# BAMresearch/PGDrome

Hardware: AMD Instinct MI355X
Metric: PGD fixed-point iters/sec + SpMV HBM GB/s, 256^3 P1 space x 1D param (higher is better)
Workload: dtype f64

## Files before the change

### include/pgd_amd.h

```cpp
#ifndef PGD_AMD_H
#define PGD_AMD_H

#include <stdint.h>

#ifdef __cplusplus
extern "C" {
#endif

typedef int64_t pgd_handle;

enum {
    PGD_OK = 0,
    PGD_ERR_INVALID = -1,
    PGD_ERR_HIP = -2,
    PGD_ERR_NOMEM = -3,
    PGD_ERR_LIMIT = -4,
    PGD_ERR_SINGULAR = -5,
    PGD_ERR_NODEVICE = -6,
    PGD_ERR_TIMEOUT = -7,
    PGD_ERR_PEER = -8
};

enum {
    PGD_ATOM_MASS = 0,
// ... 139 lines not shown
int pgd_comm_push(pgd_handle ctx, int mode, int *state);
int pgd_comm_allreduce_attach(pgd_handle ctx, const uint8_t *all_blobs, int *state);
int pgd_comm_allreduce_direct(pgd_handle ctx, int mode, int *state);
int pgd_pcg_solve_sharded(pgd_handle ctx, pgd_handle A, pgd_handle b, pgd_handle x, int64_t own0,
                          int64_t own1, int64_t lo_ghost, int64_t hi_ghost, double rtol, double atol,
                          int maxit, int *iters, double *rel_res);

int pgd_bicgstab_solve(pgd_handle ctx, pgd_handle A, pgd_handle b, pgd_handle x, double rtol, double atol,
                       int maxit, int *iters, double *rel_res);

int pgd_start_gram(pgd_handle ctx, pgd_handle A, const pgd_handle *vecs, int k, pgd_handle b, int64_t r0,
                   int64_t r1, double *out);
int pgd_start_residual(pgd_handle ctx, pgd_handle A, int k, const double *coefs, pgd_handle b, pgd_handle r);

int pgd_vec_multidot(pgd_handle ctx, pgd_handle x, const pgd_handle *ys, int k, int64_t lo, int64_t hi,
                     double *out);

int pgd_vec_multidot_pair(pgd_handle ctx, pgd_handle x0, pgd_handle x1, const pgd_handle *ys, int k, int64_t lo,
                          int64_t hi, double *out);

enum { PGD_BLOCK_F32 = 0, PGD_BLOCK_F64 = 1 };
int pgd_block_create(pgd_handle ctx, int64_t n, int k, int dtype, pgd_handle *block);
int pgd_block_free(pgd_handle ctx, pgd_handle block);
int pgd_block_info(pgd_handle ctx, pgd_handle block, int64_t *n, int *k, int *dtype, int64_t *bytes);
int pgd_block_storage(pgd_handle ctx, int *dtype);
int pgd_block_set_column(pgd_handle ctx, pgd_handle block, int j, pgd_handle vec);
int pgd_block_get_column(pgd_handle ctx, pgd_handle block, int j, pgd_handle vec);
int pgd_block_dots(pgd_handle ctx, pgd_handle block, pgd_handle vec_r, int64_t lo, int64_t hi, double *out);
int pgd_block_combine(pgd_handle ctx, pgd_handle block, const double *coefs, pgd_handle vec_base_or_0, pgd_handle vec_x);

enum { PGD_EVAL_STATS = 1, PGD_EVAL_ENVELOPE = 2, PGD_EVAL_EXCEED = 4, PGD_EVAL_FIELDS = 8 };
int pgd_eval_batch(pgd_handle ctx, const pgd_handle *modes, int k, const double *coefs, int64_t s, int want,
                   double threshold, double *sample_stats, pgd_handle env_min, pgd_handle env_max, pgd_handle exceed,
                   pgd_handle fields);

int pgd_cell_gradient(pgd_handle ctx, pgd_handle mesh, pgd_handle u, const double *L, int q, pgd_handle scale_or_0,
                      pgd_handle out);

int pgd_eval_batch_norm(pgd_handle ctx, const pgd_handle *modes, int k, int q, const double *coefs, int64_t s, int want,
                        double threshold, double *sample_stats, pgd_handle env_min, pgd_handle env_max, pgd_handle exceed,
                        pgd_handle fields);
int pgd_eval_batch_grad(pgd_handle ctx, pgd_handle mesh, const pgd_handle *modes, int k, const double *L, int q,
                        pgd_handle scale_or_0, const double *coefs, int64_t s, int want, double threshold, double *sample_stats,
                        pgd_handle env_min, pgd_handle env_max, pgd_handle exceed, pgd_handle fields);
int pgd_eval_norm_last_shape(pgd_handle ctx, int *rows, int *staged);

int pgd_cell_gradient_p2(pgd_handle ctx, pgd_handle mesh, pgd_handle u, const double *lam, int npt, const double *L, int q,
                         pgd_handle scale_or_0, pgd_handle out);
int pgd_eval_batch_grad_p2(pgd_handle ctx, pgd_handle mesh, const pgd_handle *modes, int k, const double *lam, int npt,
                           const double *L, int q, pgd_handle scale_or_0, const double *coefs, int64_t s, int want, double threshold,
                           double *sample_stats, pgd_handle env_min, pgd_handle env_max, pgd_handle exceed, pgd_handle fields);

enum {
    PGD_TUNE_SPMV_P2_LATTICE = 59,
    PGD_TUNE_SPMV_BLOCK_DIA = 58,
    PGD_TUNE_PCG_FUSED_MARCH = 57,
    PGD_TUNE_PCG_SCALAR_S = 56,
    PGD_TUNE_PCG_FOLD_MARCH = 55,
    PGD_TUNE_BLOCK_STORAGE = 54,
    PGD_TUNE_PCG_RECOMPUTE_Q = 53,
    PGD_TUNE_EVAL_SAMPLE_CHUNK = 52,
    PGD_TUNE_EVAL_GRID_MAX = 51,
    PGD_TUNE_EVAL_VARIANT = 50,
    PGD_TUNE_PUSH_IN_UPDATE = 49,
    PGD_TUNE_STENCIL_ROWS = 48,
    PGD_TUNE_DIA_MARCH3 = 47,
    PGD_TUNE_SHARD_ONE_MARCH = 46,
    PGD_TUNE_HALO_OVERLAP_MIN_ROWS = 45,
    PGD_TUNE_COMM_SELF_PERIODIC = 44,
    PGD_TUNE_PCG_DERIVE_SCALED = 43,
    PGD_TUNE_MG_MARCH_MIN = 42,
    PGD_TUNE_MG_CHUNK = 41,
    PGD_TUNE_PCG_PRECOND = 40,
    PGD_TUNE_CLS_CACHE = 39,
    PGD_TUNE_STENCIL_DEPTH = 38,
    PGD_TUNE_STENCIL_WG_PER_CU = 37,
    PGD_TUNE_SPMV_ZCHUNK_STENCIL = 36,
    PGD_TUNE_SPMV_STENCIL = 35,
    PGD_TUNE_FAULT_STALL_MS = 34,
    PGD_TUNE_FAULT_STAGE = 33,
    PGD_TUNE_SPMV_ZCHUNK_CODED2 = 32,
    PGD_TUNE_PCG_PIPELINE = 31,
    PGD_TUNE_PCG_EXACT_PHASE = 30,
    PGD_TUNE_PCG_FOLD_FINISH = 29,
    PGD_TUNE_LAZY_CSR = 28,
    PGD_TUNE_ATOM_FAST = 27,
    PGD_TUNE_SPMV_ROWS = 1,
    PGD_TUNE_SPMV_GRID_MIN_BYTES = 8,
    PGD_TUNE_PCG_FOLD_REDUCE = 12,
    PGD_TUNE_PCG_SCALED = 10,
    PGD_TUNE_SPMV_ZCHUNK_FORCE = 7,
    PGD_TUNE_PCG_SMALL_ROWS = 26,
    PGD_TUNE_PCG_SMALL_SINGLE_SYNC = 25,
    PGD_TUNE_SPMV_FETCH_DEPTH = 24,
    PGD_TUNE_PCG_STREAM_HINTS = 23,
    PGD_TUNE_PCG_LAG_X = 22,
    PGD_TUNE_SPMV_ZCHUNK_CODED = 21,
    PGD_TUNE_ASM_LATTICE = 20,
    PGD_TUNE_SPMV_ROW_CLASSES = 19,
    PGD_TUNE_PCG_SINGLE_SYNC = 18,
    PGD_TUNE_UNIT_DIAG = 17,
    PGD_TUNE_PCG_DEFER_X = 16,
    PGD_TUNE_FAULT_ITERATION = 15,
    PGD_TUNE_COMBINE_DIA = 14,
    PGD_TUNE_SPMV_VARIANT = 13,
    PGD_TUNE_SPMV_ZCHUNK = 6,
    PGD_TUNE_SPMV_SYM = 3,
    PGD_TUNE_SPMV_DICT = 2
};
int pgd_tune(pgd_handle ctx, int knob, int64_t value);

int pgd_prof_enable(pgd_handle ctx, int on);
int pgd_prof_read(pgd_handle ctx, int64_t *launches, double *seconds, double *alg_bytes);
int pgd_prof_read_own(pgd_handle ctx, double *own_bytes);
int pgd_prof_read_update(pgd_handle ctx, int64_t *launches, double *seconds, double *bytes);
int pgd_prof_read_dropped(pgd_handle ctx, int64_t *dropped);
int pgd_prof_event_overhead(pgd_handle ctx, double *seconds);
int pgd_kernel_counts(pgd_handle ctx, int64_t *out, int n);
int pgd_pcg_recompute_counts(pgd_handle ctx, int64_t *updates);
int pgd_pcg_fused_counts(pgd_handle ctx, int64_t *marches);
int pgd_classify_counts(pgd_handle ctx, int64_t *full, int64_t *cached);
int pgd_mg_counts(pgd_handle ctx, int64_t *solves, int64_t *fallbacks);
int pgd_vmg_counts(pgd_handle ctx, int64_t *solves, int64_t *fallbacks, int64_t *levels);
int pgd_vmg_times(pgd_handle ctx, double *setup_ms, int64_t *march_passes);
int pgd_cmg_counts(pgd_handle ctx, int64_t *solves, int64_t *fallbacks, int64_t *levels);
int pgd_cmg_times(pgd_handle ctx, double *setup_ms, int64_t *march_passes);
int pgd_pmg_counts(pgd_handle ctx, int64_t *solves, int64_t *fallbacks, int64_t *levels);
int pgd_pmg_times(pgd_handle ctx, double *setup_ms, int64_t *march_passes);
int pgd_pmg_coarse(pgd_handle ctx, int comp, double *slots_out, uint8_t *el_out);
int pgd_bdia_counts(pgd_handle ctx, int64_t *forms_built, int64_t *products, int64_t *fallbacks);
int pgd_bdia_times(pgd_handle ctx, double *extract_ms);
int pgd_p2lat_counts(pgd_handle ctx, int64_t *forms_built, int64_t *products, int64_t *fallbacks);
int pgd_p2lat_times(pgd_handle ctx, double *extract_ms);
int pgd_mg_slab_setup(pgd_handle ctx, pgd_handle A, int nz_global, int z_first, int64_t own0, int64_t own1,
                      int64_t *n_coarse, int *applies);
int pgd_mg_slab_fix_start(pgd_handle ctx, pgd_handle A, pgd_handle b, pgd_handle x, int64_t own0, int64_t own1);
int pgd_mg_slab_down(pgd_handle ctx, pgd_handle r, pgd_handle t);
int pgd_mg_slab_restrict(pgd_handle ctx, pgd_handle t, pgd_handle b1);
int pgd_mg_coarse(pgd_handle ctx, pgd_handle b1, pgd_handle x1);
int pgd_mg_slab_up(pgd_handle ctx, pgd_handle r, pgd_handle x1, pgd_handle t, pgd_handle z, int slot, double *dot);
int pgd_calib_stream(pgd_handle ctx, pgd_handle vec, int bytes_per_lane, int store);
int pgd_timer_start(pgd_handle ctx);
int pgd_timer_stop(pgd_handle ctx, double *seconds);

#ifdef __cplusplus
}
#endif
#endif
```

### pgdrome_amd/_lib.py

```python
from __future__ import annotations

import ctypes as C
from pathlib import Path

import numpy as np

LIB_PATH = Path(__file__).resolve().parent / "lib" / "libpgd_amd.so"

H = C.c_int64
I64 = C.c_int64
I32 = C.c_int32
F64 = C.c_double
PD = C.POINTER(C.c_double)
PI32 = C.POINTER(C.c_int32)
PI64 = C.POINTER(C.c_int64)
PH = C.POINTER(C.c_int64)
VP = C.c_void_p

PU8 = C.POINTER(C.c_uint8)
HALO_FN = C.CFUNCTYPE(C.c_int, VP, H, I64, I64, I64, I64)
ALLREDUCE_FN = C.CFUNCTYPE(C.c_int, VP, C.c_int, C.c_int)

SIGNATURES = {
    "pgd_ctx_create": (C.c_int, [C.c_int, VP, PH]),
# ... 63 lines not shown
    "pgd_mg_slab_up": (C.c_int, [H, H, H, H, H, C.c_int, PD]),
    "pgd_bicgstab_solve": (C.c_int, [H, H, H, H, C.c_double, C.c_double, C.c_int, C.POINTER(C.c_int), PD]),
    "pgd_atom_product_form": (C.c_int, [H, H, C.POINTER(C.c_int)]),
    "pgd_product_plan": (C.c_int, [H, H, I64, I64, C.c_int, PI64, C.c_int]),
    "pgd_vec_multidot": (C.c_int, [H, H, PH, C.c_int, I64, I64, PD]),
    "pgd_vec_multidot_pair": (C.c_int, [H, H, H, PH, C.c_int, I64, I64, PD]),
    "pgd_pcg_solve": (C.c_int, [H, H, H, H, F64, F64, C.c_int, C.POINTER(C.c_int), PD]),
    "pgd_pcg_last_form": (C.c_int, [H, C.POINTER(C.c_int), C.POINTER(C.c_int)]),
    "pgd_band_solve": (C.c_int, [H, H, H, H]),
    "pgd_slots_ptr": (C.c_int, [H, C.POINTER(VP)]),
    "pgd_slots_download": (C.c_int, [H, PD, C.c_int, C.c_int]),
    "pgd_slots_upload": (C.c_int, [H, PD, C.c_int, C.c_int]),
    "pgd_flags_reset": (C.c_int, [H]),
    "pgd_flags_download": (C.c_int, [H, PI32, PI32, PI32]),
    "pgd_op_diag_inv": (C.c_int, [H, H, H]),
    "pgd_spmv_dot_slot": (C.c_int, [H, H, H, H, H, I64, I64, C.c_int]),
    "pgd_pcg_init_slot": (C.c_int, [H, H, H, H, H, H, H, I64, I64, C.c_int]),
    "pgd_pcg_tol_slot": (C.c_int, [H, F64, F64, C.c_int, C.c_int, C.c_int]),
    "pgd_pcg_xr_slot": (C.c_int, [H, H, H, H, H, H, H, I64, I64, C.c_int, C.c_int, C.c_int]),
    "pgd_pcg_check_slot": (C.c_int, [H, C.c_int, C.c_int]),
    "pgd_pcg_p_slot": (C.c_int, [H, H, H, I64, I64, C.c_int, C.c_int]),
    "pgd_cg_init_slot": (C.c_int, [H, H, H, H, H, H, H, H, I64, I64, C.c_int]),
    "pgd_cg_update_slot": (C.c_int, [H, H, H, H, H, H, H, H, I64, I64, C.c_int]),
    "pgd_cg_scalars_slot": (C.c_int, [H, C.c_int, C.c_int, F64, F64]),
    "pgd_comm_bind_callbacks": (C.c_int, [H, HALO_FN, ALLREDUCE_FN, VP, C.c_int, C.c_int]),
    "pgd_comm_unique_id": (C.c_int, [H, PU8]),
    "pgd_comm_bind_rccl": (C.c_int, [H, PU8, C.c_int, C.c_int]),
    "pgd_comm_overlap": (C.c_int, [H, C.c_int, C.POINTER(C.c_int)]),
    "pgd_comm_unbind": (C.c_int, [H]),
    "pgd_comm_timeout": (C.c_int, [H, F64]),
    "pgd_comm_prof": (C.c_int, [H, C.c_int, PD]),
    "pgd_comm_info": (C.c_int, [H, C.POINTER(C.c_int), C.POINTER(C.c_int), C.POINTER(C.c_int)]),
    "pgd_comm_halo": (C.c_int, [H, H, I64, I64, I64, I64]),
    "pgd_comm_allreduce_slots": (C.c_int, [H, C.c_int, C.c_int]),
    "pgd_comm_push_export": (C.c_int, [H, I64, I64, I64, I64, I64, PU8]),
    "pgd_comm_push_attach": (C.c_int, [H, PU8, PU8, C.POINTER(C.c_int)]),
    "pgd_comm_push": (C.c_int, [H, C.c_int, C.POINTER(C.c_int)]),
    "pgd_comm_allreduce_attach": (C.c_int, [H, PU8, C.POINTER(C.c_int)]),
    "pgd_comm_allreduce_direct": (C.c_int, [H, C.c_int, C.POINTER(C.c_int)]),
    "pgd_pcg_solve_sharded": (C.c_int, [H, H, H, H, I64, I64, I64, I64, F64, F64, C.c_int, C.POINTER(C.c_int), PD]),
    "pgd_op_symmetrize": (C.c_int, [H, H, C.POINTER(C.c_int)]),
    "pgd_op_classify": (C.c_int, [H, H, C.POINTER(C.c_int)]),
    "pgd_tune": (C.c_int, [H, C.c_int, I64]),
    "pgd_prof_enable": (C.c_int, [H, C.c_int]),
    "pgd_prof_read": (C.c_int, [H, PI64, PD, PD]),
    "pgd_prof_read_own": (C.c_int, [H, PD]),
    "pgd_prof_read_update": (C.c_int, [H, PI64, PD, PD]),
    "pgd_prof_read_dropped": (C.c_int, [H, PI64]),
    "pgd_prof_event_overhead": (C.c_int, [H, PD]),
    "pgd_kernel_counts": (C.c_int, [H, PI64, C.c_int]),
    "pgd_pcg_recompute_counts": (C.c_int, [H, PI64]),
    "pgd_pcg_fused_counts": (C.c_int, [H, PI64]),
    "pgd_classify_counts": (C.c_int, [H, PI64, PI64]),
    "pgd_mg_counts": (C.c_int, [H, PI64, PI64]),
    "pgd_vmg_counts": (C.c_int, [H, PI64, PI64, PI64]),
    "pgd_vmg_times": (C.c_int, [H, C.POINTER(C.c_double), PI64]),
    "pgd_cmg_counts": (C.c_int, [H, PI64, PI64, PI64]),
    "pgd_cmg_times": (C.c_int, [H, C.POINTER(C.c_double), PI64]),
    "pgd_pmg_counts": (C.c_int, [H, PI64, PI64, PI64]),
    "pgd_pmg_times": (C.c_int, [H, C.POINTER(C.c_double), PI64]),
    "pgd_pmg_coarse": (C.c_int, [H, C.c_int, PD, PU8]),
    "pgd_bdia_counts": (C.c_int, [H, PI64, PI64, PI64]),
    "pgd_bdia_times": (C.c_int, [H, C.POINTER(C.c_double)]),
    "pgd_p2lat_counts": (C.c_int, [H, PI64, PI64, PI64]),
    "pgd_p2lat_times": (C.c_int, [H, C.POINTER(C.c_double)]),
    "pgd_calib_stream": (C.c_int, [H, H, C.c_int, C.c_int]),
    "pgd_timer_start": (C.c_int, [H]),
    "pgd_timer_stop": (C.c_int, [H, PD]),
}

NSLOTS = 64
EVAL_STATS, EVAL_ENVELOPE, EVAL_EXCEED, EVAL_FIELDS = 1, 2, 4, 8
TUNE_EVAL_VARIANT, TUNE_EVAL_GRID_MAX, TUNE_EVAL_SAMPLE_CHUNK = 50, 51, 52
TUNE_BLOCK_STORAGE = 54
TUNE_PCG_FOLD_MARCH, TUNE_PCG_SCALAR_S, TUNE_PCG_FUSED_MARCH = 55, 56, 57
TUNE_SPMV_BLOCK_DIA = 58
TUNE_SPMV_P2_LATTICE = 59
BLOCK_F32, BLOCK_F64, BLOCK_MAXK = 0, 1, 64


ERR_TIMEOUT, ERR_PEER = -7, -8


class PgdError(RuntimeError):
    def __init__(self, code, msg):
        super().__init__(f"libpgd_amd error {code}: {msg}")
        self.code = code


_lib = None


def load(path: Path | None = None):
    global _lib
    if _lib is not None and path is None:
        return _lib
    p = Path(path) if path else LIB_PATH
    if not p.exists():
        raise RuntimeError(
            f"{p} not found: build the HIP library first (python -m pgdrome_amd.build). "
            "pgdrome_amd has no CPU fallback.")
    _preload_hip_runtime()
    lib = C.CDLL(str(p))
    for name, (res, args) in SIGNATURES.items():
        fn = getattr(lib, name)
        fn.restype = res
# ... 620 lines not shown
        n = C.c_int(0)
        self._ck(self.lib.pgd_op_classify(self.h, op, C.byref(n)))
        return int(n.value)

    def tune(self, knob, value):
        self._ck(self.lib.pgd_tune(self.h, int(knob), int(value)))

    def prof_enable(self, on=True):
        self._ck(self.lib.pgd_prof_enable(self.h, int(on)))

    def prof_read(self):
        n, s, b = I64(), F64(), F64()
        self._ck(self.lib.pgd_prof_read(self.h, C.byref(n), C.byref(s), C.byref(b)))
        own = F64()
        self._ck(self.lib.pgd_prof_read_own(self.h, C.byref(own)))
        un, us, ub = I64(), F64(), F64()
        self._ck(self.lib.pgd_prof_read_update(self.h, C.byref(un), C.byref(us), C.byref(ub)))
        dr, ov = I64(), F64()
        self._ck(self.lib.pgd_prof_read_dropped(self.h, C.byref(dr)))
        self._ck(self.lib.pgd_prof_event_overhead(self.h, C.byref(ov)))
        return dict(launches=n.value, seconds=s.value, bytes=b.value, own_bytes=own.value,
                    update_launches=un.value, update_seconds=us.value, update_bytes=ub.value, dropped_noop_samples=dr.value,
                    event_overhead=ov.value)

    KERNEL_FAMILIES = ("csr", "csr_dict", "sym_rows", "dia_rows", "dia_march", "multi", "diac_march", "stencil_march")

    def kernel_counts(self):
        out = (C.c_int64 * 8)()
        self._ck(self.lib.pgd_kernel_counts(self.h, out, 8))
        return {k: int(out[i]) for i, k in enumerate(self.KERNEL_FAMILIES)}

    def product_plan(self, op, r0=0, r1=-1, pcg_like=True):
        out = (C.c_int64 * 7)()
        self._ck(self.lib.pgd_product_plan(self.h, op, int(r0), int(r1), 1 if pcg_like else 0, out, 7))
        plan = dict(zip(("form", "wgs", "zchunk", "tiles_x", "tiles_y", "rows_per_thread", "depth"), map(int, out)))
        plan["family"] = self.KERNEL_FAMILIES[plan["form"]] if plan["form"] >= 0 else None
        return plan

    def pcg_recompute_updates(self):
        n = I64()
        self._ck(self.lib.pgd_pcg_recompute_counts(self.h, C.byref(n)))
        return n.value

    def pcg_fused_marches(self):
        n = I64()
        self._ck(self.lib.pgd_pcg_fused_counts(self.h, C.byref(n)))
        return n.value

    def classify_counts(self):
        full, cached = I64(), I64()
        self._ck(self.lib.pgd_classify_counts(self.h, C.byref(full), C.byref(cached)))
        return {"full": full.value, "cached": cached.value}

    def precondition(self, multigrid):
        self.tune(40, 1 if multigrid else 0)
        return self.mg_stats()["solves"]

    def mg_stats(self):
        a, b = I64(), I64()
        self._ck(self.lib.pgd_mg_counts(self.h, C.byref(a), C.byref(b)))
        return {"solves": a.value, "fallbacks": b.value}

    def precondition_variable(self, on):
        self.tune(40, 2 if on else 0)
        return self.vmg_stats()["solves"]

    def vmg_stats(self):
        a, b, l, m, ms = I64(), I64(), I64(), I64(), C.c_double()
        self._ck(self.lib.pgd_vmg_counts(self.h, C.byref(a), C.byref(b), C.byref(l)))
        self._ck(self.lib.pgd_vmg_times(self.h, C.byref(ms), C.byref(m)))
        return {"solves": a.value, "fallbacks": b.value, "levels": l.value, "setup_ms": ms.value, "march_passes": m.value}

    def precondition_component(self, on):
        self.tune(40, 3 if on else 0)
        return self.cmg_stats()["solves"]

    def cmg_stats(self):
        a, b, l, m, ms = I64(), I64(), I64(), I64(), C.c_double()
        self._ck(self.lib.pgd_cmg_counts(self.h, C.byref(a), C.byref(b), C.byref(l)))
        self._ck(self.lib.pgd_cmg_times(self.h, C.byref(ms), C.byref(m)))
        return {"solves": a.value, "fallbacks": b.value, "levels": l.value, "setup_ms": ms.value, "march_passes": m.value}

    def precondition_p(self, on):
        self.tune(40, 4 if on else 0)
        return self.pmg_stats()["solves"]

    def pmg_stats(self):
        a, b, l, m, ms = I64(), I64(), I64(), I64(), C.c_double()
        self._ck(self.lib.pgd_pmg_counts(self.h, C.byref(a), C.byref(b), C.byref(l)))
        self._ck(self.lib.pgd_pmg_times(self.h, C.byref(ms), C.byref(m)))
        return {"solves": a.value, "fallbacks": b.value, "levels": l.value, "setup_ms": ms.value, "march_passes": m.value}

    def pmg_coarse(self, comp, nvert):
        slots = np.empty((8, int(nvert)), dtype=np.float64)
        el = np.empty(int(nvert), dtype=np.uint8)
        self._ck(self.lib.pgd_pmg_coarse(self.h, int(comp), dptr(slots), el.ctypes.data_as(PU8)))
        return slots, el

    def block_product(self, on):
        self.tune(TUNE_SPMV_BLOCK_DIA, 1 if on else 0)
        return self.bdia_stats()["products"]

    def bdia_stats(self):
        f, p, b, ms = I64(), I64(), I64(), C.c_double()
        self._ck(self.lib.pgd_bdia_counts(self.h, C.byref(f), C.byref(p), C.byref(b)))
        self._ck(self.lib.pgd_bdia_times(self.h, C.byref(ms)))
# ... 23 lines not shown
```

### pgdrome_amd/csrc/pgd_classify.hip

```cpp
#include <algorithm>
#include <cstdarg>
#include <cstdlib>
#include <cstring>

#include "pgd_internal.h"

namespace pgd {

constexpr int CLS_SLOTS = 1024;

struct StencilInfo { int ok, ident, base, split; double c[8]; int zm0, zm1, g_lo, g_hi; };

__global__ void k_stencil_pick(const uint8_t *__restrict__ cls, double *__restrict__ table, const int *__restrict__ info,
                               int nx, int ny, int z_lo, int z_hi, StencilInfo *S) {
    if (threadIdx.x != 0 || blockIdx.x != 0) return;
    S->ok = 0; S->ident = -1; S->base = -1; S->split = 0;
    const int ncls = info[0];
    if (info[1] != 0 || ncls <= 0 || ncls >= CLS_MAX || z_hi <= z_lo) return;
    const int64_t mid = (int64_t)nx * ny * ((z_lo + z_hi) / 2) + (int64_t)nx * (ny / 2) + nx / 2;
    for (int k = 0; k < ncls; ++k) {
        bool id = table[k * 8 + cls_pos(0)] == 1.0;
        for (int s = 1; s < 8; ++s) id = id && table[k * 8 + cls_pos(s)] == 0.0;
        if (id) S->ident = k;
    }
    int base = cls[mid], best = -1;
    for (int k = 0; k < ncls; ++k) {
        int nzc = 0;
        for (int s = 1; s < 8; ++s) nzc += table[k * 8 + cls_pos(s)] != 0.0 ? 1 : 0;
        if (nzc > best || (nzc == best && k == (int)cls[mid])) { best = nzc; base = k; }
    }
    if (base == S->ident) return;
    S->base = base;
    for (int s = 0; s < 8; ++s) S->c[s] = table[base * 8 + cls_pos(s)];
    if (S->ident >= 0) {
        for (int s = 0; s < 8; ++s) { table[ncls * 8 + s] = table[S->ident * 8 + s]; table[(ncls + 1) * 8 + s] = 0.0; }
    }
    S->ok = 1;
}

__global__ __launch_bounds__(TPB) void k_stencil_split(uint8_t *__restrict__ cls, const double *__restrict__ table, const int *__restrict__ info,
                                                       int nx, int ny, int64_t nv, StencilInfo *S) {
    if (!S->ok || S->ident < 0) return;
    const int64_t i = (int64_t)blockIdx.x * TPB + threadIdx.x;
    if (i >= nv || (int)cls[i] != S->ident) return;
    const int64_t P = (int64_t)nx * ny;
    const int z = (int)(i / P), rem = (int)(i - (int64_t)z * P), y = rem / nx, x = rem - y * nx;
    bool coupled = false;
#pragma unroll
    for (int s = 1; s < 8; ++s) {
        const int dx = s & 1, dy = (s >> 1) & 1, dz = s >> 2;
        if (x - dx < 0 || y - dy < 0 || z - dz < 0) continue;
        const int kc = cls[i - dx - (int64_t)nx * dy - P * dz];
        coupled = coupled || table[kc * 8 + cls_pos(s)] != 0.0;
    }
    if (coupled) { cls[i] = (uint8_t)info[0]; S->split = 1; }
}

__global__ void k_stencil_commit(double *__restrict__ table, int *__restrict__ info, StencilInfo *S) {
    if (threadIdx.x != 0 || blockIdx.x != 0 || !S->ok || S->ident < 0) return;
    const int n = info[0];
    if (S->split) info[0] = n + 1;
    else for (int s = 0; s < 8; ++s) table[n * 8 + s] = 0.0;
// ... 228 lines not shown
        if (k == ident) {
            good = table[k * 8 + cls_pos(0)] == 1.0;
            for (int s = 1; s < 8; ++s) good = good && table[k * 8 + cls_pos(s)] == 0.0;
        } else {
            good = __double_as_longlong(table[k * 8 + cls_pos(0)]) == __double_as_longlong(table[base * 8 + cls_pos(0)]);
            for (int s = 1; s < 8; ++s) {
                const double v = table[k * 8 + cls_pos(s)];
                good = good && (((pat.b[k] >> s) & 1) ? v == 0.0
                                                      : __double_as_longlong(v) == __double_as_longlong(table[base * 8 + cls_pos(s)]));
            }
        }
        if (!good) s_bad = 1;
    }
    __syncthreads();
    if (threadIdx.x == 0) {
        S->ok = s_bad ? 0 : 1; S->ident = ident; S->base = base; S->split = 0;
        for (int s = 0; s < 8; ++s) S->c[s] = table[base * 8 + cls_pos(s)];
    }
}

__global__ __launch_bounds__(TPB) void k_cls_reps(const uint8_t *__restrict__ cls, int64_t nv, int *__restrict__ reps) {
    const int64_t i = (int64_t)blockIdx.x * TPB + threadIdx.x;
    const bool active = i < nv;
    const int code = active ? (int)cls[i] : -1;
    unsigned long long todo = __ballot(active);
    const int lane = threadIdx.x & 63;
    while (todo) {
        const int leader = __ffsll((long long)todo) - 1;
        const int c0 = __shfl(code, leader);
        todo &= ~__ballot(active && code == c0);
        if (lane == leader && reps[c0] > (int)i) atomicMin(&reps[c0], (int)i);
    }
}

struct ClsJob {
    Ctx *c; const Mesh *m; Csr *a;
    int64_t plane;
    int nzp, z_lo, z_hi, g;
    bool try_stencil, dbg_cls, dbg_stencil;
    int scaled_key;
    ClsScratch *S; StencilInfo *SI;
    int info[4]; StencilInfo si;
};

__attribute__((format(printf, 2, 3))) static void cls_debug(bool on, const char *fmt, ...) {
    if (!on) return;
    va_list ap;
    va_start(ap, fmt);
    vfprintf(stderr, fmt, ap);
    va_end(ap);
}

static size_t plane_flag_bytes(int nzp) { return ((size_t)nzp * sizeof(int) + 63) / 64 * 64; }

constexpr size_t CLS_CACHE_MAX = 4, CLS_REPS_BYTES = 256 * sizeof(int);

static bool cls_cache_alloc(Mesh::ClsCache &E, int64_t nv, int nzp) {
    const size_t same_b = plane_flag_bytes(nzp);
    if (hipMalloc(&E.block, (size_t)nv + same_b + CLS_REPS_BYTES + 64 + PAD_BYTES) != hipSuccess) { E.block = nullptr; return false; }
    E.same = (int *)E.block;
    E.reps = (int *)((uint8_t *)E.block + same_b);
    E.codes = (uint8_t *)E.block + same_b + CLS_REPS_BYTES;
    return true;
}

static void cls_cache_touch(const Mesh *m, Mesh::ClsCache &E) { E.used = ++m->cls_clock; }

static void cls_cache_insert(const Mesh *m, Mesh::ClsCache &E) {
    cls_cache_touch(m, E);
    if (m->cls_cache.size() >= CLS_CACHE_MAX) {
        size_t old = 0;
        for (size_t e = 1; e < m->cls_cache.size(); ++e) if (m->cls_cache[e].used < m->cls_cache[old].used) old = e;
        m->cls_cache[old].release();
        m->cls_cache.erase(m->cls_cache.begin() + (long)old);
    }
    m->cls_cache.push_back(E);
}

static int cls_begin(ClsJob &J, Ctx *c, const Mesh *m, Csr *a, int zrange_lo, int zrange_hi, bool *go) {
    *go = false;
    if (!c->spmv_classes || m->sym_nx <= 0 || !(a->uvals && a->uvals_valid) || m->nv >= ((int64_t)1 << 31)) return PGD_OK;
    const int64_t plane = (int64_t)m->sym_nx * m->sym_ny;
    if (m->nv / plane < 3 || plane * 64 < c->spmv_grid_min_plane_bytes) return PGD_OK;
    if (m->nv / plane > 65536) return PGD_OK;
    void *p;
    if (!c->cls_scratch) { PGD_TRY(dev_alloc(c, &p, sizeof(ClsScratch) + sizeof(StencilInfo) + 2 * 65536 * sizeof(int))); c->cls_scratch = p; }
    const int nzp = (int)(m->nv / plane);
    if (!a->cls) {
        const size_t table_b = (size_t)(CLS_MAX + 1) * 8 * sizeof(double), same_b = plane_flag_bytes(nzp);
        a->cls_bytes = (size_t)m->nv + table_b + same_b + 64;
        PGD_TRY(dev_alloc(c, &p, a->cls_bytes));
        a->cls_table = (double *)p;
        a->cls_same = (int *)((uint8_t *)p + table_b);
        a->cls = (uint8_t *)a->cls_same + same_b;
    }
    J.c = c; J.m = m; J.a = a;
    J.plane = plane; J.nzp = nzp;
    J.g = (int)((m->nv + TPB - 1) / TPB);
    J.z_lo = 0; J.z_hi = nzp;
    if (zrange_lo >= 0) { J.z_lo = std::max(0, zrange_lo); J.z_hi = std::min(nzp, zrange_hi); }
    J.S = (ClsScratch *)c->cls_scratch;
    J.SI = reinterpret_cast<StencilInfo *>(J.S + 1);
    J.try_stencil = c->spmv_stencil && J.z_hi - J.z_lo >= 3;
    J.scaled_key = (a->uvals_scaled ? 1 : 0) + (a->uvals_unit ? 2 : 0) + (J.try_stencil ? 4 : 0);
    J.dbg_cls = getenv("PGD_DEBUG_CLS") != nullptr;
    J.dbg_stencil = getenv("PGD_DEBUG_STENCIL") != nullptr;
    *go = true;
    return PGD_OK;
}

static void adopt_stencil(Csr *a, const StencilInfo &si, int z_lo, int z_hi) {
    a->st_ok = true;
    a->st_ident = si.ident;
    a->st_z0 = z_lo; a->st_z1 = z_hi;
    a->st_zm0 = si.zm0; a->st_zm1 = si.zm1;
    a->st_g_lo = si.g_lo != 0; a->st_g_hi = si.g_hi != 0;
    for (int s2 = 0; s2 < 8; ++s2) a->st_c[s2] = si.c[s2];
}

static int verify_known(ClsJob &J, const Mesh::ClsCache &E) {
    Ctx *c = J.c; const Mesh *m = J.m; Csr *a = J.a;
    hipStream_t st = c->stream;
    PGD_HIP(c, hipMemsetAsync(J.S->info, 0, sizeof J.S->info, st));
    PGD_HIP(c, hipMemcpyAsync(a->cls, E.codes, (size_t)m->nv, hipMemcpyDeviceToDevice, st));
    PGD_HIP(c, hipMemcpyAsync(a->cls_same, E.same, (size_t)J.nzp * sizeof(int), hipMemcpyDeviceToDevice, st));
    k_cls_table_known<<<1, 256, 0, st>>>(a->uvals, a->uvals_stride, m->nv, E.reps, E.ncls, a->cls_table);
    k_cls_verify_known<<<J.g, TPB, 0, st>>>(a->uvals, a->uvals_stride, m->nv, a->cls_table, a->cls, E.ncls, J.S->info);
    J.si.ok = 0;
    if (E.st_ok) {
        ZeroPat zp, use;
        memcpy(zp.b, E.zero_pat, sizeof zp.b);
        memcpy(use.b, E.in_range, sizeof use.b);
        k_stencil_known<<<1, 256, 0, st>>>(a->cls_table, E.ncls, E.ident, E.base, zp, use, J.SI);
        k_stencil_ghost_init<<<1, 1, 0, st>>>(J.SI, J.z_lo, J.z_hi, J.nzp, E.zm0, E.zm1);
        if (J.z_lo > 0 || J.z_hi < J.nzp)
            k_stencil_ghost<<<(int)((J.plane + TPB - 1) / TPB), TPB, 0, st>>>(a->cls, a->cls_table, m->sym_nx, m->sym_ny, J.z_lo, J.z_hi, E.zm0, J.SI);
    }
    J.info[1] = 1;
    PGD_HIP(c, hipMemcpyAsync(J.info, J.S->info, sizeof J.info, hipMemcpyDeviceToHost, st));
    if (E.st_ok) PGD_HIP(c, hipMemcpyAsync(&J.si, J.SI, sizeof(StencilInfo), hipMemcpyDeviceToHost, st));
    PGD_HIP(c, hipStreamSynchronize(st));
    PGD_LAUNCH_CHECK(c);
    if (E.st_ok) { J.si.zm0 = E.zm0; J.si.zm1 = E.zm1; }
    return PGD_OK;
}

static int classify_known(ClsJob &J, bool *hit) {
    Ctx *c = J.c; const Mesh *m = J.m; Csr *a = J.a;
    *hit = false;
    for (size_t e = 0; e < m->cls_cache.size(); ++e) {
        Mesh::ClsCache &E = m->cls_cache[e];
        if (E.sig != a->bc_sig || E.scaled != J.scaled_key || E.z_lo != J.z_lo || E.z_hi != J.z_hi || !E.codes) continue;
        PGD_TRY(verify_known(J, E));
        cls_debug(J.dbg_cls, "[dia_classify] known structure %zu of %zu: z %d..%d mismatches %d (info %d %d %d %d) stencil %d -> %d\n", e,
                  m->cls_cache.size(), J.z_lo, J.z_hi, J.info[1], J.info[0], J.info[1], J.info[2], J.info[3], (int)E.st_ok, J.si.ok);
        if (J.info[1] != 0 || (E.st_ok && !J.si.ok)) {
            E.release();
            m->cls_cache.erase(m->cls_cache.begin() + (long)e);
            return PGD_OK;
        }
        cls_cache_touch(m, E);
        c->cls_fast += 1;
        a->cls_count = E.ncls;
        if (E.st_ok) adopt_stencil(a, J.si, J.z_lo, J.z_hi);
        *hit = true;
        return PGD_OK;
    }
    return PGD_OK;
}

static int classify_full(ClsJob &J) {
    Ctx *c = J.c; const Mesh *m = J.m; Csr *a = J.a;
    ClsScratch *S = J.S; StencilInfo *SI = J.SI;
    hipStream_t st = c->stream;
    const int g = J.g, nzp = J.nzp, z_lo = J.z_lo, z_hi = J.z_hi;
    c->cls_full += 1;
    PGD_HIP(c, hipMemsetAsync(S->keys, 0, sizeof S->keys, st));
    PGD_HIP(c, hipMemsetAsync(S->rep, 0x7f, sizeof S->rep, st));
    PGD_HIP(c, hipMemsetAsync(S->info, 0, sizeof S->info, st));
    k_cls_insert<<<g, TPB, 0, st>>>(a->uvals, a->uvals_stride, m->nv, S);
    k_cls_table<<<1, CLS_SLOTS, 0, st>>>(a->uvals, a->uvals_stride, S, a->cls_table);
    k_cls_assign<<<g, TPB, 0, st>>>(a->uvals, a->uvals_stride, m->nv, S, a->cls_table, a->cls);
    if (J.try_stencil) {
        k_stencil_pick<<<1, 64, 0, st>>>(a->cls, a->cls_table, S->info, m->sym_nx, m->sym_ny, z_lo, z_hi, SI);
        k_stencil_split<<<g, TPB, 0, st>>>(a->cls, a->cls_table, S->info, m->sym_nx, m->sym_ny, m->nv, SI);
        k_stencil_commit<<<1, 64, 0, st>>>(a->cls_table, S->info, SI);
    }
    k_cls_planes<<<nzp, TPB, 0, st>>>(a->cls, J.plane, nzp, a->cls_same);
    if (J.try_stencil) {
        const int64_t rows = J.plane * (z_hi - z_lo);
        k_stencil_verify<<<(int)((rows + TPB - 1) / TPB), TPB, 0, st>>>(a->cls, a->cls_table, m->sym_nx, m->sym_ny, nzp, z_lo, z_hi, SI);
        int *allid = reinterpret_cast<int *>(SI + 1);
        k_stencil_allid<<<nzp, TPB, 0, st>>>(a->cls, J.plane, SI, allid, allid + 65536);
        k_stencil_planes<<<1, 64, 0, st>>>(allid + 65536, allid, z_lo, z_hi, SI);
        k_stencil_ghost_init<<<1, 1, 0, st>>>(SI, z_lo, z_hi, nzp, -1, -1);
        if (z_lo > 0 || z_hi < nzp)
            k_stencil_ghost<<<(int)((J.plane + TPB - 1) / TPB), TPB, 0, st>>>(a->cls, a->cls_table, m->sym_nx, m->sym_ny, z_lo, z_hi, -1, SI);
    }
    J.info[0] = 0; J.info[1] = 1; J.si.ok = 0;
    PGD_HIP(c, hipMemcpyAsync(J.info, S->info, sizeof J.info, hipMemcpyDeviceToHost, st));
    if (J.try_stencil) PGD_HIP(c, hipMemcpyAsync(&J.si, SI, sizeof(StencilInfo), hipMemcpyDeviceToHost, st));
    PGD_HIP(c, hipStreamSynchronize(st));
    PGD_LAUNCH_CHECK(c);
    if (J.info[1] != 0 || J.info[0] <= 0 || J.info[0] > CLS_MAX) return PGD_OK;
    a->cls_count = J.info[0];
    cls_debug(J.dbg_stencil, "[dia_classify] classes %d info1 %d try %d ok %d ident %d base %d c = %.17g %.17g %.17g %.17g %.17g %.17g %.17g %.17g  z [%d, %d)\n",
              J.info[0], J.info[1], (int)J.try_stencil, J.si.ok, J.si.ident, J.si.base, J.si.c[0], J.si.c[1], J.si.c[2], J.si.c[3], J.si.c[4],
              J.si.c[5], J.si.c[6], J.si.c[7], z_lo, z_hi);
    cls_debug(J.dbg_stencil, "[dia_classify] main run [%d, %d)\n", J.si.zm0, J.si.zm1);
    return PGD_OK;
}

static bool cls_cache_fill(const ClsJob &J, Mesh::ClsCache &E, int (&reps_rng)[256], double *tab) {
    const Mesh *m = J.m; const Csr *a = J.a;
    hipStream_t st = J.c->stream;
    bool okc = hipMemcpyAsync(E.codes, a->cls, (size_t)m->nv, hipMemcpyDeviceToDevice, st) == hipSuccess &&
               hipMemcpyAsync(E.same, a->cls_same, (size_t)J.nzp * sizeof(int), hipMemcpyDeviceToDevice, st) == hipSuccess &&
               hipMemsetAsync(E.reps, 0x7f, CLS_REPS_BYTES, st) == hipSuccess;
    if (okc) {
        const int64_t r0 = (int64_t)J.z_lo * J.plane, r1 = std::min<int64_t>((int64_t)J.z_hi * J.plane, m->nv);
        if (r1 > r0) k_cls_reps<<<(int)((r1 - r0 + TPB - 1) / TPB), TPB, 0, st>>>(a->cls + r0, r1 - r0, E.reps);
        okc = hipMemcpyAsync(reps_rng, E.reps, sizeof reps_rng, hipMemcpyDeviceToHost, st) == hipSuccess &&
              hipStreamSynchronize(st) == hipSuccess && hipMemsetAsync(E.reps, 0x7f, CLS_REPS_BYTES, st) == hipSuccess;
    }
    if (okc) {
        k_cls_reps<<<J.g, TPB, 0, st>>>(a->cls, m->nv, E.reps);
        okc = hipMemcpyAsync(tab, a->cls_table, (size_t)(E.ncls + 1) * 8 * sizeof(double), hipMemcpyDeviceToHost, st) == hipSuccess &&
              hipStreamSynchronize(st) == hipSuccess;
    }
    return okc;
}

static void remember(const ClsJob &J) {
    const Csr *a = J.a;
    const int ncls = a->cls_count;
    Mesh::ClsCache E;
    E.sig = a->bc_sig; E.scaled = J.scaled_key; E.z_lo = J.z_lo; E.z_hi = J.z_hi; E.ncls = ncls;
    if (!cls_cache_alloc(E, J.m->nv, J.nzp)) { (void)hipGetLastError(); return; }
    double tab[(CLS_MAX + 1) * 8];
    int reps_rng[256];
    if (!cls_cache_fill(J, E, reps_rng, tab)) {
        E.release();
        (void)hipGetLastError();
        return;
    }
    E.st_ok = a->st_ok; E.ident = a->st_ident; E.base = J.try_stencil ? J.si.base : -1; E.zm0 = a->st_zm0; E.zm1 = a->st_zm1;
    for (int k = 0; k < 256; ++k) E.in_range[k] = (k < ncls && reps_rng[k] >= 0 && reps_rng[k] < 0x7f000000) ? 1 : 0;
    for (int k = 0; k < 256; ++k) {
        uint8_t b = 0;
        if (k < ncls) for (int s2 = 1; s2 < 8; ++s2) if (tab[k * 8 + cls_pos(s2)] == 0.0) b |= (uint8_t)(1u << s2);
        E.zero_pat[k] = b;
    }
    if (E.base >= 0) for (int k = 0; k < ncls; ++k) E.zero_pat[k] &= (uint8_t)~E.zero_pat[E.base];
    cls_cache_insert(J.m, E);
}

int dia_classify(Ctx *c, const Mesh *m, Csr *a, int zrange_lo, int zrange_hi) {
    a->drop_classes();
    ClsJob J;
    bool go = false, hit = false;
    PGD_TRY(cls_begin(J, c, m, a, zrange_lo, zrange_hi, &go));
    if (!go) return PGD_OK;
    if (c->cls_cache_on) PGD_TRY(classify_known(J, &hit));
    if (hit) return PGD_OK;
    PGD_TRY(classify_full(J));
    if (a->cls_count <= 0) return PGD_OK;
    if (J.try_stencil && J.si.ok) adopt_stencil(a, J.si, J.z_lo, J.z_hi);
    if (c->cls_cache_on) remember(J);
    return PGD_OK;
}

}
```

### pgdrome_amd/csrc/pgd_internal.h

```cpp
#pragma once

#include <hip/hip_runtime.h>

#include <chrono>
#include <cstdint>
#include <cstdio>
#include <map>
#include <memory>
#include <string>
#include <vector>

#include "../../include/pgd_amd.h"

namespace pgd {

constexpr int WAVE = 64;
constexpr int TPB = 256;
constexpr int MAX_VEC_BLOCKS = 2048;
constexpr int N_XCD = 8;
constexpr int DICT_MAXP = 256;
constexpr int DICT_DLEN = 32;
constexpr size_t PAD_BYTES = 256;

enum { S_PQ = 2, S_TOL2 = 5, S_DMIN = 7 , S_TMP = 8  };
enum { S1_RZ = 24, S1_RR = 25, S1_ALPHA = 26, S1_BETA = 27, S1_PQ = 28, S1_QQ = 29,
       S1_ALPHA_PREV = 40, S1_BETA_PREV = 41, S1_PEND = 42 };
enum { S1F_ALPHA = 44 , S1F_BETA = 46 , S1F_EXACT = 48  };
constexpr double LAG_MIN_BETA = 0.01;

struct Ctx;
void dev_release(Ctx *c, void *p, size_t bytes);

struct Obj {
    enum Kind { FREE = 0, VEC, MESH, CSR, BLOCK } kind = FREE;
    Ctx *ctx = nullptr;
    uint64_t serial = 0;
    virtual ~Obj() {}
};

struct Vec : Obj {
    double *d = nullptr;
    int64_t n = 0;
    ~Vec() override { if (d) dev_release(ctx, d, (size_t)(n > 0 ? n : 1) * sizeof(double)); }
};

struct Block : Obj {
    void *d = nullptr;
    int64_t n = 0, stride = 0;
    int k = 0, dtype = 0;
    size_t bytes = 0;
    ~Block() override { if (d) dev_release(ctx, d, bytes); }
};

struct Mesh : Obj {
    int gdim = 0, nvpc = 0;
    int ncomp = 1;
    pgd_handle base = 0;
    int64_t nv = 0, nc = 0, nnz = 0;
    double *coords = nullptr;
    int4 *cells = nullptr;
    int *cellsN = nullptr;
    int *v2c_ptr = nullptr;
    int *v2c = nullptr;
    int *row_ptr = nullptr;
    int *cols = nullptr;
    int max_row = 0, kl = 0, ku = 0;
    int *sym_tab = nullptr;
    int sym_w = 0;
    int sym_nx = 0, sym_ny = 0;
    bool lattice = false;
    bool lattice_unit = false;
    bool lattice_regular = false;
    int pat_off[6][4] = {{0}};
    int pat_loc[6][8] = {{0}};
    double lat_h[3] = {0.0, 0.0, 0.0};
    struct ClsCache {
        uint64_t sig = 0; int scaled = 0, z_lo = 0, z_hi = 0, ncls = 0;
        void *block = nullptr;
        uint8_t *codes = nullptr; int *same = nullptr; int *reps = nullptr;
        bool st_ok = false; int ident = -1, base = -1, zm0 = 0, zm1 = 0;
        uint8_t zero_pat[256];
        uint8_t in_range[256];
        uint64_t used = 0;
        void release() { if (block) (void)hipFree(block); block = nullptr; codes = nullptr; same = reps = nullptr; }
    };
    mutable std::vector<ClsCache> cls_cache;
    mutable uint64_t cls_clock = 0;
    std::vector<int32_t> bc_host;
    int *bc_dev = nullptr;
    size_t bc_dev_bytes = 0;
    uint16_t *pids = nullptr;
    int *dict_off = nullptr;
    int dict_count = 0;
    int p2_bound = 0;
    int p2_nx = 0, p2_ny = 0, p2_nz = 0;
    int64_t p2_nvert = 0;
    int *p2_par = nullptr;
    int *p2_v2e = nullptr;
    int p2_lat = 0;
    ~Mesh() override {
        for (void *p : {(void *)coords, (void *)cells, (void *)cellsN, (void *)v2c_ptr, (void *)v2c,
                        (void *)row_ptr, (void *)cols, (void *)pids, (void *)dict_off, (void *)sym_tab, (void *)p2_par, (void *)p2_v2e})
            if (p) (void)hipFree(p);
        for (ClsCache &e : cls_cache) e.release();
        if (bc_dev) (void)hipFree(bc_dev);
    }
};

struct Csr : Obj {
    pgd_handle mesh = 0;
    double *vals = nullptr;
    double *dinv = nullptr;
    bool dinv_valid = false;
    double *uvals = nullptr;
    bool uvals_valid = false;
    bool uvals_scaled = false;
    bool uvals_unit = false;
    int64_t uvals_stride = 0;
    uint8_t *cls = nullptr;
    int *cls_same = nullptr;
    double *cls_table = nullptr;
    int cls_count = 0;
    uint64_t bc_sig = 0;
    bool st_ok = false;
    int st_ident = -1, st_z0 = 0, st_z1 = 0, st_zm0 = 0, st_zm1 = 0;
    double st_c[8] = {0, 0, 0, 0, 0, 0, 0, 0};
    bool st_g_lo = false, st_g_hi = false;
    void drop_classes() { cls_count = 0; st_ok = false; st_g_lo = st_g_hi = false; }
    bool st_virtual = false;
    bool cls_tried = false;
    bool immutable = false;
    uint64_t version = 0;
    bool vals_pending = false;
    std::vector<pgd_handle> rec_atoms;
    std::vector<uint64_t> rec_serials, rec_versions;
    std::vector<double> rec_coefs;
    int *rec_bc = nullptr;
    int64_t rec_nbc = 0;
    size_t rec_bc_bytes = 0;
    size_t vals_bytes = 0, dinv_bytes = 0, uvals_bytes = 0, cls_bytes = 0;
    double *bdia = nullptr;
    size_t bdia_bytes = 0;
    int64_t bdia_stride = 0;
    uint64_t bdia_seen = 0;
    bool bdia_ok = false;
    double *p2lat = nullptr;
    size_t p2lat_bytes = 0;
    int64_t p2lat_sv = 0, p2lat_se = 0;
    uint64_t p2lat_seen = 0;
    bool p2lat_ok = false;
    ~Csr() override {
        if (p2lat) dev_release(ctx, p2lat, p2lat_bytes);
        if (bdia) dev_release(ctx, bdia, bdia_bytes);
        if (rec_bc) dev_release(ctx, rec_bc, rec_bc_bytes);
        if (cls_table) dev_release(ctx, cls_table, cls_bytes);
        if (vals) dev_release(ctx, vals, vals_bytes);
        if (dinv) dev_release(ctx, dinv, dinv_bytes);
        if (uvals) dev_release(ctx, uvals, uvals_bytes);
    }
};

struct Comm {
    int kind = 0;
    int rank = 0, world = 1;
    pgd_halo_fn halo_cb = nullptr;
    pgd_allreduce_fn allreduce_cb = nullptr;
    void *user = nullptr;
    void *nccl = nullptr;
    void *nccl_halo = nullptr;
    hipStream_t halo_stream = nullptr;
    hipEvent_t ev_ready = nullptr, ev_halo = nullptr;
    bool overlap = false;
    int64_t overlap_min_rows = (int64_t)1 << 40;
    bool overlap_used = false;
    bool self_periodic = false;
    pgd_handle work[7] = {0, 0, 0, 0, 0, 0, 0};
    int64_t work_n = 0;
    double timeout_s = 60.0;
    int *snap_flags = nullptr;
    double *snap_vote = nullptr;
    hipEvent_t snap_ev[2] = {nullptr, nullptr};
    bool prof = false;
    hipEvent_t mark[2][7] = {{nullptr, nullptr, nullptr, nullptr, nullptr, nullptr, nullptr}, {nullptr, nullptr, nullptr, nullptr, nullptr, nullptr, nullptr}};
// ... 50 lines not shown

    Comm comm;

    int num_cu = 256;
    int spmv_dict = 1;
    int spmv_rows = 64;
    int64_t spmv_grid_min_plane_bytes = 0;
    int spmv_zchunk_force = 0;
    int fault_iteration = -1;
    int fault_stage = 0;
    int fault_stall_ms = 0;
    int64_t pcg_small_ss_rows = (int64_t)1 << 22;
    int pcg_small_ss = 1;
    int pcg_stream_hints = 1;
    int pcg_lag_x = 1;
    int pcg_recompute_q = 1;
    int64_t pcg_recompute_launches = 0;
    int pcg_fold_march = 0;
    int64_t pcg_fused_launches = 0;
    int pcg_fused_march = 1;
    int pcg_scalar_s = 1;
    int asm_lattice = 1;
    int spmv_fetch_depth = 6;
    int spmv_zchunk_coded2 = 96;
    int spmv_zchunk_coded = 24;
    int pcg_exact_phase = 1;
    int pcg_fold_finish = 1;
    int atom_fast = 1;
    int lazy_csr = 1;
    uint64_t next_serial = 1;
    int pcg_precond = 0;
    struct Mg *mg = nullptr;
    struct Mg *mg_slab = nullptr;
    int64_t mg_solves = 0, mg_fallbacks = 0;
    struct Vmg *vmg = nullptr;
    int64_t vmg_solves = 0, vmg_fallbacks = 0, vmg_marches = 0;
    double vmg_setup_ms = 0.0;
    struct Cmg *cmg = nullptr;
    int64_t cmg_solves = 0, cmg_fallbacks = 0, cmg_marches = 0;
    double cmg_setup_ms = 0.0;
    struct Pmg *pmg = nullptr;
    int64_t pmg_solves = 0, pmg_fallbacks = 0, pmg_marches = 0;
    double pmg_setup_ms = 0.0;
    int eval_variant = 1, eval_grid_max = 0, eval_chunk = 0;
    int eval_norm_rows = 0, eval_norm_staged = -1;
    double *eval_pin = nullptr;
    size_t eval_pin_bytes = 0;
    hipEvent_t eval_ev[2] = {nullptr, nullptr};
    bool eval_ev_set[2] = {false, false};
    int mg_chunk = 2;
    int mg_march_min = 64;
    int cls_cache_on = 1;
    int64_t cls_fast = 0, cls_full = 0;
    int spmv_stencil = 1;
    int spmv_zchunk_stencil = 0;
    int stencil_depth = 0;
    int stencil_wg_per_cu = 2;
    int spmv_classes = 1;
    void *cls_scratch = nullptr;
    double *gram_w = nullptr;
    size_t gram_w_bytes = 0;
    pgd_handle gram_op = 0;
    int gram_k = 0;
    int64_t gram_n = 0;
    int spmv_variant = 0;
    int spmv_zchunk = 8;
    int pcg_fold_reduce = 1;
    int spmv_qq = 0;
    int pcg_single_sync = 1;
    int spmv_unit_diag = 1;
    int pcg_defer_x = 1;
    int pcg_scaled = 1;
    int stencil_rows = 0;
    int dia_march3 = 0;
    int push_in_update = 1;
    int shard_one_march = 1;
    int pcg_derive_scaled = 1;
    int spmv_combine_dia = 1;
    int spmv_sym = 1;
    int spmv_block_dia = 0;
    int64_t bdia_forms = 0, bdia_products = 0, bdia_fallbacks = 0;
    double bdia_extract_ms = 0.0;
    hipEvent_t bdia_ev[2] = {nullptr, nullptr};
    int spmv_p2_lattice = 0;
    int64_t p2lat_forms = 0, p2lat_products = 0, p2lat_fallbacks = 0;
    double p2lat_extract_ms = 0.0;
    hipEvent_t p2lat_ev[2] = {nullptr, nullptr};
    uint16_t *p2lat_tab = nullptr;
    int16_t *p2lat_slot = nullptr;
    int block_storage = 1;

    bool prof = false;
    bool prof_pcg_only = false;
    std::vector<hipEvent_t> ev;
    struct ProfRec { uint8_t kind; int iter; double bytes, own, seconds; };
    std::vector<ProfRec> ev_rec;
    std::vector<ProfRec> prof_pend;
    int prof_iter = -1;
    int64_t prof_dropped = 0;
    double prof_overhead = -1.0;
    size_t ev_used = 0;
    int64_t prof_upd_launches = 0, prof_upd_seen = 0;
    double prof_upd_seconds = 0.0, prof_upd_bytes = 0.0;
    int64_t prof_launches = 0, prof_seen = 0;
    double prof_seconds = 0.0, prof_bytes = 0.0;
    double prof_own_bytes = 0.0;
// ... 6 lines not shown
};

struct ProfIterGuard { Ctx *c; ~ProfIterGuard() { c->prof_iter = -1; } };
inline double host_now() { return std::chrono::duration<double>(std::chrono::steady_clock::now().time_since_epoch()).count(); }

enum { KC_CSR = 0, KC_CSR_DICT = 1, KC_SYM_ROWS = 2, KC_DIA_ROWS = 3, KC_DIA_MARCH = 4, KC_MULTI = 5, KC_DIAC_MARCH = 6, KC_STENCIL_MARCH = 7 };

Ctx *get_ctx(pgd_handle h);
int fail(Ctx *c, int code, const char *fmt, ...);
pgd_handle put_obj(Ctx *c, Obj *o);
Obj *get_obj(Ctx *c, pgd_handle h, Obj::Kind k);
int free_obj(Ctx *c, pgd_handle h, Obj::Kind k);
int dev_alloc(Ctx *c, void **p, size_t bytes);
int ensure_partials(Ctx *c, int64_t n);
int ensure_work(Ctx *c, int i, int64_t n);
int ensure_mask(Ctx *c, int64_t n);
int pcg_flag_snapshots(Ctx *c);
int ensure_ibuf(Ctx *c, int64_t n);
void prof_flush(Ctx *c);
void prof_commit(Ctx *c, int valid_products, int valid_updates);
void comm_release(Ctx *c);
struct Mesh;
struct Csr;
int build_sym_tables(Ctx *c, Mesh *m);
int ensure_sym(Ctx *c, const Mesh *m, Csr *a, bool *usable);
int cg_init_s(Ctx *c, const double *b, const double *q, const double *sc, double *r, double *p, double *s, int64_t lo,
              int64_t hi, int base);
int cg_update_s(Ctx *c, double *x, double *r, const double *w, double *p, double *s, const double *sc, int64_t lo, int64_t hi,
                int base);
int cg_update_s2(Ctx *c, double *x, double *r, const double *w, double *p, double *s, const double *sc, int64_t lo, int64_t hi,
                 int base, int parity, int *nblocks);
int reduce_two_slots(Ctx *c, int na, int nb, int base);
int pcg1_seed(Ctx *c, int npairs, int slot_rz, int slot_rr);
int pcg1_tol(Ctx *c, int base, double rtol, double atol, int slot_p8);
int pcg1_aux(Ctx *c, const double *s, const double *r, int64_t lo, int64_t hi, int slot);
int pcg1_sums(Ctx *c, int nprod, int nvec, int base);
int pcg1_finish_slots(Ctx *c, int base);
struct PushArgs {
    double *dst_lo = nullptr, *dst_hi = nullptr;
    int64_t lo_end = 0, hi_begin = 0;
    unsigned long long *post_lo = nullptr, *post_hi = nullptr;
    const unsigned long long *wait_a = nullptr, *wait_b = nullptr;
    unsigned long long seq = 0, *ticket = nullptr;
    unsigned int nblocks = 0;
    long long ticks = 0;
};
unsigned int pcg1_update_push_blocks(int g, int64_t lo, int64_t hi, int64_t lo_end, int64_t hi_begin);
int pcg1_update(Ctx *c, double *x, double *r, double *p, const double *q, const double *sc, int64_t lo, int64_t hi, int base,
                int *nblocks, int lag, int fold_par, const PushArgs *push = nullptr);
int pcg1_flush_x(Ctx *c, double *x, const double *p, const double *r, int64_t lo, int64_t hi, int base, int fold_par);
int vec_sqrt(Ctx *c, double *v, int64_t n);
int vec_div_mul(Ctx *c, double *x, const double *sc, int64_t n, int mul);
int ensure_vals(Ctx *c, const Mesh *m, Csr *a);
bool atom_fast_form(Ctx *c, const Mesh *m, Csr *a, int64_t r0, int64_t r1);
constexpr int CLS_MAX = 255;
__host__ __device__ constexpr int cls_pos(int s) {
    return s == 1 ? 0 : s == 5 ? 1 : s == 3 ? 2 : s == 7 ? 3 : s == 2 ? 4 : s == 6 ? 5 : s == 4 ? 6 : 7;
}
int dia_classify(Ctx *c, const Mesh *m, Csr *a, int zrange_lo = -1, int zrange_hi = -1);
bool stencil_row_range(const Ctx *c, const Mesh *m, const Csr *a, int64_t r0, int64_t r1);
bool stencil_whole_grid(const Ctx *c, const Mesh *m, const Csr *a);
struct StencilFold {
    const double *prod; int nprod;
    const double *vec_in; int nvec;
    int par;
};
int stencil_update_blocks(const Ctx *c, const Mesh *m, const Csr *a);
int launch_stencil_update(Ctx *c, const Mesh *m, const Csr *a, const double *p_in, double *p_out, double *x, double *r, const double *s,
                          double *pairs, int lag, double s_free = 0.0, const StencilFold *fold = nullptr);
bool stencil_fused_ok(const Ctx *c, const Mesh *m, const Csr *a);
int launch_stencil_fused(Ctx *c, const Mesh *m, const Csr *a, const double *p_in, double *p_out, double *x, const double *r_in, double *r_out,
                         const double *s, double *pairs, int lag, double s_free);
int launch_stencil_pass(Ctx *c, const uint8_t *cls, int ident, const double cst[8], int nx, int ny, int nz, int zm0, int zm1,
                        const double *x, const double *b, double *y, double w, int epi, bool dot, int *nparts, int z0 = 0, int z1 = -1);
bool mg_prepare(Ctx *c, const Mesh *m, const Csr *a);
int mg_fix_start(Ctx *c, const Csr *a, const double *b, double *x, int64_t n);
int mg_vcycle(Ctx *c, const double *r, bool dot, int *nparts, double *z_out = nullptr);
double *mg_result(Ctx *c);
void mg_release(Ctx *c);
struct Vmg;
bool vmg_prepare(Ctx *c, Vmg *&M, const Mesh *m, const Csr *a);
int vmg_fix_start(Ctx *c, Vmg *M, const double *sc, const double *b, double *x, int64_t n);
int vmg_vcycle(Ctx *c, Vmg *M, const double *r, bool dot, int *nparts, double *z_out, int64_t *marches);
double *vmg_result(Vmg *M);
void vmg_note_setup(Ctx *c);
void vmg_release(Ctx *c);
bool cmg_prepare(Ctx *c, const Mesh *m, const Mesh *base, const Csr *a);
int cmg_fix_start(Ctx *c, const double *b, double *x, int64_t n);
int cmg_apply(Ctx *c, const double *r, double *z, int64_t n, int *nparts);
void cmg_note_setup(Ctx *c);
bool pmg_prepare(Ctx *c, const Mesh *m, const Csr *a);
int pmg_fix_start(Ctx *c, const double *b, double *x, int64_t n);
int pmg_apply(Ctx *c, const Csr *a, const double *r, double *z, int64_t n, int *nparts);
void pmg_note_setup(Ctx *c);
void pmg_release(Ctx *c);
void eval_release(Ctx *c);
int sym_scale(Ctx *c, const Mesh *m, Csr *a, const double *s);
int launch_spmv_dia_rows2(Ctx *c, const Mesh *m, const Csr *a, const double *x, double *y, const double *w, int64_t r0a,
                          int64_t r1a, int64_t r0b, int64_t r1b, bool dot, const int *flags, int *nparts_out, bool *done);
int combine_dia(Ctx *c, const Mesh *m, Csr *o, Csr *const *atoms, const double *coefs, int n, const uint8_t *mask);
int launch_spmv_op(Ctx *c, const Mesh *m, const Csr *a, const double *x, double *y, const double *w, int64_t r0,
                   int64_t r1, bool dot, bool store, const int *flags, int *nparts_out);
int launch_spmv_bdia(Ctx *c, const Mesh *m, Csr *a, const double *x, double *y, const double *w, bool dot, bool store,
                     const int *flags, int *nparts_out, bool *done);
bool p2lat_degree2(Ctx *c, const Mesh *m);
int launch_spmv_p2lat(Ctx *c, const Mesh *m, Csr *a, const double *x, double *y, const double *w, bool dot, bool store,
// ... 107 lines not shown
```

### pgdrome_amd/csrc/pgd_pcg.hip

```cpp
#include "pgd_internal.h"

#include <cmath>

#include <cstring>

#include <algorithm>

namespace pgd {

constexpr int MAXT = 8;
constexpr int CHECK_EVERY = 16;
constexpr int PROF_EAGER_EVERY = 8;

struct CombineArgs {
    const double *in[MAXT];
    double coef[MAXT];
    int n;
};

__global__ __launch_bounds__(TPB) void k_combine(CombineArgs A, double *__restrict__ out, const int *__restrict__ cols,
                                                 const uint8_t *__restrict__ colmask, int64_t nnz) {
    for (int64_t k = (int64_t)blockIdx.x * TPB + threadIdx.x; k < nnz; k += (int64_t)gridDim.x * TPB) {
        double s = 0.0;
#pragma unroll
        for (int t = 0; t < MAXT; ++t)
            if (t < A.n) s = fma(A.coef[t], A.in[t][k], s);
        if (colmask && colmask[cols[k]]) s = 0.0;
        out[k] = s;
    }
}

__global__ __launch_bounds__(TPB) void k_mask_set(uint8_t *__restrict__ mask, const int *__restrict__ dofs, int64_t n) {
    for (int64_t i = (int64_t)blockIdx.x * TPB + threadIdx.x; i < n; i += (int64_t)gridDim.x * TPB) mask[dofs[i]] = 1;
}

__global__ __launch_bounds__(TPB) void k_dirichlet_rows(const int *__restrict__ dofs, int64_t n,
                                                        const int *__restrict__ row_ptr, const int *__restrict__ cols,
                                                        double *__restrict__ vals) {
    for (int64_t i = (int64_t)blockIdx.x * TPB + threadIdx.x; i < n; i += (int64_t)gridDim.x * TPB) {
        const int r = dofs[i];
        for (int k = row_ptr[r]; k < row_ptr[r + 1]; ++k) vals[k] = (cols[k] == r) ? 1.0 : 0.0;
    }
}

__global__ __launch_bounds__(TPB) void k_diag_inv(const int *__restrict__ row_ptr, const int *__restrict__ cols,
                                                  const double *__restrict__ vals, double *__restrict__ dinv, int64_t n) {
    for (int64_t r = (int64_t)blockIdx.x * TPB + threadIdx.x; r < n; r += (int64_t)gridDim.x * TPB) {
        double d = 0.0;
        for (int k = row_ptr[r]; k < row_ptr[r + 1]; ++k)
            if (cols[k] == (int)r) d = vals[k];
        dinv[r] = 1.0 / d;
    }
}
// ... 323 lines not shown
                    const double t = W[a1]; W[a1] = W[a2]; W[a2] = t;
                }
                const double t = rhs[j]; rhs[j] = rhs[piv]; rhs[piv] = t;
            }
            const double dinv = 1.0 / W[kv + (int64_t)j * ld];
            for (int i = j + 1; i <= imax; ++i) {
                const double l = W[(i - j + kv) + (int64_t)j * ld] * dinv;
                if (l != 0.0) {
                    for (int cc = j + 1; cc <= cmax; ++cc)
                        W[(i - cc + kv) + (int64_t)cc * ld] -= l * W[(j - cc + kv) + (int64_t)cc * ld];
                    rhs[i] -= l * rhs[j];
                }
            }
        }
        if (!singular) {
            for (int j = n - 1; j >= 0; --j) {
                const int cmax = min(j + kv, n - 1);
                double s = rhs[j];
                for (int cc = j + 1; cc <= cmax; ++cc) s -= W[(j - cc + kv) + (int64_t)cc * ld] * rhs[cc];
                rhs[j] = s / W[kv + (int64_t)j * ld];
            }
        } else {
            flags[2] = PGD_ERR_SINGULAR;
        }
    }
    __syncthreads();
    for (int i = threadIdx.x; i < n; i += TPB) x[i] = rhs[i];
}


__global__ __launch_bounds__(TPB) void k_scale_in(const double *__restrict__ dinv, double *__restrict__ s,
                                                  double *__restrict__ x, int64_t n, unsigned long long *__restrict__ dmax_bits) {
    double mx = 0.0;
    for (int64_t i = (int64_t)blockIdx.x * TPB + threadIdx.x; i < n; i += (int64_t)gridDim.x * TPB) {
        const double di = dinv[i], si = sqrt(di);
        s[i] = si;
        x[i] = x[i] / si;
        mx = fmax(mx, di);
    }
    for (int o = 32; o > 0; o >>= 1) mx = fmax(mx, __shfl_xor(mx, o));
    if ((threadIdx.x & 63) == 0) {
        const unsigned long long mine = (unsigned long long)__double_as_longlong(mx);
        if (mine > __hip_atomic_load(dmax_bits, __ATOMIC_RELAXED, __HIP_MEMORY_SCOPE_AGENT)) atomicMax(dmax_bits, mine);
    }
}

struct StencilTuple { double c[8]; };
__global__ void k_stencil_derive(StencilTuple A, int unit, double *__restrict__ out) {
    if (threadIdx.x != 0 || blockIdx.x != 0) return;
    const double dinv = 1.0 / A.c[0], si = sqrt(dinv);
    out[0] = unit ? 1.0 : A.c[0] * si * si;
    for (int s = 1; s < 8; ++s) { double v = A.c[s]; v *= si * si; out[s] = v; }
    out[8] = si;
}

__global__ void k_dmin_slot(const unsigned long long *__restrict__ dmax_bits, double *__restrict__ slots, int *__restrict__ flags) {
    const double dmax_inv = __longlong_as_double((long long)dmax_bits[0]);
    slots[S_DMIN] = dmax_inv > 0.0 ? 1.0 / dmax_inv : 0.0;
    if (!(dmax_inv > 0.0) || !(dmax_inv < 1e300)) { flags[0] = 1; flags[2] = PGD_ERR_SINGULAR; }
}

__global__ __launch_bounds__(TPB) void k_pcg_init_s(const double *__restrict__ b, const double *__restrict__ q,
                                                    const double *__restrict__ s, double *__restrict__ r,
                                                    double *__restrict__ p, int64_t n, double *__restrict__ partials) {
    __shared__ double s_red[4];
    double rz = 0.0, rr = 0.0, bb = 0.0;
    for (int64_t i = (int64_t)blockIdx.x * TPB + threadIdx.x; i < n; i += (int64_t)gridDim.x * TPB) {
        const double bi = b[i], si = s[i], ri = si * bi - q[i], ti = ri / si;
        r[i] = ri; p[i] = ri;
        rz = fma(ri, ri, rz); rr = fma(ti, ti, rr); bb = fma(bi, bi, bb);
    }
    rz = block_sum(rz, s_red);
    rr = block_sum(rr, s_red);
    bb = block_sum(bb, s_red);
    if (threadIdx.x == 0) {
        partials[3 * blockIdx.x + 0] = rz;
        partials[3 * blockIdx.x + 1] = rr;
        partials[3 * blockIdx.x + 2] = bb;
    }
}

__global__ __launch_bounds__(TPB) void k_pcg_xr_s(double *__restrict__ x, double *__restrict__ r, const double *__restrict__ p,
                                                  const double *__restrict__ q, const double *__restrict__ s, int64_t n,
                                                  const double *__restrict__ slots, int slot_rz, int slot_pq,
                                                  double *__restrict__ partials, const int *__restrict__ flags) {
    if (flags[0]) return;
    __shared__ double s_red[4];
    typedef double d2 __attribute__((ext_vector_type(2)));
    const double alpha = slots[slot_rz] / slots[slot_pq];
    const bool exact = flags[3] != 0;
    double rz = 0.0, rr = 0.0;
    const int64_t npair = n >> 1;
    for (int64_t k = (int64_t)blockIdx.x * TPB + threadIdx.x; k < npair; k += (int64_t)gridDim.x * TPB) {
        const int64_t i = 2 * k;
        const d2 pi = *reinterpret_cast<const d2 *>(p + i), qi = *reinterpret_cast<const d2 *>(q + i);
        d2 xi = *reinterpret_cast<d2 *>(x + i), ri = *reinterpret_cast<d2 *>(r + i);
        xi.x = fma(alpha, pi.x, xi.x); xi.y = fma(alpha, pi.y, xi.y);
        ri.x = fma(-alpha, qi.x, ri.x); ri.y = fma(-alpha, qi.y, ri.y);
        *reinterpret_cast<d2 *>(x + i) = xi;
        *reinterpret_cast<d2 *>(r + i) = ri;
        rz = fma(ri.x, ri.x, rz); rz = fma(ri.y, ri.y, rz);
        if (exact) {
            const d2 si = *reinterpret_cast<const d2 *>(s + i);
            const double tx = ri.x / si.x, ty = ri.y / si.y;
            rr = fma(tx, tx, rr); rr = fma(ty, ty, rr);
        }
// ... 489 lines not shown
        if (n & 1) p[n - 1] = fma(beta, p[n - 1], r[n - 1]);
        slots[out] = rz; slots[out + 1] = rr;
        const double tol2 = slots[slot_tol2];
        flags[1] += 1;
        if (!(rz == rz) || !(rr == rr)) { flags[0] = 1; flags[2] = PGD_ERR_SINGULAR; }
        else if (flags[3]) { if (rr <= tol2) flags[0] = 1; }
        else if (rz * slots[S_DMIN] <= 1e4 * tol2) flags[3] = 1;
    }
}

int ensure_vals(Ctx *c, const Mesh *m, Csr *o) {
    if (!o->vals_pending) return o->vals ? PGD_OK : fail(c, PGD_ERR_INVALID, "operator without values (its pgd_op_combine failed?)");
    const int n = (int)o->rec_atoms.size();
    if (!o->vals) {
        void *p;
        const size_t cnt = (size_t)(m->nnz > 0 ? m->nnz : 1);
        o->vals_bytes = cnt * sizeof(double);
        PGD_TRY(dev_alloc(c, &p, o->vals_bytes));
        o->vals = (double *)p;
        const size_t used = (size_t)(m->nnz > 0 ? m->nnz : 0);
        PGD_HIP(c, hipMemsetAsync(o->vals + used, 0, (cnt - used) * sizeof(double) + PAD_BYTES, c->stream));
    }
    std::vector<const double *> in((size_t)n);
    for (int t = 0; t < n; ++t) {
        Csr *a = get_csr(c, o->rec_atoms[(size_t)t]);
        if (!a || a->serial != o->rec_serials[(size_t)t] || a->version != o->rec_versions[(size_t)t])
            return fail(c, PGD_ERR_INVALID, "operator: its CSR values were left to the first reader and atom %d has been freed or rewritten since", t);
        PGD_TRY(ensure_vals(c, m, a));
        in[(size_t)t] = a->vals;
    }
    const uint8_t *mask = nullptr;
    if (o->rec_nbc > 0) {
        PGD_TRY(ensure_mask(c, m->nv));
        PGD_HIP(c, hipMemsetAsync(c->mask, 0, (size_t)m->nv, c->stream));
        k_mask_set<<<grid_for(o->rec_nbc), TPB, 0, c->stream>>>(c->mask, o->rec_bc, o->rec_nbc);
        mask = c->mask;
    }
    const int g = grid_for(m->nnz, TPB, 4 * MAX_VEC_BLOCKS);
    for (int t = 0, pass = 0; t < n; ++pass) {
        CombineArgs A;
        int cnt = 0;
        if (pass > 0) { A.in[0] = o->vals; A.coef[0] = 1.0; cnt = 1; }
        while (t < n && cnt < MAXT) { A.in[cnt] = in[(size_t)t]; A.coef[cnt] = o->rec_coefs[(size_t)t]; ++cnt; ++t; }
        for (int k = cnt; k < MAXT; ++k) { A.in[k] = in[0]; A.coef[k] = 0.0; }
        A.n = cnt;
        k_combine<<<g, TPB, 0, c->stream>>>(A, o->vals, m->cols, (t >= n) ? mask : nullptr, m->nnz);
    }
    if (o->rec_nbc > 0) k_dirichlet_rows<<<grid_for(o->rec_nbc), TPB, 0, c->stream>>>(o->rec_bc, o->rec_nbc, m->row_ptr, m->cols, o->vals);
    PGD_LAUNCH_CHECK(c);
    o->vals_pending = false;
    return PGD_OK;
}

int csr_diag_inv(Ctx *c, const Mesh *m, Csr *a) {
    if (a->dinv_valid) return PGD_OK;
    if (!a->dinv) {
        void *p;
        a->dinv_bytes = (size_t)m->nv * sizeof(double);
        PGD_TRY(dev_alloc(c, &p, a->dinv_bytes));
        a->dinv = (double *)p;
    }
    PGD_TRY(ensure_vals(c, m, a));
    k_diag_inv<<<grid_for(m->nv), TPB, 0, c->stream>>>(m->row_ptr, m->cols, a->vals, a->dinv, m->nv);
    PGD_LAUNCH_CHECK(c);
    a->dinv_valid = true;
    return PGD_OK;
}

static int pcg_init(Ctx *c, const double *b, const double *q, const double *dinv, double *r, double *z, double *p,
                    int64_t lo, int64_t hi, int slot) {
    const int g = grid_for(hi - lo);
    PGD_TRY(ensure_partials(c, 4 * (int64_t)MAX_VEC_BLOCKS));
    k_pcg_init<<<g, TPB, 0, c->stream>>>(b, q, dinv, r, z, p, lo, hi, c->partials);
    PGD_LAUNCH_CHECK(c);
    return reduce_partials(c, c->partials, g, 3, slot, -1, 0, 0);
}

int cg_init_s(Ctx *c, const double *b, const double *q, const double *sc, double *r, double *p, double *s, int64_t lo,
              int64_t hi, int base) {
    if (hi == lo) return PGD_OK;
    const int g = grid_for(hi - lo);
    PGD_TRY(ensure_partials(c, 4 * (int64_t)MAX_VEC_BLOCKS));
    k_cg_init_s<<<g, TPB, 0, c->stream>>>(b, q, sc, r, p, s, lo, hi, c->partials);
    PGD_LAUNCH_CHECK(c);
    PGD_TRY(reduce_partials(c, c->partials, g, 3, 40, -1, 0, 0));
    PGD_HIP(c, hipMemcpyAsync(c->slots + base, c->slots + 40, 2 * sizeof(double), hipMemcpyDeviceToDevice, c->stream));
    PGD_HIP(c, hipMemcpyAsync(c->slots + base + 8, c->slots + 42, sizeof(double), hipMemcpyDeviceToDevice, c->stream));
    return PGD_OK;
}

int cg_update_s(Ctx *c, double *x, double *r, const double *w, double *p, double *s, const double *sc, int64_t lo, int64_t hi,
                int base) {
    if (hi == lo) return PGD_OK;
    const int g = grid_for(hi - lo);
    PGD_TRY(ensure_partials(c, 4 * (int64_t)MAX_VEC_BLOCKS));
    k_cg_update_s<<<g, TPB, 0, c->stream>>>(x, r, w, p, s, sc, lo, hi, c->slots, base, c->partials, c->flags);
    PGD_LAUNCH_CHECK(c);
    return reduce_partials(c, c->partials, g, 2, base, 0, 0, 0);
}

int cg_update_s2(Ctx *c, double *x, double *r, const double *w, double *p, double *s, const double *sc, int64_t lo, int64_t hi,
                 int base, int parity, int *nblocks) {
    *nblocks = 0;
    if (hi == lo) return PGD_OK;
    const int g = grid_for(hi - lo);
    PGD_TRY(ensure_work(c, 6, 2 * (int64_t)MAX_VEC_BLOCKS));
    k_cg_update_s2<<<g, TPB, 0, c->stream>>>(x, r, w, p, s, sc, lo, hi, c->slots, base, parity, c->work[6], c->flags);
// ... 207 lines not shown
    const double *fprod = nullptr;
    int fnprod = 0;
    double st_saved[8] = {0, 0, 0, 0, 0, 0, 0, 0};
    ~PcgRun() {
        if (virt) {
            for (int s2 = 0; s2 < 8; ++s2) o->st_c[s2] = st_saved[s2];
            o->st_virtual = false;
        }
        if (!x_scaled) return;
        (void)vec_div_mul(c, x, sc, n, 1);
        if (!virt) invalidate_slots();
    }
    void invalidate_slots() { o->uvals_valid = false; o->uvals_scaled = false; }
    int out(int k) const { return S_PAIR + 2 * (k & 1); }
    int old(int k) const { return S_PAIR + 2 * ((k + 1) & 1); }
    int g2() const { return grid_for((n + 1) / 2); }
};

static int pcg_precond_prepare(PcgRun &R) {
    Ctx *c = R.c;
    const Mesh *m = R.m;
    const int want = c->pcg_precond;
    if (want == 1 && R.scaled && mg_prepare(c, m, R.o)) { R.precond = PGD_PCG_PRECOND_MG; c->mg_solves += 1; return mg_fix_start(c, R.o, R.b, R.x, R.n); }
    if (want == 2 && R.scaled && m->sym_nx > 0 && vmg_prepare(c, c->vmg, m, R.o)) { R.precond = PGD_PCG_PRECOND_VMG; c->vmg_solves += 1; return vmg_fix_start(c, c->vmg, R.sc, R.b, R.x, R.n); }
    if (want == 3 && !R.scaled && m->ncomp >= 2) {
        PGD_TRY(ensure_vals(c, m, R.o));
        if (cmg_prepare(c, m, get_mesh(c, m->base), R.o)) { R.precond = PGD_PCG_PRECOND_CMG; c->cmg_solves += 1; return cmg_fix_start(c, R.b, R.x, R.n); }
    }
    if (want == 4 && !R.scaled) {
        PGD_TRY(ensure_vals(c, m, R.o));
        if (pmg_prepare(c, m, R.o)) { R.precond = PGD_PCG_PRECOND_PMG; c->pmg_solves += 1; return pmg_fix_start(c, R.b, R.x, R.n); }
    }
    if (want == 1) c->mg_fallbacks += 1;
    if (want == 2) c->vmg_fallbacks += 1;
    if (want == 3) c->cmg_fallbacks += 1;
    if (want == 4) c->pmg_fallbacks += 1;
    return PGD_OK;
}

static int pcg_precond_apply(PcgRun &R, const double *r, double *z_out, int *np) {
    switch (R.precond) {
    case PGD_PCG_PRECOND_MG: return mg_vcycle(R.c, r, true, np, z_out);
    case PGD_PCG_PRECOND_VMG: return vmg_vcycle(R.c, R.c->vmg, r, true, np, z_out, &R.c->vmg_marches);
    case PGD_PCG_PRECOND_CMG: return cmg_apply(R.c, r, z_out ? z_out : R.z, R.n, np);
    case PGD_PCG_PRECOND_PMG: return pmg_apply(R.c, R.o, r, z_out ? z_out : R.z, R.n, np);
    case PGD_PCG_PRECOND_JACOBI: break;
    }
    return fail(R.c, PGD_ERR_INVALID, "pcg_solve: no cycle to apply");
}
static double *pcg_precond_result(PcgRun &R) {
    return R.precond == PGD_PCG_PRECOND_MG ? mg_result(R.c) : R.precond == PGD_PCG_PRECOND_VMG ? vmg_result(R.c->vmg) : R.z;
}

static int pcg_derive_stencil(PcgRun &R) {
    Ctx *c = R.c;
    Csr *o = R.o;
    if (!(c->pcg_derive_scaled && R.m->sym_nx > 0 && c->pcg_precond != 2)) return PGD_OK;
    if (o->cls_count <= 0) PGD_TRY(dia_classify(c, R.m, o));
    if (!(stencil_whole_grid(c, R.m, o) && o->st_ident >= 0 && o->st_c[0] > 0.0)) return PGD_OK;
    PGD_TRY(ensure_work(c, 5, 4096));
    StencilTuple in;
    for (int s2 = 0; s2 < 8; ++s2) in.c[s2] = o->st_c[s2];
    k_stencil_derive<<<1, 1, 0, c->stream>>>(in, c->spmv_unit_diag, c->work[5] + 16);
    PGD_LAUNCH_CHECK(c);
    double out9[9];
    PGD_HIP(c, hipMemcpyAsync(out9, c->work[5] + 16, sizeof out9, hipMemcpyDeviceToHost, c->stream));
    PGD_HIP(c, hipStreamSynchronize(c->stream));
    for (double v : out9) if (!std::isfinite(v)) return PGD_OK;
    for (int s2 = 0; s2 < 8; ++s2) { R.st_saved[s2] = o->st_c[s2]; o->st_c[s2] = out9[s2]; }
    o->st_virtual = R.virt = true;
    R.s_free = out9[8];
    return PGD_OK;
}

static int pcg_setup_scaled(PcgRun &R) {
    Ctx *c = R.c;
    const int64_t n = R.n;
    PGD_TRY(ensure_work(c, 5, 4096));
    unsigned long long *bits = reinterpret_cast<unsigned long long *>(c->work[5]);
    PGD_HIP(c, hipMemsetAsync(bits, 0, sizeof(unsigned long long), c->stream));
    k_scale_in<<<grid_for(n), TPB, 0, c->stream>>>(R.o->dinv, R.sc, R.x, n, bits);
    k_dmin_slot<<<1, 1, 0, c->stream>>>(bits, c->slots, c->flags);
    PGD_LAUNCH_CHECK(c);
    R.x_scaled = true;
    PGD_TRY(pcg_derive_stencil(R));
    if (!R.virt) {
        PGD_TRY(sym_scale(c, R.m, R.o, R.sc));
        PGD_TRY(dia_classify(c, R.m, R.o));
    }
    PGD_TRY(pcg_precond_prepare(R));
    PGD_TRY(launch_spmv_op(c, R.m, R.o, R.x, R.q, nullptr, 0, n, false, true, nullptr, nullptr));
    const int g = grid_for(n);
    PGD_TRY(ensure_partials(c, 4 * (int64_t)MAX_VEC_BLOCKS));
    k_pcg_init_s<<<g, TPB, 0, c->stream>>>(R.b, R.q, R.sc, R.r, R.p, n, c->partials);
    PGD_LAUNCH_CHECK(c);
    return reduce_partials(c, c->partials, g, 3, R.S_INIT, -1, 0, 0);
}

static int pcg_setup_unscaled(PcgRun &R) {
    PGD_TRY(pcg_precond_prepare(R));
    PGD_TRY(launch_spmv_op(R.c, R.m, R.o, R.x, R.q, nullptr, 0, R.n, false, true, nullptr, nullptr));
    return pcg_init(R.c, R.b, R.q, R.o->dinv, R.r, R.z, R.p, 0, R.n, R.S_INIT);
}

static int64_t pcg_partials_needed(int64_t n) { return std::max<int64_t>(4 * (int64_t)MAX_VEC_BLOCKS, 2 * ((n + 63) / 64) + 64); }

static int pcg_choose_and_seed(PcgRun &R) {
    Ctx *c = R.c;
    const int64_t n = R.n;
    if (R.precond != PGD_PCG_PRECOND_JACOBI) {
        int np = 0;
        PGD_TRY(pcg_precond_apply(R, R.r, R.p, &np));
        PGD_TRY(reduce_partials(c, c->partials, np, 1, R.S_INIT, -1, 0, 0));
    }
    PGD_TRY(ensure_work(c, 6, 4 * (int64_t)MAX_VEC_BLOCKS));
    c->pcg_last_precond = R.precond;
    c->pcg_last_form = R.form = pcg_choose(c, R.precond, R.scaled, n, R.m->sym_nx > 0, stencil_whole_grid(c, R.m, R.o));
    R.lag_x = c->pcg_lag_x && pcg_single_sync(R.form);
    R.g2v = grid_for((n + 1) / 2, TPB, (n > ((int64_t)1 << 20) && n <= c->pcg_small_ss_rows && c->pcg_small_ss) ? 512 : MAX_VEC_BLOCKS);
    R.gvec = R.form == PGD_PCG_FORM_SINGLE_SYNC_RECOMPUTE ? stencil_update_blocks(c, R.m, R.o) : R.g2v;
    R.fused = R.form == PGD_PCG_FORM_SINGLE_SYNC_RECOMPUTE && c->pcg_fused_march && stencil_fused_ok(c, R.m, R.o);
    R.fold_march = R.form == PGD_PCG_FORM_SINGLE_SYNC_RECOMPUTE && c->pcg_fold_march && !R.fused;
    const int64_t half = 2 * std::max<int64_t>(MAX_VEC_BLOCKS, R.fold_march ? R.gvec : 0);
    PGD_TRY(ensure_work(c, 6, std::max<int64_t>(2 * half, 2 * (int64_t)R.gvec)));
    R.part2 = c->work[6];
    R.part2b = R.part2 + half;
    if (!pcg_single_sync(R.form)) return PGD_OK;
    const bool two = R.form == PGD_PCG_FORM_TWO_LAUNCH || R.fold_march;
    k_pcg1_seed<<<8, TPB, 0, c->stream>>>(two ? R.part2b : R.part2, R.gvec, c->slots, R.S_INIT, R.S_INIT + 1);
    if (two) PGD_HIP(c, hipMemsetAsync(c->slots + S1F_ALPHA, 0, 6 * sizeof(double), c->stream));
    PGD_LAUNCH_CHECK(c);
    if (R.fused) {
        PGD_TRY(ensure_work(c, 4, n));
        R.r2 = c->work[4];
        PGD_TRY(ensure_partials(c, pcg_partials_needed(n)));
        PGD_TRY(ensure_work(c, 5, 4096));
        if (c->prof) c->prof_seen &= ~(int64_t)3;
        c->spmv_qq = 1;
// ... 215 lines not shown
    return rc_loop;
}

static int pcg_finish(PcgRun &R, const int f[4], int *iters, double *relres) {
    Ctx *c = R.c;
    if (R.scaled) {
        const int g = grid_for(R.n);
        R.x_scaled = false;
        const bool pending = R.form == PGD_PCG_FORM_DEFERRED_X && f[0] != 0 && f[1] > 0;
        const bool lag_pending = R.lag_x && f[1] > 0 && ((f[1] - 1) & 1) == 0;
        const int last_par = f[1] > 0 ? (f[1] - 1) & 1 : 0;
        const bool two = R.form == PGD_PCG_FORM_TWO_LAUNCH || R.fold_march;
        const double *p_live = R.form == PGD_PCG_FORM_SINGLE_SYNC_RECOMPUTE && (f[1] & 1) ? R.q : R.p;
        const double *r_live = R.fused && (f[1] & 1) ? R.r2 : R.r;
        k_scale_out<<<g, TPB, 0, c->stream>>>(R.x, r_live, R.sc, R.n, c->partials, (pending || lag_pending) ? p_live : nullptr, c->slots,
                                              R.S_PAIR + 2 * (f[1] & 1), S_PQ, lag_pending ? 1 : 0,
                                              two ? S1F_ALPHA + last_par : S1_ALPHA, two ? S1F_BETA + last_par : S1_BETA);
        PGD_LAUNCH_CHECK(c);
        PGD_TRY(reduce_partials(c, c->partials, g, 1, S_TMP, -1, 0, 0));
        if (!R.virt) R.invalidate_slots();
    }
    PGD_LAUNCH_CHECK(c);
    double s[PGD_NSLOTS];
    PGD_HIP(c, hipMemcpyAsync(s, c->slots, sizeof s, hipMemcpyDeviceToHost, c->stream));
    PGD_HIP(c, hipStreamSynchronize(c->stream));
    if (R.precond == PGD_PCG_PRECOND_VMG) vmg_note_setup(c);
    if (R.precond == PGD_PCG_PRECOND_CMG) cmg_note_setup(c);
    if (R.precond == PGD_PCG_PRECOND_PMG) pmg_note_setup(c);
    if (iters) *iters = f[1];
    const double rr = R.scaled ? s[S_TMP] : (f[1] > 0) ? s[R.S_PAIR + 2 * ((f[1] - 1) & 1) + 1] : s[R.S_INIT + 1];
    const double bb = s[R.S_INIT + 2];
    if (relres) *relres = (bb > 0.0) ? sqrt(rr / bb) : 0.0;
    if (f[2] != 0) return fail(c, f[2], "pcg_solve: breakdown (NaN residual) after %d iterations", f[1]);
    return PGD_OK;
}

}

using namespace pgd;

extern "C" {

int pgd_op_combine(pgd_handle h, pgd_handle mh, const pgd_handle *atoms, const double *coefs, int n,
                   const int32_t *bc_dofs, int64_t nbc, pgd_handle *op) {
    PGD_CTX(c, h);
    Mesh *m = get_mesh(c, mh);
    if (!m || !atoms || !coefs || !op || n < 1 || nbc < 0 || (nbc > 0 && !bc_dofs))
        return fail(c, PGD_ERR_INVALID, "op_combine: invalid arguments");
    std::vector<Csr *> atom_objs((size_t)n);
    for (int t = 0; t < n; ++t) {
        Csr *a = get_csr(c, atoms[t]);
        if (!a || a->mesh != mh) return fail(c, PGD_ERR_INVALID, "op_combine: atom %d is not on this mesh", t);
        if (*op && atoms[t] == *op) return fail(c, PGD_ERR_INVALID, "op_combine: output aliases an input");
        atom_objs[t] = a;
    }
    const bool bc_known = nbc > 0 && m->bc_dev && m->bc_host.size() == (size_t)nbc &&
                          std::memcmp(m->bc_host.data(), bc_dofs, (size_t)nbc * sizeof(int32_t)) == 0;
    if (!bc_known)
        for (int64_t i = 0; i < nbc; ++i)
            if (bc_dofs[i] < 0 || bc_dofs[i] >= m->nv) return fail(c, PGD_ERR_INVALID, "op_combine: bc dof out of range");
    Csr *o = nullptr;
    if (*op) {
        o = get_csr(c, *op);
        if (!o || o->mesh != mh) return fail(c, PGD_ERR_INVALID, "op_combine: *op is not an operator on this mesh");
    } else {
        std::unique_ptr<Csr> a(new Csr);
        a->kind = Obj::CSR;
        a->mesh = mh;
        o = a.get();
        *op = put_obj(c, a.release());
    }
    o->dinv_valid = false;
    o->uvals_valid = false;
    o->vals_pending = false;
    o->version += 1;
    o->rec_atoms.assign(atoms, atoms + n);
    o->rec_coefs.assign(coefs, coefs + n);
    o->rec_serials.resize((size_t)n);
    o->rec_versions.resize((size_t)n);
    for (int t = 0; t < n; ++t) { o->rec_serials[(size_t)t] = atom_objs[t]->serial; o->rec_versions[(size_t)t] = atom_objs[t]->version; }
    if (o->rec_bc && o->rec_bc_bytes < (size_t)nbc * sizeof(int)) { dev_release(c, o->rec_bc, o->rec_bc_bytes); o->rec_bc = nullptr; }
    o->rec_nbc = nbc;
    {
        uint64_t hsig = 0x9e3779b97f4a7c15ull ^ (uint64_t)nbc;
        auto mix = [&](uint64_t v) { hsig = (hsig ^ v) * 0xff51afd7ed558ccdull; hsig ^= hsig >> 32; };
        const int64_t step = nbc > 4096 ? nbc / 4096 : 1;
        for (int64_t i = 0; i < nbc; i += step) mix((uint64_t)(uint32_t)bc_dofs[i]);
        if (nbc > 0) mix((uint64_t)(uint32_t)bc_dofs[nbc - 1]);
        for (int t = 0; t < n; ++t) mix(atom_objs[t]->serial);
        o->bc_sig = hsig ? hsig : 1;
    }
    const uint8_t *mask = nullptr;
    if (nbc > 0) {
        if (!o->rec_bc) {
            void *p;
            o->rec_bc_bytes = (size_t)nbc * sizeof(int);
            PGD_TRY(dev_alloc(c, &p, o->rec_bc_bytes));
            o->rec_bc = (int *)p;
        }
        PGD_TRY(ensure_mask(c, m->nv));
        PGD_HIP(c, hipMemsetAsync(c->mask, 0, (size_t)m->nv, c->stream));
        if (!bc_known) {
            m->bc_host.clear();
            if (m->bc_dev && m->bc_dev_bytes < (size_t)nbc * sizeof(int)) { (void)hipFree(m->bc_dev); m->bc_dev = nullptr; }
            if (!m->bc_dev) {
                void *p = nullptr;
                m->bc_dev_bytes = (size_t)nbc * sizeof(int);
                if (hipMalloc(&p, m->bc_dev_bytes + PAD_BYTES) != hipSuccess) { (void)hipGetLastError(); m->bc_dev_bytes = 0; }
                m->bc_dev = (int *)p;
            }
            PGD_HIP(c, hipMemcpyAsync(o->rec_bc, bc_dofs, (size_t)nbc * sizeof(int), hipMemcpyHostToDevice, c->stream));
            if (m->bc_dev) {
                PGD_HIP(c, hipMemcpyAsync(m->bc_dev, o->rec_bc, (size_t)nbc * sizeof(int), hipMemcpyDeviceToDevice, c->stream));
                m->bc_host.assign(bc_dofs, bc_dofs + nbc);
            }
        } else {
            PGD_HIP(c, hipMemcpyAsync(o->rec_bc, m->bc_dev, (size_t)nbc * sizeof(int), hipMemcpyDeviceToDevice, c->stream));
        }
        k_mask_set<<<grid_for(nbc), TPB, 0, c->stream>>>(c->mask, o->rec_bc, nbc);
        mask = c->mask;
    }
    o->vals_pending = true;
    PGD_TRY(combine_dia(c, m, o, atom_objs.data(), coefs, n, mask));
    if (!(c->lazy_csr && o->uvals_valid)) PGD_TRY(ensure_vals(c, m, o));
    if (nbc > 0 && !bc_known) PGD_HIP(c, hipStreamSynchronize(c->stream));
    return PGD_OK;
}

int pgd_op_diag_inv(pgd_handle h, pgd_handle oh, pgd_handle dh) {
    PGD_CTX(c, h);
    Csr *o = get_csr(c, oh);
    Mesh *m = o ? get_mesh(c, o->mesh) : nullptr;
    Vec *d = get_vec(c, dh);
    if (!o || !m || !d || d->n != m->nv) return fail(c, PGD_ERR_INVALID, "op_diag_inv: invalid handles");
    if (o->dinv_valid && o->dinv) {
        PGD_HIP(c, hipMemcpyAsync(d->d, o->dinv, (size_t)m->nv * sizeof(double), hipMemcpyDeviceToDevice, c->stream));
        return PGD_OK;
    }
    PGD_TRY(ensure_vals(c, m, o));
    k_diag_inv<<<grid_for(m->nv), TPB, 0, c->stream>>>(m->row_ptr, m->cols, o->vals, d->d, m->nv);
    PGD_LAUNCH_CHECK(c);
    return PGD_OK;
}

int pgd_pcg_solve(pgd_handle h, pgd_handle oh, pgd_handle bh, pgd_handle xh, double rtol, double atol, int maxit,
                  int *iters, double *relres) {
    PGD_CTX(c, h);
    Csr *o = get_csr(c, oh);
    Mesh *m = o ? get_mesh(c, o->mesh) : nullptr;
    Vec *b = get_vec(c, bh), *x = get_vec(c, xh);
    if (!o || !m || !b || !x || b->n != m->nv || x->n != m->nv || b == x || maxit < 0)
        return fail(c, PGD_ERR_INVALID, "pcg_solve: invalid handles or size mismatch");
    const int64_t n = m->nv;
    const bool dbg_t = getenv("PGD_DEBUG_PCG") != nullptr;
    const double dbg_t0 = host_now();
    ProfIterGuard prof_iter_guard{c};
    c->prof_pend.clear();
    PGD_TRY(csr_diag_inv(c, m, o));
    bool sym = false;
    PGD_TRY(ensure_sym(c, m, o, &sym));
    for (int i = 0; i < 4; ++i) PGD_TRY(ensure_work(c, i, n));
    PGD_HIP(c, hipMemsetAsync(c->flags, 0, 8 * sizeof(int), c->stream));
    PcgRun R{c, m, o, b->d, x->d, n, c->work[0], c->work[1], c->work[2], c->work[3], c->work[1]};
    R.scaled = sym && c->pcg_scaled && n >= 2;
    PGD_TRY(R.scaled ? pcg_setup_scaled(R) : pcg_setup_unscaled(R));
    k_pcg_tol<<<1, 64, 0, c->stream>>>(c->slots, c->flags, rtol, atol, R.S_INIT + 1, R.S_INIT + 2, S_TOL2);
    PGD_LAUNCH_CHECK(c);
    PGD_TRY(pcg_choose_and_seed(R));

    const int CE = R.form == PGD_PCG_FORM_PRECOND ? std::max(2, std::min(c->mg_chunk & ~1, CHECK_EVERY)) : CHECK_EVERY;
    int f[4] = {0, 0, 0, 0}, enq = 0;
    double dbg[4] = {0, 0, 0, 0};
    const int rc_loop = pcg_drive(R, CE, maxit, f, enq, dbg_t ? dbg : nullptr);
    if (dbg_t) fprintf(stderr, "[pcg_solve] n %lld graph %s iterations queued %d counted %d stencil %d cls %d form %d precond %d | setup %.2f ms capture %.2f ms loop %.2f ms = %.1f us/it\n", (long long)n, dbg[3] != 0.0 ? "yes" : "NO", enq, f[1], (int)o->st_ok, o->cls_count, (int)R.form, (int)R.precond, 1e3 * (dbg[0] - dbg_t0), 1e3 * (dbg[1] - dbg[0]), 1e3 * (dbg[2] - dbg[1]), 1e6 * (dbg[2] - dbg[1]) / (f[1] > 0 ? f[1] : 1));
    c->prof_iter = -1;
    if (c->prof) prof_commit(c, rc_loop == PGD_OK ? f[1] + (pcg_single_sync(R.form) ? 1 : 0) : 0, rc_loop == PGD_OK ? f[1] : 0);
    if (rc_loop != PGD_OK) return rc_loop;
    return pcg_finish(R, f, iters, relres);
}

int pgd_pcg_last_form(pgd_handle h, int *form, int *precond) {
    PGD_CTX(c, h);
    if (form) *form = c->pcg_last_form;
    if (precond) *precond = c->pcg_last_precond;
    return PGD_OK;
}

int pgd_band_solve(pgd_handle h, pgd_handle oh, pgd_handle bh, pgd_handle xh) {
    PGD_CTX(c, h);
    Csr *o = get_csr(c, oh);
    Mesh *m = o ? get_mesh(c, o->mesh) : nullptr;
    Vec *b = get_vec(c, bh), *x = get_vec(c, xh);
    if (!o || !m || !b || !x || b->n != m->nv || x->n != m->nv)
        return fail(c, PGD_ERR_INVALID, "band_solve: invalid handles or size mismatch");
    const int64_t n = m->nv, ld = 2 * (int64_t)m->kl + m->ku + 1;
    const int64_t need = n * ld + n;
    if (need > ((int64_t)1 << 27)) return fail(c, PGD_ERR_LIMIT, "band_solve: system too large for the direct path (n=%lld, band=%lld)", (long long)n, (long long)ld);
    const int use_lds = need <= BAND_LDS_DOUBLES;
    if (!use_lds) PGD_TRY(ensure_work(c, 4, need));
    PGD_TRY(ensure_vals(c, m, o));
    PGD_HIP(c, hipMemsetAsync(c->flags, 0, 8 * sizeof(int), c->stream));
    k_band_solve<<<1, TPB, 0, c->stream>>>(m->row_ptr, m->cols, o->vals, b->d, x->d, (int)n, m->kl, m->ku,
                                           use_lds ? nullptr : c->work[4], use_lds, c->flags);
    PGD_LAUNCH_CHECK(c);
    int f[4];
    PGD_HIP(c, hipMemcpyAsync(f, c->flags, sizeof f, hipMemcpyDeviceToHost, c->stream));
    PGD_HIP(c, hipStreamSynchronize(c->stream));
    if (f[2] != 0) return fail(c, PGD_ERR_SINGULAR, "band_solve: zero pivot");
    return PGD_OK;
}

static int get3(Ctx *c, pgd_handle a, pgd_handle b, pgd_handle d, Vec **A, Vec **B, Vec **D) {
    *A = get_vec(c, a); *B = get_vec(c, b); *D = get_vec(c, d);
// ... 108 lines not shown
```

### pgdrome_amd/csrc/pgd_product_plan.h

```cpp
#pragma once

#include "pgd_internal.h"

#include <algorithm>

namespace pgd {

constexpr int DIAC_MAXCHUNK = 1024;

enum { PLAN_NOT_BY_FORM = -1 };
enum { MARCH_WY8 = 0, MARCH_WY4 = 1, MARCH_2 = 2, MARCH_3 = 3 };

struct ProductPlan {
    int form = PLAN_NOT_BY_FORM;
    int variant = 0;
    int nblk = 0;
    int wgs = 0;
    int z0 = 0, z1 = 0, zchunk = 0, tiles_x = 0, tiles_y = 0;
    int rows_per_thread = 0, depth = 0;
    bool six = false;
};

struct StencilShape { int rows_per_thread, tiles_x, tiles_y, zchunk, wgs; };
inline StencilShape stencil_shape(const Ctx *c, int nx, int ny, int planes, int depth) {
    StencilShape sh;
    sh.tiles_x = (nx + 63) / 64;
    sh.tiles_y = (ny + 15) / 16;
    const int64_t slots = (int64_t)c->stencil_wg_per_cu * c->num_cu;
    const int64_t marches4 = std::max<int64_t>(1, slots / ((int64_t)sh.tiles_x * sh.tiles_y));
    const int zc4 = (int)((planes + marches4 - 1) / marches4);
    sh.rows_per_thread = (c->stencil_rows == 2 || (c->stencil_rows == 0 && zc4 < 8 && ny >= 16 && c->spmv_zchunk_stencil <= 0 && c->stencil_depth != 6)) ? 2 : 4;
    if (sh.rows_per_thread == 2) sh.tiles_y = (ny + 7) / 8;
    const int64_t tiles = (int64_t)sh.tiles_x * sh.tiles_y;
    const int64_t marches = std::max<int64_t>(1, slots / tiles);
    int zc = (int)((planes + marches - 1) / marches);
    if (c->spmv_zchunk_stencil > 0) zc = c->spmv_zchunk_stencil;
    sh.zchunk = std::max(depth, zc);
    sh.wgs = (int)(((planes + sh.zchunk - 1) / sh.zchunk) * tiles);
    return sh;
}

inline ProductPlan plan_product(const Ctx *c, const Mesh *m, const Csr *a, int64_t r0, int64_t r1, bool pcg_like, int depth = 0) {
    ProductPlan P;
    if (!(c->spmv_sym && m->sym_w && a->uvals_valid && a->uvals)) return P;
    if (r1 < 0) r1 = m->nv;
    if (r0 < 0 || r0 > r1 || r1 > m->nv) return P;
    P.wgs = P.nblk = (int)((r1 - r0 + 63) / 64);
    P.form = KC_SYM_ROWS;
    if (m->sym_nx <= 0) return P;
    const int64_t plane = (int64_t)m->sym_nx * m->sym_ny;
    const int nx = m->sym_nx, ny = m->sym_ny, nz = (int)(m->nv / plane);
    P.z0 = (int)(r0 / plane); P.z1 = (int)(r1 / plane);
    const int wy = c->spmv_variant <= 1 ? 8 : 4;
    P.tiles_x = (nx + 63) / 64; P.tiles_y = (ny + wy - 1) / wy;
    const int64_t tile_planes = (int64_t)P.tiles_x * P.tiles_y * (P.z1 - P.z0);
    int chunks = 0;
    if (pcg_like && r0 % plane == 0 && r1 % plane == 0 && c->spmv_zchunk > 0 && plane * 64 >= c->spmv_grid_min_plane_bytes) {
        P.zchunk = (int)std::min<int64_t>(c->spmv_zchunk, tile_planes * (wy / 4) / (4 * (int64_t)c->num_cu));
        if (c->spmv_zchunk_force > 0) P.zchunk = c->spmv_zchunk_force;
        chunks = (P.zchunk >= 3 || c->spmv_zchunk_force > 0) ? (P.z1 - P.z0 + P.zchunk - 1) / P.zchunk : 0;
    }
    const int64_t gg = (int64_t)chunks * P.tiles_x * P.tiles_y;
    P.form = KC_DIA_ROWS;
    if (!(gg > 0 && gg < ((int64_t)1 << 30))) return P;
    const int wgs = (int)gg;
    bool coded = c->spmv_variant == 0 && c->spmv_classes && a->cls_count > 0;
    int wgs_c = wgs, zchunk_c = P.zchunk;
    if (coded && c->spmv_zchunk_force <= 0) {
        zchunk_c = (int)std::min<int64_t>(c->spmv_zchunk_coded, (tile_planes + c->num_cu / 2) / (int64_t)c->num_cu);
        zchunk_c = zchunk_c >= 9 ? std::max(12, (zchunk_c + 3) / 6 * 6) : std::max(3, zchunk_c / 3 * 3);
        const int64_t per_slot2 = (tile_planes + c->num_cu) / (2 * (int64_t)c->num_cu);
        if (c->spmv_zchunk_coded2 > 0 && per_slot2 >= 8)
            zchunk_c = (int)std::min<int64_t>(c->spmv_zchunk_coded2, per_slot2 >= 12 ? (per_slot2 + 5) / 6 * 6 : (per_slot2 + 2) / 3 * 3);
        wgs_c = (P.z1 - P.z0 + zchunk_c - 1) / zchunk_c * P.tiles_x * P.tiles_y;
    }
    coded = coded && zchunk_c <= DIAC_MAXCHUNK;
    const bool st_lower = P.z0 == 0 ? a->st_z0 == 0 : (P.z0 - 1 >= a->st_z0 || (P.z0 == a->st_z0 && a->st_g_lo));
    const bool st_upper = P.z1 == nz ? a->st_z1 == nz : (P.z1 + 1 <= a->st_z1 || (P.z1 == a->st_z1 && a->st_g_hi));
    if (coded && c->spmv_stencil && a->st_ok && (c->spmv_zchunk_force <= 0 || c->spmv_zchunk_stencil > 0) && st_lower && st_upper &&
        plane < ((int64_t)1 << 26)) {
        P.form = KC_STENCIL_MARCH;
        P.depth = depth > 0 ? depth : c->stencil_depth > 0 ? c->stencil_depth : 3;
        const StencilShape sh = stencil_shape(c, nx, ny, P.z1 - P.z0, P.depth);
        P.rows_per_thread = (sh.rows_per_thread == 2 && P.depth != 6) ? 2 : 4;
        P.tiles_y = sh.tiles_y; P.zchunk = sh.zchunk; P.wgs = sh.wgs;
    } else if (coded) {
        P.form = KC_DIAC_MARCH;
        P.zchunk = zchunk_c; P.wgs = wgs_c;
        P.six = zchunk_c >= 12 && zchunk_c % 6 == 0 && c->spmv_fetch_depth != 3;
    } else {
        P.form = KC_DIA_MARCH;
        P.wgs = wgs;
        if (c->spmv_variant == 0 && c->dia_march3 && (int64_t)64 * a->uvals_stride < ((int64_t)1 << 31) && plane < ((int64_t)1 << 27)) P.variant = MARCH_3;
        else P.variant = c->spmv_variant == 0 ? MARCH_2 : wy == 8 ? MARCH_WY8 : MARCH_WY4;
    }
    return P;
}
// ... 3 lines not shown
```

### pgdrome_amd/csrc/pgd_spmv.hip

```cpp
#include <chrono>
#include <cstring>

#include "pgd_internal.h"
#include "pgd_dia_march.h"
#include "pgd_product_plan.h"

#include <algorithm>
#include <type_traits>

namespace pgd {

constexpr int SPMV_CAP = 4096;
constexpr int SPMV_VROUNDS = 8;
constexpr int SPMV_CROUNDS = 4;
constexpr int MAXY = 8;

struct SpmvArgs {
    const int *row_ptr, *cols;
    const double *vals, *x, *w;
    double *y, *partials;
    const int *flags;
    int row_begin, row_end;
};

// ... 1781 lines not shown
    for (int k = 0; k < ((tab[(size_t)best * 16] >> 4) & 15); ++k) d.push_back(tab[(size_t)best * 16 + 8 + k]);
    std::sort(d.begin(), d.end());
    m->sym_nx = m->sym_ny = 0;
    if (d.size() == 7 && d[0] == 1 && d[2] == d[1] + 1 && d[4] == d[3] + 1 && d[5] == d[3] + d[1] && d[6] == d[5] + 1 &&
        d[3] % d[1] == 0 && m->nv % d[3] == 0 && d[1] >= 2) {
        m->sym_nx = d[1];
        m->sym_ny = d[3] / d[1];
    }
    if (m->sym_nx > 0) {
        const int nzg = (int)(m->nv / ((int64_t)m->sym_nx * m->sym_ny));
        int *vf = nullptr;
        PGD_TRY(dev_alloc(c, &p, 8 * sizeof(int))); vf = (int *)p;
        PGD_HIP(c, hipMemsetAsync(vf, 0, 8 * sizeof(int), st));
        k_dia_verify<<<(int)((m->nv + TPB - 1) / TPB), TPB, 0, st>>>(m->row_ptr, m->cols, m->nv, m->sym_nx, m->sym_ny, nzg, vf);
        int bad = 1;
        PGD_HIP(c, hipMemcpyAsync(&bad, vf, sizeof bad, hipMemcpyDeviceToHost, st));
        PGD_HIP(c, hipStreamSynchronize(st));
        (void)hipFree(vf);
        PGD_LAUNCH_CHECK(c);
        if (bad) m->sym_nx = m->sym_ny = 0;
    }
    return PGD_OK;
}

template <int W>
__global__ __launch_bounds__(TPB) void k_sym_scale(double *__restrict__ uvals, int64_t stride, const uint16_t *__restrict__ pids,
                                                   const int *__restrict__ tab, const double *__restrict__ sc, int64_t n) {
    const int64_t i = (int64_t)blockIdx.x * TPB + threadIdx.x;
    if (i >= n) return;
    const int *t = tab + (int)pids[i] * 16;
    const int ulen = t[0] & 15;
    const double si = sc[i];
#pragma unroll
    for (int s = 0; s < W; ++s)
        if (s < ulen) uvals[(int64_t)s * stride + i] *= si * sc[i + (s > 0 ? t[s] : 0)];
}

int sym_scale(Ctx *c, const Mesh *m, Csr *a, const double *sc) {
    if (!(a->uvals && a->uvals_valid) || a->uvals_scaled) return fail(c, PGD_ERR_INVALID, "sym_scale: no unscaled symmetric copy");
    a->drop_classes();
    const int g = (int)((m->nv + TPB - 1) / TPB);
    if (m->sym_nx > 0) k_dia_scale<<<g, TPB, 0, c->stream>>>(a->uvals, a->uvals_stride, sc, m->nv, m->sym_nx, m->sym_ny, c->spmv_unit_diag);
    else if (m->sym_w == 4) k_sym_scale<4><<<g, TPB, 0, c->stream>>>(a->uvals, a->uvals_stride, m->pids, m->sym_tab, sc, m->nv);
    else k_sym_scale<8><<<g, TPB, 0, c->stream>>>(a->uvals, a->uvals_stride, m->pids, m->sym_tab, sc, m->nv);
    PGD_LAUNCH_CHECK(c);
    a->uvals_scaled = true;
    a->uvals_unit = m->sym_nx > 0 && c->spmv_unit_diag;
    return PGD_OK;
}

int ensure_sym(Ctx *c, const Mesh *m, Csr *a, bool *usable) {
    *usable = false;
    if (!c->spmv_sym || m->sym_w == 0) return PGD_OK;
    if (a->uvals_valid && !a->uvals_scaled) { *usable = a->uvals != nullptr; return PGD_OK; }
    a->uvals_scaled = false;
    a->drop_classes();
    a->uvals_valid = true;
    const int64_t stride = m->nv;
    if (a->uvals && a->uvals_stride != stride) { dev_release(c, a->uvals, a->uvals_bytes); a->uvals = nullptr; }
    if (!a->uvals) {
        void *p;
        a->uvals_bytes = (size_t)m->sym_w * (size_t)stride * sizeof(double);
        PGD_TRY(dev_alloc(c, &p, a->uvals_bytes));
        a->uvals = (double *)p;
        a->uvals_stride = stride;
    }
    PGD_TRY(ensure_vals(c, m, a));
    a->cls_tried = false;
    PGD_HIP(c, hipMemsetAsync(c->flags + 4, 0, 4 * sizeof(int), c->stream));
    const int g = (int)((m->nv + TPB - 1) / TPB);
    if (m->sym_nx > 0) k_csr_to_dia<<<g, TPB, 0, c->stream>>>(m->row_ptr, m->cols, a->vals, m->nv, m->sym_nx, m->sym_ny, stride, a->uvals, c->flags + 4);
    else if (m->sym_w == 4) k_csr_to_sym<4><<<g, TPB, 0, c->stream>>>(m->row_ptr, a->vals, m->pids, m->sym_tab, m->nv, stride, a->uvals, c->flags + 4);
    else k_csr_to_sym<8><<<g, TPB, 0, c->stream>>>(m->row_ptr, a->vals, m->pids, m->sym_tab, m->nv, stride, a->uvals, c->flags + 4);
    int f[2] = {0, 0};
    PGD_HIP(c, hipMemcpyAsync(f, c->flags + 4, sizeof f, hipMemcpyDeviceToHost, c->stream));
    PGD_HIP(c, hipStreamSynchronize(c->stream));
    PGD_LAUNCH_CHECK(c);
    if (f[1] != 0) {
        dev_release(c, a->uvals, a->uvals_bytes);
        a->uvals = nullptr;
        return PGD_OK;
    }
    *usable = true;
    return PGD_OK;
}

constexpr int DIA_MAXT = 8;
struct CombineDiaArgs {
    const double *in[DIA_MAXT];
    double coef[DIA_MAXT];
    int n;
};

__global__ __launch_bounds__(TPB) void k_combine_dia(CombineDiaArgs A, double *__restrict__ out, int64_t stride,
                                                     const uint8_t *__restrict__ mask, double *__restrict__ dinv, int64_t nv,
                                                     int nx, int ny) {
    const int64_t i = (int64_t)blockIdx.x * TPB + threadIdx.x;
    if (i >= nv) return;
    const int64_t P = (int64_t)nx * ny;
    const bool bi = mask && mask[i];
#pragma unroll
    for (int s = 0; s < 8; ++s) {
        double v = 0.0;
#pragma unroll
        for (int t = 0; t < DIA_MAXT; ++t)
            if (t < A.n) v = fma(A.coef[t], A.in[t][(int64_t)s * stride + i], v);
// ... 134 lines not shown
    });
    c->kcount[KC_DIAC_MARCH] += 1;
    if (timed) PGD_TRY(prof_end(c, m, k.r1 - k.r0, 17.0));
    PGD_LAUNCH_CHECK(c);
    return PGD_OK;
}

static int launch_product_dia(Ctx *c, const Mesh *m, const Csr *a, const ProductPlan &P, const ProductCall &k) {
    DiaArgs D;
    D.uvals = a->uvals; D.x = k.x; D.w = k.w; D.y = k.y; D.partials = c->partials + c->partials_off; D.flags = k.flags; D.n = a->uvals_stride;
    D.nx = m->sym_nx; D.ny = m->sym_ny; D.nz = (int)(m->nv / ((int64_t)m->sym_nx * m->sym_ny));
    D.row_begin = (int)k.r0; D.row_end = (int)k.r1;
    D.nblk1 = -1; D.row_begin2 = D.row_end2 = 0;
    D.z0 = P.z0; D.z1 = P.z1; D.tiles_x = P.tiles_x; D.tiles_y = P.tiles_y; D.zchunk = P.zchunk;
    D.unit_diag = (a->uvals_scaled && a->uvals_unit) ? 1 : 0;
    D.qq = k.qq;
    bool timed = false;
    PGD_TRY(prof_begin(c, k.dot, k.store, &timed));
    with_product_kind(k.dot, k.store, false, [&](auto DT, auto S, auto) {
        if (P.form == KC_DIA_ROWS) k_spmv_dia_rows<DT.value, S.value><<<P.nblk, 64, 0, c->stream>>>(D);
        else if (P.variant == MARCH_3) k_spmv_dia_march3<DT.value, S.value><<<P.wgs, 256, 0, c->stream>>>(D);
        else if (P.variant == MARCH_2) k_spmv_dia_march2<DT.value, S.value><<<P.wgs, 256, 0, c->stream>>>(D);
        else if (P.variant == MARCH_WY8) k_spmv_dia_march<DT.value, S.value, 8><<<P.wgs, 64 * 8, 0, c->stream>>>(D);
        else k_spmv_dia_march<DT.value, S.value, 4><<<P.wgs, 64 * 4, 0, c->stream>>>(D);
    });
    c->kcount[P.form] += 1;
    if (timed) PGD_TRY(prof_end(c, m, k.r1 - k.r0, 8.0 * (D.unit_diag ? 7 : 8) + 16));
    PGD_LAUNCH_CHECK(c);
    return PGD_OK;
}

static int launch_product_sym(Ctx *c, const Mesh *m, const Csr *a, const ProductPlan &P, const ProductCall &k) {
    SymArgs A;
    A.uvals = a->uvals; A.x = k.x; A.w = k.w; A.y = k.y; A.partials = c->partials + c->partials_off; A.flags = k.flags;
    A.tab = m->sym_tab; A.pids = m->pids; A.n = a->uvals_stride; A.row_begin = (int)k.r0; A.row_end = (int)k.r1;
    A.qq = k.qq;
    bool timed = false;
    PGD_TRY(prof_begin(c, k.dot, k.store, &timed));
    with_product_kind(k.dot, k.store, false, [&](auto D, auto S, auto) {
        if (m->sym_w == 4) k_spmv_sym<D.value, S.value, 4><<<P.nblk, 64, 0, c->stream>>>(A);
        else k_spmv_sym<D.value, S.value, 8><<<P.nblk, 64, 0, c->stream>>>(A);
    });
    c->kcount[KC_SYM_ROWS] += 1;
    if (timed) PGD_TRY(prof_end(c, m, k.r1 - k.r0, 8.0 * m->sym_w + 18));
    PGD_LAUNCH_CHECK(c);
    return PGD_OK;
}

int launch_spmv_op(Ctx *c, const Mesh *m, const Csr *a, const double *x, double *y, const double *w, int64_t r0,
                   int64_t r1, bool dot, bool store, const int *flags, int *nparts_out) {
    auto not_virtual = [&](bool ok) -> int {
        return a->st_virtual && !ok ? fail(c, PGD_ERR_INVALID, "spmv: the operator is held as a scaled stencil; this launch cannot take that form") : PGD_OK;
    };
    if (!(c->spmv_sym && m->sym_w && a->uvals_valid && a->uvals)) {
        PGD_TRY(not_virtual(false));
        PGD_TRY(ensure_vals(c, m, const_cast<Csr *>(a)));
        if (c->spmv_p2_lattice && !a->immutable && r0 == 0 && (r1 < 0 || r1 == m->nv) && p2lat_degree2(c, m)) {
            bool done = false;
            PGD_TRY(launch_spmv_p2lat(c, m, const_cast<Csr *>(a), x, y, w, dot, store, flags, nparts_out, &done));
            if (done) return PGD_OK;
        }
        if (c->spmv_block_dia && m->ncomp > 1 && !a->immutable && r0 == 0 && (r1 < 0 || r1 == m->nv)) {
            bool done = false;
            PGD_TRY(launch_spmv_bdia(c, m, const_cast<Csr *>(a), x, y, w, dot, store, flags, nparts_out, &done));
            if (done) return PGD_OK;
        }
        return launch_spmv(c, m, a->vals, x, y, w, r0, r1, dot, store, flags, nparts_out);
    }
    if (c->spmv_block_dia && m->ncomp > 1 && !a->immutable && r0 == 0 && (r1 < 0 || r1 == m->nv) && a->bdia_seen != a->version) {
        Csr *o = const_cast<Csr *>(a);
        o->bdia_seen = a->version;
        o->bdia_ok = false;
        c->bdia_fallbacks += 1;
    }
    if (c->spmv_p2_lattice && !a->immutable && r0 == 0 && (r1 < 0 || r1 == m->nv) && a->p2lat_seen != a->version && p2lat_degree2(c, m)) {
        Csr *o = const_cast<Csr *>(a);
        o->p2lat_seen = a->version;
        o->p2lat_ok = false;
        c->p2lat_fallbacks += 1;
    }
    if (r1 < 0) r1 = m->nv;
    if (r0 < 0 || r0 > r1 || r1 > m->nv) return fail(c, PGD_ERR_INVALID, "spmv: bad row range");
    const ProductPlan P = plan_product(c, m, a, r0, r1, !dot || w == x);
    if (nparts_out) *nparts_out = P.wgs;
    if (P.nblk == 0) return PGD_OK;
    const ProductCall k = {x, y, w, r0, r1, dot, store, flags, (dot && c->spmv_qq) ? 1 : 0};
    if (dot) PGD_TRY(ensure_partials(c, std::max<int64_t>(c->partials_off + 2 * (int64_t)std::max(P.nblk, P.wgs), 4 * MAX_VEC_BLOCKS)));
    PGD_TRY(not_virtual(P.form == KC_STENCIL_MARCH));
    switch (P.form) {
    case KC_STENCIL_MARCH: return launch_product_stencil(c, m, a, P, k);
    case KC_DIAC_MARCH: return launch_product_diac(c, m, a, P, k);
    case KC_DIA_MARCH:
    case KC_DIA_ROWS: return launch_product_dia(c, m, a, P, k);
    default: return launch_product_sym(c, m, a, P, k);
    }
}

static ProductPlan plan_stencil_update(const Ctx *c, const Mesh *m, const Csr *a) { return plan_product(c, m, a, 0, m->nv, true, 3); }

int stencil_update_blocks(const Ctx *c, const Mesh *m, const Csr *a) { return plan_stencil_update(c, m, a).wgs; }

int launch_stencil_update(Ctx *c, const Mesh *m, const Csr *a, const double *p_in, double *p_out, double *x, double *r, const double *s,
                          double *pairs, int lag, double s_free, const StencilFold *fold) {
    const ProductPlan P = plan_stencil_update(c, m, a);
    if (P.form != KC_STENCIL_MARCH || !c->flags || p_in == p_out || (fold && (fold->vec_in == pairs || !fold->prod || !fold->vec_in)))
        return fail(c, PGD_ERR_INVALID, "stencil update: the operator's products do not run in the stencil march over the whole grid");
    StencilArgs F;
// ... 159 lines not shown
    D.qq = (dot && c->spmv_qq) ? 1 : 0;
    if (dot) PGD_TRY(ensure_partials(c, std::max<int64_t>(c->partials_off + (D.qq ? 2 : 1) * (int64_t)(n1 + n2), 4 * MAX_VEC_BLOCKS)));
    D.uvals = a->uvals; D.x = x; D.w = w; D.y = y; D.partials = c->partials + c->partials_off; D.flags = flags; D.n = a->uvals_stride;
    D.nx = m->sym_nx; D.ny = m->sym_ny; D.nz = (int)(m->nv / plane);
    D.row_begin = (int)r0a; D.row_end = (int)r1a; D.nblk1 = n1; D.row_begin2 = (int)r0b; D.row_end2 = (int)r1b;
    D.z0 = D.z1 = D.zchunk = D.tiles_x = D.tiles_y = 0;
    D.unit_diag = (a->uvals_scaled && a->uvals_unit) ? 1 : 0;
    if (dot) k_spmv_dia_rows<true, true><<<n1 + n2, 64, 0, c->stream>>>(D);
    else k_spmv_dia_rows<false, true><<<n1 + n2, 64, 0, c->stream>>>(D);
    c->kcount[KC_DIA_ROWS] += 1;
    PGD_LAUNCH_CHECK(c);
    if (nparts_out) *nparts_out = n1 + n2;
    *done = true;
    return PGD_OK;
}

int launch_spmv_multi(Ctx *c, const Mesh *m, const double *vals, const double *x, const double *const *ys,
                      int ny, int64_t r0, int64_t r1, double *out_host) {
    if (r1 < 0) r1 = m->nv;
    if (r0 < 0 || r0 > r1 || r1 > m->nv) return fail(c, PGD_ERR_INVALID, "bilinear_many: bad row range");
    const int nblk = (int)((r1 - r0 + TPB - 1) / TPB);
    for (int first = 0; first < ny; first += MAXY) {
        const int cnt = (ny - first < MAXY) ? ny - first : MAXY;
        if (nblk == 0) { for (int k = 0; k < cnt; ++k) out_host[first + k] = 0.0; continue; }
        PGD_TRY(ensure_partials(c, (int64_t)nblk * MAXY > 4 * MAX_VEC_BLOCKS ? (int64_t)nblk * MAXY : 4 * MAX_VEC_BLOCKS));
        SpmvMultiArgs A;
        A.row_ptr = m->row_ptr; A.cols = m->cols; A.vals = vals; A.x = x; A.partials = c->partials;
        A.row_begin = (int)r0; A.row_end = (int)r1; A.ny = cnt;
        for (int k = 0; k < MAXY; ++k) A.ys[k] = ys[first + (k < cnt ? k : 0)];
        k_spmv_multi<<<nblk, TPB, 0, c->stream>>>(A);
        c->kcount[KC_MULTI] += 1;
        PGD_LAUNCH_CHECK(c);
        PGD_TRY(reduce_partials(c, c->partials, nblk, cnt, S_TMP, -1, 0, 0));
        PGD_HIP(c, hipMemcpyAsync(out_host + first, c->slots + S_TMP, cnt * sizeof(double), hipMemcpyDeviceToHost, c->stream));
        PGD_HIP(c, hipStreamSynchronize(c->stream));
    }
    return PGD_OK;
}

}

using namespace pgd;

extern "C" {

#if defined(PGD_STENCIL_TIMING) || defined(PGD_STENCIL_WHATIF)
int pgd_debug_read_partials(pgd_handle h, double *out, int first, int count) {
    PGD_CTX(c, h);
    PGD_HIP(c, hipMemcpyAsync(out, c->partials + first, (size_t)count * sizeof(double), hipMemcpyDeviceToHost, c->stream));
    PGD_HIP(c, hipStreamSynchronize(c->stream));
    return PGD_OK;
}
#endif

int pgd_classify_counts(pgd_handle h, int64_t *full, int64_t *cached) {
    PGD_CTX(c, h);
    if (full) *full = c->cls_full;
    if (cached) *cached = c->cls_fast;
    return PGD_OK;
}

int pgd_tune(pgd_handle h, int knob, int64_t value) {
    PGD_CTX(c, h);
    if (knob == PGD_TUNE_SPMV_ROWS && (value == 64 || value == 128 || value == 256)) { c->spmv_rows = (int)value; return PGD_OK; }
    if (knob == PGD_TUNE_SPMV_DICT && value >= 0 && value <= 2) { c->spmv_dict = (int)value; return PGD_OK; }
    if (knob == PGD_TUNE_SPMV_SYM && value >= 0 && value <= 1) { c->spmv_sym = (int)value; return PGD_OK; }
    if (knob == PGD_TUNE_SPMV_GRID_MIN_BYTES && value >= 0) { c->spmv_grid_min_plane_bytes = value; return PGD_OK; }
    if (knob == PGD_TUNE_SPMV_ZCHUNK_FORCE && value >= 0 && value <= 65536) { c->spmv_zchunk_force = (int)value; return PGD_OK; }
    if (knob == PGD_TUNE_PCG_FOLD_REDUCE && value >= 0 && value <= 1) { c->pcg_fold_reduce = (int)value; return PGD_OK; }
    if (knob == PGD_TUNE_PCG_SCALED && value >= 0 && value <= 1) { c->pcg_scaled = (int)value; return PGD_OK; }
    if (knob == PGD_TUNE_SPMV_ZCHUNK && value >= 0 && value <= 65536) { c->spmv_zchunk = (int)value; return PGD_OK; }
    if (knob == PGD_TUNE_PCG_SINGLE_SYNC && value >= 0 && value <= 1) { c->pcg_single_sync = (int)value; return PGD_OK; }
    if (knob == PGD_TUNE_UNIT_DIAG && value >= 0 && value <= 1) { c->spmv_unit_diag = (int)value; return PGD_OK; }
    if (knob == PGD_TUNE_PCG_DEFER_X && value >= 0 && value <= 1) { c->pcg_defer_x = (int)value; return PGD_OK; }
    if (knob == PGD_TUNE_FAULT_ITERATION && value >= -1 && value <= (1 << 30)) { c->fault_iteration = (int)value; return PGD_OK; }
    if (knob == PGD_TUNE_CLS_CACHE && value >= 0 && value <= 1) { c->cls_cache_on = (int)value; return PGD_OK; }
    if (knob == PGD_TUNE_SPMV_STENCIL && value >= 0 && value <= 1) { c->spmv_stencil = (int)value; return PGD_OK; }
    if (knob == PGD_TUNE_SPMV_ZCHUNK_STENCIL && value >= 0 && value <= 1024) { c->spmv_zchunk_stencil = (int)value; return PGD_OK; }
    if (knob == PGD_TUNE_STENCIL_DEPTH && (value == 0 || value == 3 || value == 6)) { c->stencil_depth = (int)value; return PGD_OK; }
    if (knob == PGD_TUNE_STENCIL_WG_PER_CU && value >= 1 && value <= 8) { c->stencil_wg_per_cu = (int)value; return PGD_OK; }
    if (knob == PGD_TUNE_FAULT_STAGE && value >= 0 && value <= 4) { c->fault_stage = (int)value; return PGD_OK; }
    if (knob == PGD_TUNE_FAULT_STALL_MS && value >= 0 && value <= 20000) { c->fault_stall_ms = (int)value; return PGD_OK; }
    if (knob == PGD_TUNE_COMBINE_DIA && value >= 0 && value <= 1) { c->spmv_combine_dia = (int)value; return PGD_OK; }
    if (knob == PGD_TUNE_SPMV_VARIANT && value >= 0 && value <= 2) { c->spmv_variant = (int)value; return PGD_OK; }
    if (knob == PGD_TUNE_SPMV_ROW_CLASSES && value >= 0 && value <= 1) { c->spmv_classes = (int)value; return PGD_OK; }
    if (knob == PGD_TUNE_ASM_LATTICE && value >= 0 && value <= 3) { c->asm_lattice = (int)value; return PGD_OK; }
    if (knob == PGD_TUNE_PCG_LAG_X && value >= 0 && value <= 1) { c->pcg_lag_x = (int)value; return PGD_OK; }
    if (knob == PGD_TUNE_PCG_STREAM_HINTS && value >= 0 && value <= 1) { c->pcg_stream_hints = (int)value; return PGD_OK; }
    if (knob == PGD_TUNE_PCG_SMALL_SINGLE_SYNC && value >= 0 && value <= 1) { c->pcg_small_ss = (int)value; return PGD_OK; }
    if (knob == PGD_TUNE_PCG_SMALL_ROWS && value >= 0) { c->pcg_small_ss_rows = value; return PGD_OK; }
    if (knob == PGD_TUNE_SPMV_FETCH_DEPTH && (value == 3 || value == 6)) { c->spmv_fetch_depth = (int)value; return PGD_OK; }
    if (knob == PGD_TUNE_SPMV_ZCHUNK_CODED2 && value >= 0 && value <= 1020) { c->spmv_zchunk_coded2 = (int)value / 6 * 6; return PGD_OK; }
    if (knob == PGD_TUNE_PCG_PIPELINE && value >= 0 && value <= 1) { c->pcg_pipeline = (int)value; return PGD_OK; }
    if (knob == PGD_TUNE_PCG_EXACT_PHASE && value >= 0 && value <= 1) { c->pcg_exact_phase = (int)value; return PGD_OK; }
    if (knob == PGD_TUNE_PCG_FOLD_FINISH && value >= 0 && value <= 1) { c->pcg_fold_finish = (int)value; return PGD_OK; }
    if (knob == PGD_TUNE_ATOM_FAST && value >= 0 && value <= 1) { c->atom_fast = (int)value; return PGD_OK; }
    if (knob == PGD_TUNE_LAZY_CSR && value >= 0 && value <= 1) { c->lazy_csr = (int)value; return PGD_OK; }
    if (knob == PGD_TUNE_SPMV_ZCHUNK_CODED && value >= 3 && value <= 1024) { c->spmv_zchunk_coded = (int)value; return PGD_OK; }
    if (knob == PGD_TUNE_PCG_PRECOND && value >= 0 && value <= 4) { c->pcg_precond = (int)value; return PGD_OK; }
    if (knob == PGD_TUNE_PCG_DERIVE_SCALED && value >= 0 && value <= 1) { c->pcg_derive_scaled = (int)value; return PGD_OK; }
    if (knob == PGD_TUNE_COMM_SELF_PERIODIC && value >= 0 && value <= 1) { c->comm.self_periodic = value != 0; return PGD_OK; }
    if (knob == PGD_TUNE_HALO_OVERLAP_MIN_ROWS && value >= 0) { c->comm.overlap_min_rows = value; return PGD_OK; }
    if (knob == PGD_TUNE_SHARD_ONE_MARCH && value >= 0 && value <= 1) { c->shard_one_march = (int)value; return PGD_OK; }
    if (knob == PGD_TUNE_DIA_MARCH3 && value >= 0 && value <= 1) { c->dia_march3 = (int)value; return PGD_OK; }
    if (knob == PGD_TUNE_STENCIL_ROWS && (value == 0 || value == 2 || value == 4)) { c->stencil_rows = (int)value; return PGD_OK; }
    if (knob == PGD_TUNE_PUSH_IN_UPDATE && (value == 0 || value == 1)) { c->push_in_update = (int)value; return PGD_OK; }
    if (knob == PGD_TUNE_MG_CHUNK && value >= 2 && value <= 16 && value % 2 == 0) { c->mg_chunk = (int)value; return PGD_OK; }
    if (knob == PGD_TUNE_MG_MARCH_MIN && value >= 0 && value <= 1 << 20) { c->mg_march_min = (int)value; return PGD_OK; }
    if (knob == PGD_TUNE_EVAL_VARIANT && value >= 0 && value <= 1) { c->eval_variant = (int)value; return PGD_OK; }
    if (knob == PGD_TUNE_EVAL_GRID_MAX && value >= 0 && value <= 1 << 20) { c->eval_grid_max = (int)value; return PGD_OK; }
    if (knob == PGD_TUNE_EVAL_SAMPLE_CHUNK && value >= 0 && value <= 1024) { c->eval_chunk = (int)value; return PGD_OK; }
    if (knob == PGD_TUNE_PCG_RECOMPUTE_Q && value >= 0 && value <= 1) { c->pcg_recompute_q = (int)value; return PGD_OK; }
    if (knob == PGD_TUNE_PCG_FOLD_MARCH && value >= 0 && value <= 1) { c->pcg_fold_march = (int)value; return PGD_OK; }
    if (knob == PGD_TUNE_PCG_SCALAR_S && value >= 0 && value <= 1) { c->pcg_scalar_s = (int)value; return PGD_OK; }
    if (knob == PGD_TUNE_PCG_FUSED_MARCH && value >= 0 && value <= 1) { c->pcg_fused_march = (int)value; return PGD_OK; }
    if (knob == PGD_TUNE_BLOCK_STORAGE && value >= 0 && value <= 2) { c->block_storage = (int)value; return PGD_OK; }
    if (knob == PGD_TUNE_SPMV_BLOCK_DIA && value >= 0 && value <= 1) { c->spmv_block_dia = (int)value; return PGD_OK; }
    if (knob == PGD_TUNE_SPMV_P2_LATTICE && value >= 0 && value <= 1) { c->spmv_p2_lattice = (int)value; return PGD_OK; }
    return fail(c, PGD_ERR_INVALID, "tune: unknown knob %d or value out of range", knob);
}

int pgd_spmv(pgd_handle h, pgd_handle ah, pgd_handle xh, pgd_handle yh, int64_t r0, int64_t r1) {
    PGD_CTX(c, h);
    Csr *a = get_csr(c, ah);
    Mesh *m = a ? get_mesh(c, a->mesh) : nullptr;
    Vec *x = get_vec(c, xh), *y = get_vec(c, yh);
    if (!a || !m || !x || !y || x->n != m->nv || y->n != m->nv || x == y)
        return fail(c, PGD_ERR_INVALID, "spmv: invalid handles, size mismatch or x aliases y");
    if (atom_fast_form(c, m, a, r0, r1)) return launch_spmv_op(c, m, a, x->d, y->d, nullptr, r0, r1, false, true, nullptr, nullptr);
    if (c->spmv_sym && c->atom_fast && m->sym_nx > 0 && !a->immutable && a->uvals && a->uvals_valid && !a->uvals_scaled && !a->st_virtual) {
        const int64_t plane = (int64_t)m->sym_nx * m->sym_ny;
        const int64_t q0 = r0 < 0 ? 0 : r0, q1 = r1 < 0 ? m->nv : r1;
        if (q0 >= 0 && q1 <= m->nv && q0 <= q1 && q0 % plane == 0 && q1 % plane == 0)
            return launch_spmv_op(c, m, a, x->d, y->d, nullptr, q0, q1, false, true, nullptr, nullptr);
    }
    if (c->spmv_block_dia && m->ncomp > 1 && !a->immutable) return launch_spmv_op(c, m, a, x->d, y->d, nullptr, r0, r1, false, true, nullptr, nullptr);
    if (c->spmv_p2_lattice && !a->immutable && p2lat_degree2(c, m)) return launch_spmv_op(c, m, a, x->d, y->d, nullptr, r0, r1, false, true, nullptr, nullptr);
    PGD_TRY(ensure_vals(c, m, a));
    return launch_spmv(c, m, a->vals, x->d, y->d, nullptr, r0, r1, false, true, nullptr, nullptr);
}

int pgd_bilinear(pgd_handle h, pgd_handle ah, pgd_handle xh, pgd_handle yh, int64_t r0, int64_t r1, double *out) {
    PGD_CTX(c, h);
    Csr *a = get_csr(c, ah);
    Mesh *m = a ? get_mesh(c, a->mesh) : nullptr;
    Vec *x = get_vec(c, xh), *y = get_vec(c, yh);
    if (!a || !m || !x || !y || !out || x->n != m->nv || y->n != m->nv)
        return fail(c, PGD_ERR_INVALID, "bilinear: invalid handles or size mismatch");
    int nparts = 0;
    PGD_TRY(ensure_vals(c, m, a));
    PGD_TRY(launch_spmv(c, m, a->vals, y->d, nullptr, x->d, r0, r1, true, false, nullptr, &nparts));
    if (nparts == 0) { *out = 0.0; return PGD_OK; }
    PGD_TRY(reduce_partials(c, c->partials, nparts, 1, S_TMP, -1, 0, 0));
    PGD_HIP(c, hipMemcpyAsync(out, c->slots + S_TMP, sizeof(double), hipMemcpyDeviceToHost, c->stream));
    PGD_HIP(c, hipStreamSynchronize(c->stream));
    return PGD_OK;
}

int pgd_bilinear_many(pgd_handle h, pgd_handle ah, pgd_handle xh, const pgd_handle *yhs, int ny, int64_t r0,
                      int64_t r1, double *out) {
    PGD_CTX(c, h);
    Csr *a = get_csr(c, ah);
    Mesh *m = a ? get_mesh(c, a->mesh) : nullptr;
    Vec *x = get_vec(c, xh);
    if (!a || !m || !x || !out || ny < 0 || (ny > 0 && !yhs) || x->n != m->nv)
        return fail(c, PGD_ERR_INVALID, "bilinear_many: invalid handles or size mismatch");
    std::vector<const double *> ys((size_t)ny);
    for (int k = 0; k < ny; ++k) {
        Vec *y = get_vec(c, yhs[k]);
        if (!y || y->n != m->nv) return fail(c, PGD_ERR_INVALID, "bilinear_many: invalid vector %d", k);
        ys[k] = y->d;
    }
    if (ny == 0) return PGD_OK;
    PGD_TRY(ensure_vals(c, m, a));
    return launch_spmv_multi(c, m, a->vals, x->d, ys.data(), ny, r0, r1, out);
}

int pgd_op_symmetrize(pgd_handle h, pgd_handle ah, int *used) {
    PGD_CTX(c, h);
    Csr *a = get_csr(c, ah);
    Mesh *m = a ? get_mesh(c, a->mesh) : nullptr;
    if (!a || !m) return fail(c, PGD_ERR_INVALID, "op_symmetrize: invalid handle");
    bool usable = false;
// ... 102 lines not shown
        Vec *v = get_vec(c, yhs[j]);
        if (!v || v->n != x0->n) return fail(c, PGD_ERR_INVALID, "vec_multidot_pair: invalid vector %d", j);
        y[(size_t)j] = v->d;
    }
    for (int j = 0; j < 2 * k; ++j) out[j] = 0.0;
    if (hi == lo) return PGD_OK;
    PGD_TRY(ensure_work(c, 6, 2 * (int64_t)MAX_VEC_BLOCKS > 512 ? 2 * (int64_t)MAX_VEC_BLOCKS : 512));
    double *res = c->work[6];
    const int g = grid_for(hi - lo);
    PGD_TRY(ensure_partials(c, std::max<int64_t>((int64_t)g * 2 * PAIR_MAXV, 4 * MAX_VEC_BLOCKS)));
    int off = 0;
    for (int j0 = 0; j0 < k; j0 += PAIR_MAXV) {
        const int nv = std::min(PAIR_MAXV, k - j0);
        MultiDot2Args A;
        A.w0 = x0->d; A.w1 = x1->d; A.nv = nv; A.lo = lo; A.hi = hi; A.partials = c->partials;
        for (int q = 0; q < PAIR_MAXV; ++q) A.v[q] = y[(size_t)(j0 + std::min(q, nv - 1))];
        k_multidot2<<<g, TPB, 0, c->stream>>>(A);
        PGD_LAUNCH_CHECK(c);
        PGD_TRY(reduce_partials_to(c, c->partials, g, 2 * nv, res + off));
        off += 2 * nv;
    }
    std::vector<double> host((size_t)off);
    PGD_HIP(c, hipMemcpyAsync(host.data(), res, (size_t)off * sizeof(double), hipMemcpyDeviceToHost, c->stream));
    PGD_HIP(c, hipStreamSynchronize(c->stream));
    off = 0;
    for (int j0 = 0; j0 < k; j0 += PAIR_MAXV) {
        const int nv = std::min(PAIR_MAXV, k - j0);
        for (int q = 0; q < nv; ++q) { out[j0 + q] = host[(size_t)(off + q)]; out[k + j0 + q] = host[(size_t)(off + nv + q)]; }
        off += 2 * nv;
    }
    return PGD_OK;
}

int pgd_start_gram(pgd_handle h, pgd_handle ah, const pgd_handle *vhs, int k, pgd_handle bh, int64_t r0, int64_t r1,
                   double *out) {
    PGD_CTX(c, h);
    Csr *a = get_csr(c, ah);
    Mesh *m = a ? get_mesh(c, a->mesh) : nullptr;
    Vec *b = get_vec(c, bh);
    if (!a || !m || !b || !vhs || !out || k < 1 || k > GRAM_MAXV || b->n != m->nv)
        return fail(c, PGD_ERR_INVALID, "start_gram: invalid handles or more than %d vectors", GRAM_MAXV);
    if (r1 < 0) r1 = m->nv;
    if (r0 < 0 || r0 > r1 || r1 > m->nv) return fail(c, PGD_ERR_INVALID, "start_gram: bad row range");
    const double *v[GRAM_MAXV];
    for (int j = 0; j < k; ++j) {
        Vec *x = get_vec(c, vhs[j]);
        if (!x || x->n != m->nv) return fail(c, PGD_ERR_INVALID, "start_gram: invalid vector %d", j);
        v[j] = x->d;
    }
    for (int q = 0; q < k * k + k; ++q) out[q] = 0.0;
    c->gram_op = 0; c->gram_k = 0; c->gram_n = 0;
    if (r1 == r0) return PGD_OK;
    bool sym = false;
    PGD_TRY(ensure_sym(c, m, a, &sym));
    PGD_TRY(ensure_work(c, 3, m->nv));
    PGD_TRY(ensure_work(c, 6, 2 * (int64_t)MAX_VEC_BLOCKS > 256 ? 2 * (int64_t)MAX_VEC_BLOCKS : 256));
    double *w = c->work[3], *res = c->work[6];
    const bool dbg_t = getenv("PGD_DEBUG_PCG") != nullptr;
    auto dbg_now = [] { return std::chrono::duration<double>(std::chrono::steady_clock::now().time_since_epoch()).count(); };
    const double dbg_t0 = dbg_now();
    if (k >= 2) PGD_TRY(dia_classify(c, m, a));
    if (dbg_t) fprintf(stderr, "[start_gram] k %d classify %.2f ms (cls %d stencil %d)\n", k, 1e3 * (dbg_now() - dbg_t0), a->cls_count, (int)a->st_ok);
    if (k <= GRAM9) {
        const size_t need = (size_t)k * (size_t)m->nv * sizeof(double);
        if (c->gram_w_bytes < need) {
            if (c->gram_w) dev_release(c, c->gram_w, c->gram_w_bytes);
            c->gram_w = nullptr; c->gram_w_bytes = 0;
            void *pw;
            PGD_TRY(dev_alloc(c, &pw, need));
            c->gram_w = (double *)pw; c->gram_w_bytes = need;
        }
        Gram9Args A;
        for (int j = 0; j < k; ++j) {
            double *wj = c->gram_w + (size_t)j * m->nv;
            PGD_TRY(launch_spmv_op(c, m, a, v[j], wj, nullptr, r0, r1, false, true, nullptr, nullptr));
        }
        for (int t = 0; t < GRAM9; ++t) { A.v[t] = v[t < k ? t : 0]; A.w[t] = c->gram_w + (size_t)(t < k ? t : 0) * m->nv; }
        A.b = b->d; A.k = k; A.lo = r0; A.hi = r1;
        const int nv = k * (k + 1) / 2 + k;
        const int gg = grid_for(r1 - r0, TPB, 1024);
        PGD_TRY(ensure_partials(c, std::max<int64_t>((int64_t)gg * nv, 4 * MAX_VEC_BLOCKS)));
        A.partials = c->partials;
        k_gram9<<<gg, TPB, 0, c->stream>>>(A);
        PGD_LAUNCH_CHECK(c);
        PGD_TRY(reduce_partials_to(c, c->partials, gg, nv, res));
        std::vector<double> host((size_t)nv);
        PGD_HIP(c, hipMemcpyAsync(host.data(), res, (size_t)nv * sizeof(double), hipMemcpyDeviceToHost, c->stream));
        PGD_HIP(c, hipStreamSynchronize(c->stream));
        for (int j = 0; j < k; ++j) {
            for (int i = 0; i <= j; ++i) out[i * k + j] = out[j * k + i] = host[(size_t)(j * (j + 1) / 2 + i)];
            out[k * k + j] = host[(size_t)(k * (k + 1) / 2 + j)];
        }
        if (r0 == 0 && r1 == m->nv) { c->gram_op = ah; c->gram_k = k; c->gram_n = m->nv; }
        return PGD_OK;
    }
    const int g = grid_for(r1 - r0);
    int off = 0;
    for (int j = 0; j < k; ++j) {
        PGD_TRY(launch_spmv_op(c, m, a, v[j], w, nullptr, r0, r1, false, true, nullptr, nullptr));
        PGD_TRY(ensure_partials(c, (int64_t)g * (GRAM_MAXV + 1) > 4 * MAX_VEC_BLOCKS ? (int64_t)g * (GRAM_MAXV + 1) : 4 * MAX_VEC_BLOCKS));
        MultiDotArgs A;
        A.w = w; A.b = b->d; A.nv = j + 1; A.lo = r0; A.hi = r1; A.partials = c->partials;
        for (int q = 0; q < GRAM_MAXV; ++q) A.v[q] = v[q <= j ? q : j];
        k_multidot<<<g, TPB, 0, c->stream>>>(A);
        PGD_LAUNCH_CHECK(c);
        PGD_TRY(reduce_partials_to(c, c->partials, g, j + 2, res + off));
        off += j + 2;
    }
    std::vector<double> host((size_t)off);
    PGD_HIP(c, hipMemcpyAsync(host.data(), res, (size_t)off * sizeof(double), hipMemcpyDeviceToHost, c->stream));
    PGD_HIP(c, hipStreamSynchronize(c->stream));
    off = 0;
    for (int j = 0; j < k; ++j) {
        for (int i = 0; i <= j; ++i) out[i * k + j] = out[j * k + i] = host[(size_t)off + i];
// ... 8 lines not shown
```

Measured before the change: 19.60.

## Derive combined operator class tables from cached atom tables instead of combining diagonals

When a combined operator is a linear mix of immutable atoms whose row classes match a cached classification, the combined stencil coefficients and class table are computed on the host from per-atom tuples. The row codes are copied from the cache, which skips the full diagonal combine, classification and diagonal-inverse passes over the 256^3 grid. The operator's value slots are released, and they are rebuilt lazily only if a reader needs the explicit form. This adds a validation step (a kernel plus small device-to-host copies) when a cache entry qualifies, and a lot of new state and fallback paths that may have correctness edge cases.

```diff
diff --git a/include/pgd_amd.h b/include/pgd_amd.h
--- a/include/pgd_amd.h
+++ b/include/pgd_amd.h
@@ -215,6 +215,7 @@
                            double *sample_stats, pgd_handle env_min, pgd_handle env_max, pgd_handle exceed, pgd_handle fields);
 
 enum {
+    PGD_TUNE_OP_TABLES = 60,
     PGD_TUNE_SPMV_P2_LATTICE = 59,
     PGD_TUNE_SPMV_BLOCK_DIA = 58,
     PGD_TUNE_PCG_FUSED_MARCH = 57,
@@ -283,6 +284,10 @@
 int pgd_pcg_recompute_counts(pgd_handle ctx, int64_t *updates);
 int pgd_pcg_fused_counts(pgd_handle ctx, int64_t *marches);
 int pgd_classify_counts(pgd_handle ctx, int64_t *full, int64_t *cached);
+int pgd_op_tables_counts(pgd_handle ctx, int64_t *derived, int64_t *at_combine, int64_t *later, int64_t *later_by_reader, int n_readers,
+                         int *last_reader);
+int pgd_op_form(pgd_handle ctx, pgd_handle op, int *derived, int64_t *slot_bytes, int *classes, int *st_ok, int *st_ident, double *st_c);
+int pgd_op_codes(pgd_handle ctx, pgd_handle op, uint8_t *codes, int64_t n);
 int pgd_mg_counts(pgd_handle ctx, int64_t *solves, int64_t *fallbacks);
 int pgd_vmg_counts(pgd_handle ctx, int64_t *solves, int64_t *fallbacks, int64_t *levels);
 int pgd_vmg_times(pgd_handle ctx, double *setup_ms, int64_t *march_passes);
diff --git a/pgdrome_amd/_lib.py b/pgdrome_amd/_lib.py
--- a/pgdrome_amd/_lib.py
+++ b/pgdrome_amd/_lib.py
@@ -139,6 +139,9 @@
     "pgd_pcg_recompute_counts": (C.c_int, [H, PI64]),
     "pgd_pcg_fused_counts": (C.c_int, [H, PI64]),
     "pgd_classify_counts": (C.c_int, [H, PI64, PI64]),
+    "pgd_op_tables_counts": (C.c_int, [H, PI64, PI64, PI64, PI64, C.c_int, C.POINTER(C.c_int)]),
+    "pgd_op_form": (C.c_int, [H, H, C.POINTER(C.c_int), PI64, C.POINTER(C.c_int), C.POINTER(C.c_int), C.POINTER(C.c_int), PD]),
+    "pgd_op_codes": (C.c_int, [H, H, PU8, I64]),
     "pgd_mg_counts": (C.c_int, [H, PI64, PI64]),
     "pgd_vmg_counts": (C.c_int, [H, PI64, PI64, PI64]),
     "pgd_vmg_times": (C.c_int, [H, C.POINTER(C.c_double), PI64]),
@@ -865,6 +868,29 @@
         self._ck(self.lib.pgd_classify_counts(self.h, C.byref(full), C.byref(cached)))
         return {"full": full.value, "cached": cached.value}
 
+    OP_TABLES_READERS = ("symmetric_copy", "classify", "dinv", "product", "solve", "combine_input")
+
+    def op_tables_counts(self):
+        d, a, l, last = I64(), I64(), I64(), C.c_int(-1)
+        by = (I64 * len(self.OP_TABLES_READERS))()
+        self._ck(self.lib.pgd_op_tables_counts(self.h, C.byref(d), C.byref(a), C.byref(l), by, len(by), C.byref(last)))
+        names = self.OP_TABLES_READERS
+        return {"derived": d.value, "at_combine": a.value, "later": l.value,
+                "later_by_reader": {names[i]: int(by[i]) for i in range(len(names))},
+                "last_reader": names[last.value] if 0 <= last.value < len(names) else None}
+
+    def op_form(self, op):
+        der, cls, ok, ident, nbytes = C.c_int(), C.c_int(), C.c_int(), C.c_int(), I64()
+        st = (C.c_double * 8)()
+        self._ck(self.lib.pgd_op_form(self.h, op, C.byref(der), C.byref(nbytes), C.byref(cls), C.byref(ok), C.byref(ident), st))
+        return {"derived": bool(der.value), "slot_bytes": nbytes.value, "classes": cls.value, "stencil": bool(ok.value),
+                "ident": ident.value, "st_c": np.array(list(st), dtype=np.float64)}
+
+    def op_codes(self, op, n):
+        out = np.empty(int(n), dtype=np.uint8)
+        self._ck(self.lib.pgd_op_codes(self.h, op, out.ctypes.data_as(PU8), int(n)))
+        return out
+
     def precondition(self, multigrid):
         self.tune(40, 1 if multigrid else 0)
         return self.mg_stats()["solves"]
diff --git a/pgdrome_amd/csrc/pgd_classify.hip b/pgdrome_amd/csrc/pgd_classify.hip
--- a/pgdrome_amd/csrc/pgd_classify.hip
+++ b/pgdrome_amd/csrc/pgd_classify.hip
@@ -2,12 +2,16 @@
 #include <cstdarg>
 #include <cstdlib>
 #include <cstring>
+#include <vector>
 
 #include "pgd_internal.h"
+#include "pgd_op_tables.h"
 
 namespace pgd {
 
 constexpr int CLS_SLOTS = 1024;
+constexpr int DERIVE_MAXT = 8;
+constexpr int DERIVE_MAXCLS = 31;
 
 struct StencilInfo { int ok, ident, base, split; double c[8]; int zm0, zm1, g_lo, g_hi; };
 
@@ -342,6 +346,8 @@
 }
 
 static size_t plane_flag_bytes(int nzp) { return ((size_t)nzp * sizeof(int) + 63) / 64 * 64; }
+static int cls_alloc(Ctx *c, const Mesh *m, Csr *a, int nzp);
+static int qualify_entry(const ClsJob &J, Mesh::ClsCache &E);
 
 constexpr size_t CLS_CACHE_MAX = 4, CLS_REPS_BYTES = 256 * sizeof(int);
 
@@ -376,14 +382,7 @@
     void *p;
     if (!c->cls_scratch) { PGD_TRY(dev_alloc(c, &p, sizeof(ClsScratch) + sizeof(StencilInfo) + 2 * 65536 * sizeof(int))); c->cls_scratch = p; }
     const int nzp = (int)(m->nv / plane);
-    if (!a->cls) {
-        const size_t table_b = (size_t)(CLS_MAX + 1) * 8 * sizeof(double), same_b = plane_flag_bytes(nzp);
-        a->cls_bytes = (size_t)m->nv + table_b + same_b + 64;
-        PGD_TRY(dev_alloc(c, &p, a->cls_bytes));
-        a->cls_table = (double *)p;
-        a->cls_same = (int *)((uint8_t *)p + table_b);
-        a->cls = (uint8_t *)a->cls_same + same_b;
-    }
+    PGD_TRY(cls_alloc(c, m, a, nzp));
     J.c = c; J.m = m; J.a = a;
     J.plane = plane; J.nzp = nzp;
     J.g = (int)((m->nv + TPB - 1) / TPB);
@@ -454,7 +453,7 @@
         a->cls_count = E.ncls;
         if (E.st_ok) adopt_stencil(a, J.si, J.z_lo, J.z_hi);
         *hit = true;
-        return PGD_OK;
+        return qualify_entry(J, E);
     }
     return PGD_OK;
 }
@@ -521,18 +520,18 @@
     return okc;
 }
 
-static void remember(const ClsJob &J) {
+static bool remember(const ClsJob &J) {
     const Csr *a = J.a;
     const int ncls = a->cls_count;
     Mesh::ClsCache E;
     E.sig = a->bc_sig; E.scaled = J.scaled_key; E.z_lo = J.z_lo; E.z_hi = J.z_hi; E.ncls = ncls;
-    if (!cls_cache_alloc(E, J.m->nv, J.nzp)) { (void)hipGetLastError(); return; }
+    if (!cls_cache_alloc(E, J.m->nv, J.nzp)) { (void)hipGetLastError(); return false; }
     double tab[(CLS_MAX + 1) * 8];
     int reps_rng[256];
     if (!cls_cache_fill(J, E, reps_rng, tab)) {
         E.release();
         (void)hipGetLastError();
-        return;
+        return false;
     }
     E.st_ok = a->st_ok; E.ident = a->st_ident; E.base = J.try_stencil ? J.si.base : -1; E.zm0 = a->st_zm0; E.zm1 = a->st_zm1;
     for (int k = 0; k < 256; ++k) E.in_range[k] = (k < ncls && reps_rng[k] >= 0 && reps_rng[k] < 0x7f000000) ? 1 : 0;
@@ -541,11 +540,157 @@
         if (k < ncls) for (int s2 = 1; s2 < 8; ++s2) if (tab[k * 8 + cls_pos(s2)] == 0.0) b |= (uint8_t)(1u << s2);
         E.zero_pat[k] = b;
     }
+    E.base_full = E.base >= 0 && E.zero_pat[E.base] == 0;
     if (E.base >= 0) for (int k = 0; k < ncls; ++k) E.zero_pat[k] &= (uint8_t)~E.zero_pat[E.base];
     cls_cache_insert(J.m, E);
+    return true;
+}
+
+struct AtomCodes { const uint8_t *cls[DERIVE_MAXT]; int ref[DERIVE_MAXT]; int n; };
+
+__global__ __launch_bounds__(TPB) void k_atoms_one_class(const uint8_t *__restrict__ codes, int ident, AtomCodes A, int64_t nv, int *__restrict__ bad) {
+    const int64_t i = (int64_t)blockIdx.x * TPB + threadIdx.x;
+    if (i >= nv || (int)codes[i] == ident) return;
+    bool good = true;
+#pragma unroll
+    for (int t = 0; t < DERIVE_MAXT; ++t)
+        if (t < A.n) good = good && (int)A.cls[t][i] == A.ref[t];
+    if (!good) *bad = 1;
+}
+
+struct TableRows { double v[(DERIVE_MAXCLS + 1) * 8]; int rows; };
+
+__global__ void k_cls_table_set(TableRows T, double *__restrict__ table) {
+    const int k = blockIdx.x * blockDim.x + threadIdx.x;
+    if (k < T.rows * 8) table[k] = T.v[k];
+}
+
+static int cls_alloc(Ctx *c, const Mesh *m, Csr *a, int nzp) {
+    if (a->cls) return PGD_OK;
+    void *p;
+    const size_t table_b = (size_t)(CLS_MAX + 1) * 8 * sizeof(double), same_b = plane_flag_bytes(nzp);
+    a->cls_bytes = (size_t)m->nv + table_b + same_b + 64;
+    PGD_TRY(dev_alloc(c, &p, a->cls_bytes));
+    a->cls_table = (double *)p;
+    a->cls_same = (int *)((uint8_t *)p + table_b);
+    a->cls = (uint8_t *)a->cls_same + same_b;
+    return PGD_OK;
+}
+
+static bool derive_grid_ok(const Ctx *c, const Mesh *m) {
+    if (!(c->op_tables && c->spmv_sym && c->spmv_combine_dia && c->spmv_classes && c->spmv_stencil && c->cls_cache_on && c->lazy_csr)) return false;
+    if (m->sym_nx <= 0 || m->nv >= ((int64_t)1 << 31)) return false;
+    const int64_t plane = (int64_t)m->sym_nx * m->sym_ny;
+    const int64_t nzp = m->nv / plane;
+    return nzp >= 3 && nzp <= 65536 && nzp * plane == m->nv && plane * 64 >= c->spmv_grid_min_plane_bytes;
+}
+
+static bool derive_atoms(Ctx *c, const Csr *o, Csr **atoms) {
+    const size_t n = o->rec_atoms.size();
+    if (n < 1 || n > (size_t)DERIVE_MAXT) return false;
+    for (size_t t = 0; t < n; ++t) {
+        Csr *a = get_csr(c, o->rec_atoms[t]);
+        if (!a || a->serial != o->rec_serials[t] || a->version != o->rec_versions[t] || !a->immutable || a->derived) return false;
+        if (!(a->uvals && a->uvals_valid) || a->uvals_scaled || !(a->cls && a->cls_count > 0)) return false;
+        atoms[t] = a;
+    }
+    return true;
+}
+
+static bool entry_has_key(const Mesh::ClsCache &E, const Csr *o) {
+    return E.d_ok && E.d_bc_epoch == o->bc_epoch && E.d_serials == o->rec_serials && E.d_versions == o->rec_versions;
+}
+
+static int qualify_entry(const ClsJob &J, Mesh::ClsCache &E) {
+    Ctx *c = J.c; const Mesh *m = J.m; Csr *a = J.a;
+    if (!a->derive_cand || a->bc_epoch == 0 || !derive_grid_ok(c, m) || entry_has_key(E, a)) return PGD_OK;
+    if (!(a->st_ok && E.st_ok && E.base_full && E.base >= 0 && E.ident >= 0 && E.ncls <= DERIVE_MAXCLS && E.codes)) return PGD_OK;
+    if (J.z_lo != 0 || J.z_hi != J.nzp || J.scaled_key != 4 || a->st_g_lo || a->st_g_hi) return PGD_OK;
+    Csr *atoms[DERIVE_MAXT];
+    if (!derive_atoms(c, a, atoms)) return PGD_OK;
+    const int n = (int)a->rec_atoms.size();
+    hipStream_t st = c->stream;
+    int reps[256];
+    PGD_HIP(c, hipMemcpyAsync(reps, E.reps, sizeof reps, hipMemcpyDeviceToHost, st));
+    PGD_HIP(c, hipStreamSynchronize(st));
+    const int64_t r0 = reps[E.base];
+    if (r0 < 0 || r0 >= m->nv) return PGD_OK;
+    std::vector<double> tuples((size_t)8 * n);
+    uint8_t ref[DERIVE_MAXT];
+    for (int t = 0; t < n; ++t) {
+        for (int s = 0; s < 8; ++s)
+            PGD_HIP(c, hipMemcpyAsync(&tuples[(size_t)8 * t + s], atoms[t]->uvals + (int64_t)s * atoms[t]->uvals_stride + r0, sizeof(double), hipMemcpyDeviceToHost, st));
+        PGD_HIP(c, hipMemcpyAsync(&ref[t], atoms[t]->cls + r0, 1, hipMemcpyDeviceToHost, st));
+    }
+    int *bad_dev = J.S->info + 2, bad = 1;
+    PGD_HIP(c, hipMemsetAsync(bad_dev, 0, sizeof(int), st));
+    PGD_HIP(c, hipStreamSynchronize(st));
+    AtomCodes A;
+    A.n = n;
+    for (int t = 0; t < DERIVE_MAXT; ++t) { A.cls[t] = atoms[t < n ? t : 0]->cls; A.ref[t] = ref[t < n ? t : 0]; }
+    k_atoms_one_class<<<J.g, TPB, 0, st>>>(E.codes, E.ident, A, m->nv, bad_dev);
+    PGD_HIP(c, hipMemcpyAsync(&bad, bad_dev, sizeof(int), hipMemcpyDeviceToHost, st));
+    PGD_HIP(c, hipStreamSynchronize(st));
+    PGD_LAUNCH_CHECK(c);
+    double cc[8];
+    table_combine(tuples.data(), a->rec_coefs.data(), n, cc);
+    bool same = bad == 0;
+    for (int s = 0; s < 8; ++s) same = same && std::memcmp(&cc[s], &a->st_c[s], sizeof(double)) == 0;
+    cls_debug(J.dbg_cls, "[dia_classify] table form: base row %lld, atoms one class on the free rows %d, combine reproduces the stencil %d\n",
+              (long long)r0, bad == 0 ? 1 : 0, same ? 1 : 0);
+    if (!same) return PGD_OK;
+    E.d_ok = true;
+    E.d_bc_epoch = a->bc_epoch;
+    E.d_serials = a->rec_serials;
+    E.d_versions = a->rec_versions;
+    E.d_tuples = tuples;
+    return PGD_OK;
+}
+
+int op_derive(Ctx *c, const Mesh *m, Csr *o, Csr *const *atoms_in, const double *coefs, int n, bool *derived) {
+    *derived = false;
+    (void)atoms_in;
+    if (!o->derive_cand || o->bc_epoch == 0 || !derive_grid_ok(c, m)) return PGD_OK;
+    Csr *atoms[DERIVE_MAXT];
+    if (!derive_atoms(c, o, atoms)) return PGD_OK;
+    const int nzp = (int)(m->nv / ((int64_t)m->sym_nx * m->sym_ny));
+    for (size_t e = 0; e < m->cls_cache.size(); ++e) {
+        Mesh::ClsCache &E = m->cls_cache[e];
+        if (E.sig != o->bc_sig || E.scaled != 4 || E.z_lo != 0 || E.z_hi != nzp || !E.codes || !E.st_ok || !entry_has_key(E, o)) continue;
+        double cc[8];
+        table_combine(E.d_tuples.data(), coefs, n, cc);
+        for (int s = 0; s < 8; ++s) if (!std::isfinite(cc[s])) return PGD_OK;
+        TableRows T;
+        T.rows = E.ncls + 1;
+        for (int k = 0; k <= E.ncls; ++k)
+            for (int s = 0; s < 8; ++s) {
+                double v = 0.0;
+                if (k == E.ident) v = s == 0 ? 1.0 : 0.0;
+                else if (k < E.ncls) v = (s > 0 && ((E.zero_pat[k] >> s) & 1)) ? 0.0 : cc[s];
+                T.v[k * 8 + cls_pos(s)] = v;
+            }
+        PGD_TRY(cls_alloc(c, m, o, nzp));
+        hipStream_t st = c->stream;
+        PGD_HIP(c, hipMemcpyAsync(o->cls, E.codes, (size_t)m->nv, hipMemcpyDeviceToDevice, st));
+        PGD_HIP(c, hipMemcpyAsync(o->cls_same, E.same, (size_t)nzp * sizeof(int), hipMemcpyDeviceToDevice, st));
+        k_cls_table_set<<<(T.rows * 8 + 255) / 256, 256, 0, st>>>(T, o->cls_table);
+        PGD_LAUNCH_CHECK(c);
+        StencilInfo si;
+        si.ok = 1; si.ident = E.ident; si.base = E.base; si.split = 0; si.zm0 = E.zm0; si.zm1 = E.zm1; si.g_lo = si.g_hi = 0;
+        for (int s = 0; s < 8; ++s) si.c[s] = cc[s];
+        cls_cache_touch(m, E);
+        o->cls_count = E.ncls;
+        adopt_stencil(o, si, 0, nzp);
+        o->derived = true;
+        c->opt_derived += 1;
+        *derived = true;
+        return PGD_OK;
+    }
+    return PGD_OK;
 }
 
 int dia_classify(Ctx *c, const Mesh *m, Csr *a, int zrange_lo, int zrange_hi) {
+    PGD_TRY(ensure_slots(c, m, a, OPT_READER_CLASSIFY));
     a->drop_classes();
     ClsJob J;
     bool go = false, hit = false;
@@ -556,7 +701,7 @@
     PGD_TRY(classify_full(J));
     if (a->cls_count <= 0) return PGD_OK;
     if (J.try_stencil && J.si.ok) adopt_stencil(a, J.si, J.z_lo, J.z_hi);
-    if (c->cls_cache_on) remember(J);
+    if (c->cls_cache_on && remember(J)) PGD_TRY(qualify_entry(J, m->cls_cache.back()));
     return PGD_OK;
 }
 
diff --git a/pgdrome_amd/csrc/pgd_internal.h b/pgdrome_amd/csrc/pgd_internal.h
--- a/pgdrome_amd/csrc/pgd_internal.h
+++ b/pgdrome_amd/csrc/pgd_internal.h
@@ -51,6 +51,9 @@
     size_t bytes = 0;
     ~Block() override { if (d) dev_release(ctx, d, bytes); }
 };
+
+enum { OPT_READER_SYM = 0, OPT_READER_CLASSIFY = 1, OPT_READER_DIAG = 2, OPT_READER_PRODUCT = 3, OPT_READER_PCG = 4, OPT_READER_COMBINE = 5,
+       OPT_READERS = 8 };
 
 struct Mesh : Obj {
     int gdim = 0, nvpc = 0;
@@ -82,11 +85,16 @@
         uint8_t zero_pat[256];
         uint8_t in_range[256];
         uint64_t used = 0;
+        bool base_full = false, d_ok = false;
+        uint64_t d_bc_epoch = 0;
+        std::vector<uint64_t> d_serials, d_versions;
+        std::vector<double> d_tuples;
         void release() { if (block) (void)hipFree(block); block = nullptr; codes = nullptr; same = reps = nullptr; }
     };
     mutable std::vector<ClsCache> cls_cache;
     mutable uint64_t cls_clock = 0;
     std::vector<int32_t> bc_host;
+    uint64_t bc_epoch = 0;
     int *bc_dev = nullptr;
     size_t bc_dev_bytes = 0;
     uint16_t *pids = nullptr;
@@ -129,6 +137,8 @@
     void drop_classes() { cls_count = 0; st_ok = false; st_g_lo = st_g_hi = false; }
     bool st_virtual = false;
     bool cls_tried = false;
+    bool derived = false, derive_cand = false;
+    uint64_t bc_epoch = 0;
     bool immutable = false;
     uint64_t version = 0;
     bool vals_pending = false;
@@ -285,6 +295,10 @@
     int mg_march_min = 64;
     int cls_cache_on = 1;
     int64_t cls_fast = 0, cls_full = 0;
+    int op_tables = 1;
+    int64_t opt_derived = 0, opt_at_combine = 0, opt_later = 0;
+    int64_t opt_later_by[OPT_READERS] = {0, 0, 0, 0, 0, 0, 0, 0};
+    int opt_last_reader = -1;
     int spmv_stencil = 1;
     int spmv_zchunk_stencil = 0;
     int stencil_depth = 0;
@@ -397,6 +411,8 @@
 int vec_sqrt(Ctx *c, double *v, int64_t n);
 int vec_div_mul(Ctx *c, double *x, const double *sc, int64_t n, int mul);
 int ensure_vals(Ctx *c, const Mesh *m, Csr *a);
+int ensure_slots(Ctx *c, const Mesh *m, Csr *a, int reader);
+int op_derive(Ctx *c, const Mesh *m, Csr *o, Csr *const *atoms, const double *coefs, int n, bool *derived);
 bool atom_fast_form(Ctx *c, const Mesh *m, Csr *a, int64_t r0, int64_t r1);
 constexpr int CLS_MAX = 255;
 __host__ __device__ constexpr int cls_pos(int s) {
diff --git a/pgdrome_amd/csrc/pgd_op_tables.h b/pgdrome_amd/csrc/pgd_op_tables.h
--- /dev/null
+++ b/pgdrome_amd/csrc/pgd_op_tables.h
@@ -0,0 +1,23 @@
+#pragma once
+
+#include <cmath>
+
+namespace pgd {
+
+inline void table_combine(const double *tuples, const double *coefs, int n, double out[8]) {
+    for (int s = 0; s < 8; ++s) {
+        double v = 0.0;
+        for (int t = 0; t < n; ++t) v = std::fma(coefs[t], tuples[8 * t + s], v);
+        out[s] = v;
+    }
+}
+
+inline void stencil_scaled(const double c[8], int unit, double out[10]) {
+    const double dinv = 1.0 / c[0], si = std::sqrt(dinv);
+    out[0] = unit ? 1.0 : c[0] * si * si;
+    for (int s = 1; s < 8; ++s) { double v = c[s]; v *= si * si; out[s] = v; }
+    out[8] = si;
+    out[9] = dinv;
+}
+
+}
diff --git a/pgdrome_amd/csrc/pgd_pcg.hip b/pgdrome_amd/csrc/pgd_pcg.hip
--- a/pgdrome_amd/csrc/pgd_pcg.hip
+++ b/pgdrome_amd/csrc/pgd_pcg.hip
@@ -1,4 +1,5 @@
 #include "pgd_internal.h"
+#include "pgd_op_tables.h"
 
 #include <cmath>
 
@@ -428,6 +429,20 @@
     out[0] = unit ? 1.0 : A.c[0] * si * si;
     for (int s = 1; s < 8; ++s) { double v = A.c[s]; v *= si * si; out[s] = v; }
     out[8] = si;
+}
+
+__global__ __launch_bounds__(TPB) void k_scale_in_codes(const uint8_t *__restrict__ cls, int ident, double s_free, double *__restrict__ s,
+                                                        double *__restrict__ x, int64_t n) {
+    for (int64_t i = (int64_t)blockIdx.x * TPB + threadIdx.x; i < n; i += (int64_t)gridDim.x * TPB) {
+        const double si = (int)cls[i] == ident ? 1.0 : s_free;
+        s[i] = si;
+        x[i] = x[i] / si;
+    }
+}
+
+__global__ void k_dmin_value(double dmax_inv, double *__restrict__ slots, int *__restrict__ flags) {
+    slots[S_DMIN] = dmax_inv > 0.0 ? 1.0 / dmax_inv : 0.0;
+    if (!(dmax_inv > 0.0) || !(dmax_inv < 1e300)) { flags[0] = 1; flags[2] = PGD_ERR_SINGULAR; }
 }
 
 __global__ void k_dmin_slot(const unsigned long long *__restrict__ dmax_bits, double *__restrict__ slots, int *__restrict__ flags) {
@@ -1023,7 +1038,35 @@
     return PGD_OK;
 }
 
+int ensure_slots(Ctx *c, const Mesh *m, Csr *o, int reader) {
+    if (!o->derived) return PGD_OK;
+    if (o->st_virtual) return fail(c, PGD_ERR_INVALID, "operator: held as a scaled stencil inside a solve; its slot arrays cannot be formed now");
+    const int n = (int)o->rec_atoms.size();
+    std::vector<Csr *> atoms((size_t)n);
+    for (int t = 0; t < n; ++t) {
+        Csr *a = get_csr(c, o->rec_atoms[(size_t)t]);
+        if (!a || a->serial != o->rec_serials[(size_t)t] || a->version != o->rec_versions[(size_t)t])
+            return fail(c, PGD_ERR_INVALID, "operator: its CSR values were left to the first reader and atom %d has been freed or rewritten since", t);
+        atoms[(size_t)t] = a;
+    }
+    const uint8_t *mask = nullptr;
+    if (o->rec_nbc > 0) {
+        PGD_TRY(ensure_mask(c, m->nv));
+        PGD_HIP(c, hipMemsetAsync(c->mask, 0, (size_t)m->nv, c->stream));
+        k_mask_set<<<grid_for(o->rec_nbc), TPB, 0, c->stream>>>(c->mask, o->rec_bc, o->rec_nbc);
+        mask = c->mask;
+    }
+    o->derived = false;
+    PGD_TRY(combine_dia(c, m, o, atoms.data(), o->rec_coefs.data(), n, mask));
+    c->opt_later += 1;
+    if (reader >= 0 && reader < OPT_READERS) c->opt_later_by[reader] += 1;
+    c->opt_last_reader = reader;
+    if (!(c->lazy_csr && o->uvals_valid)) PGD_TRY(ensure_vals(c, m, o));
+    return PGD_OK;
+}
+
 int csr_diag_inv(Ctx *c, const Mesh *m, Csr *a) {
+    PGD_TRY(ensure_slots(c, m, a, OPT_READER_DIAG));
     if (a->dinv_valid) return PGD_OK;
     if (!a->dinv) {
         void *p;
@@ -1337,20 +1380,34 @@
     return R.precond == PGD_PCG_PRECOND_MG ? mg_result(R.c) : R.precond == PGD_PCG_PRECOND_VMG ? vmg_result(R.c->vmg) : R.z;
 }
 
+static bool pcg_stencil_derivable(const Ctx *c, const Mesh *m, const Csr *o) {
+    if (!(c->pcg_derive_scaled && m->sym_nx > 0 && c->pcg_precond != 2 && o->cls_count > 0)) return false;
+    if (!(stencil_whole_grid(c, m, o) && o->st_ident >= 0 && o->st_c[0] > 0.0)) return false;
+    double out10[10];
+    stencil_scaled(o->st_c, c->spmv_unit_diag, out10);
+    for (double v : out10) if (!std::isfinite(v)) return false;
+    return true;
+}
+
 static int pcg_derive_stencil(PcgRun &R) {
     Ctx *c = R.c;
     Csr *o = R.o;
     if (!(c->pcg_derive_scaled && R.m->sym_nx > 0 && c->pcg_precond != 2)) return PGD_OK;
     if (o->cls_count <= 0) PGD_TRY(dia_classify(c, R.m, o));
     if (!(stencil_whole_grid(c, R.m, o) && o->st_ident >= 0 && o->st_c[0] > 0.0)) return PGD_OK;
-    PGD_TRY(ensure_work(c, 5, 4096));
-    StencilTuple in;
-    for (int s2 = 0; s2 < 8; ++s2) in.c[s2] = o->st_c[s2];
-    k_stencil_derive<<<1, 1, 0, c->stream>>>(in, c->spmv_unit_diag, c->work[5] + 16);
-    PGD_LAUNCH_CHECK(c);
-    double out9[9];
-    PGD_HIP(c, hipMemcpyAsync(out9, c->work[5] + 16, sizeof out9, hipMemcpyDeviceToHost, c->stream));
-    PGD_HIP(c, hipStreamSynchronize(c->stream));
+    double out9[10];
+    if (c->op_tables) {
+        stencil_scaled(o->st_c, c->spmv_unit_diag, out9);
+    } else {
+        PGD_TRY(ensure_work(c, 5, 4096));
+        StencilTuple in;
+        for (int s2 = 0; s2 < 8; ++s2) in.c[s2] = o->st_c[s2];
+        k_stencil_derive<<<1, 1, 0, c->stream>>>(in, c->spmv_unit_diag, c->work[5] + 16);
+        PGD_LAUNCH_CHECK(c);
+        PGD_HIP(c, hipMemcpyAsync(out9, c->work[5] + 16, 9 * sizeof(double), hipMemcpyDeviceToHost, c->stream));
+        PGD_HIP(c, hipStreamSynchronize(c->stream));
+        out9[9] = 0.0;
+    }
     for (double v : out9) if (!std::isfinite(v)) return PGD_OK;
     for (int s2 = 0; s2 < 8; ++s2) { R.st_saved[s2] = o->st_c[s2]; o->st_c[s2] = out9[s2]; }
     o->st_virtual = R.virt = true;
@@ -1361,14 +1418,24 @@
 static int pcg_setup_scaled(PcgRun &R) {
     Ctx *c = R.c;
     const int64_t n = R.n;
-    PGD_TRY(ensure_work(c, 5, 4096));
-    unsigned long long *bits = reinterpret_cast<unsigned long long *>(c->work[5]);
-    PGD_HIP(c, hipMemsetAsync(bits, 0, sizeof(unsigned long long), c->stream));
-    k_scale_in<<<grid_for(n), TPB, 0, c->stream>>>(R.o->dinv, R.sc, R.x, n, bits);
-    k_dmin_slot<<<1, 1, 0, c->stream>>>(bits, c->slots, c->flags);
-    PGD_LAUNCH_CHECK(c);
-    R.x_scaled = true;
-    PGD_TRY(pcg_derive_stencil(R));
+    if (R.o->derived) {
+        PGD_TRY(pcg_derive_stencil(R));
+        if (!R.virt) return fail(c, PGD_ERR_INVALID, "pcg_solve: an operator held as class tables did not give a scaled stencil");
+        const double dinv_free = 1.0 / R.st_saved[0];
+        k_scale_in_codes<<<grid_for(n), TPB, 0, c->stream>>>(R.o->cls, R.o->st_ident, R.s_free, R.sc, R.x, n);
+        k_dmin_value<<<1, 1, 0, c->stream>>>(fmax(1.0, dinv_free), c->slots, c->flags);
+        PGD_LAUNCH_CHECK(c);
+        R.x_scaled = true;
+    } else {
+        PGD_TRY(ensure_work(c, 5, 4096));
+        unsigned long long *bits = reinterpret_cast<unsigned long long *>(c->work[5]);
+        PGD_HIP(c, hipMemsetAsync(bits, 0, sizeof(unsigned long long), c->stream));
+        k_scale_in<<<grid_for(n), TPB, 0, c->stream>>>(R.o->dinv, R.sc, R.x, n, bits);
+        k_dmin_slot<<<1, 1, 0, c->stream>>>(bits, c->slots, c->flags);
+        PGD_LAUNCH_CHECK(c);
+        R.x_scaled = true;
+        PGD_TRY(pcg_derive_stencil(R));
+    }
     if (!R.virt) {
         PGD_TRY(sym_scale(c, R.m, R.o, R.sc));
         PGD_TRY(dia_classify(c, R.m, R.o));
@@ -1690,6 +1757,7 @@
         Csr *a = get_csr(c, atoms[t]);
         if (!a || a->mesh != mh) return fail(c, PGD_ERR_INVALID, "op_combine: atom %d is not on this mesh", t);
         if (*op && atoms[t] == *op) return fail(c, PGD_ERR_INVALID, "op_combine: output aliases an input");
+        PGD_TRY(ensure_slots(c, m, a, OPT_READER_COMBINE));
         atom_objs[t] = a;
     }
     const bool bc_known = nbc > 0 && m->bc_dev && m->bc_host.size() == (size_t)nbc &&
@@ -1711,6 +1779,7 @@
     o->dinv_valid = false;
     o->uvals_valid = false;
     o->vals_pending = false;
+    o->derived = false;
     o->version += 1;
     o->rec_atoms.assign(atoms, atoms + n);
     o->rec_coefs.assign(coefs, coefs + n);
@@ -1736,10 +1805,9 @@
             PGD_TRY(dev_alloc(c, &p, o->rec_bc_bytes));
             o->rec_bc = (int *)p;
         }
-        PGD_TRY(ensure_mask(c, m->nv));
-        PGD_HIP(c, hipMemsetAsync(c->mask, 0, (size_t)m->nv, c->stream));
         if (!bc_known) {
             m->bc_host.clear();
+            m->bc_epoch += 1;
             if (m->bc_dev && m->bc_dev_bytes < (size_t)nbc * sizeof(int)) { (void)hipFree(m->bc_dev); m->bc_dev = nullptr; }
             if (!m->bc_dev) {
                 void *p = nullptr;
@@ -1755,12 +1823,30 @@
         } else {
             PGD_HIP(c, hipMemcpyAsync(o->rec_bc, m->bc_dev, (size_t)nbc * sizeof(int), hipMemcpyDeviceToDevice, c->stream));
         }
-        k_mask_set<<<grid_for(nbc), TPB, 0, c->stream>>>(c->mask, o->rec_bc, nbc);
-        mask = c->mask;
     }
     o->vals_pending = true;
-    PGD_TRY(combine_dia(c, m, o, atom_objs.data(), coefs, n, mask));
-    if (!(c->lazy_csr && o->uvals_valid)) PGD_TRY(ensure_vals(c, m, o));
+    o->bc_epoch = (nbc > 0 && m->bc_host.size() == (size_t)nbc) ? m->bc_epoch : 0;
+    o->derive_cand = c->op_tables && o->bc_epoch != 0 && m->sym_nx > 0;
+    bool derived = false;
+    if (o->derive_cand) {
+        o->drop_classes();
+        o->cls_tried = false;
+        PGD_TRY(op_derive(c, m, o, atom_objs.data(), coefs, n, &derived));
+    }
+    if (derived) {
+        if (o->uvals) { dev_release(c, o->uvals, o->uvals_bytes); o->uvals = nullptr; o->uvals_bytes = 0; }
+        if (o->dinv) { dev_release(c, o->dinv, o->dinv_bytes); o->dinv = nullptr; o->dinv_bytes = 0; }
+    } else {
+        if (nbc > 0) {
+            PGD_TRY(ensure_mask(c, m->nv));
+            PGD_HIP(c, hipMemsetAsync(c->mask, 0, (size_t)m->nv, c->stream));
+            k_mask_set<<<grid_for(nbc), TPB, 0, c->stream>>>(c->mask, o->rec_bc, nbc);
+            mask = c->mask;
+        }
+        PGD_TRY(combine_dia(c, m, o, atom_objs.data(), coefs, n, mask));
+        if (o->uvals_valid) c->opt_at_combine += 1;
+        if (!(c->lazy_csr && o->uvals_valid)) PGD_TRY(ensure_vals(c, m, o));
+    }
     if (nbc > 0 && !bc_known) PGD_HIP(c, hipStreamSynchronize(c->stream));
     return PGD_OK;
 }
@@ -1771,6 +1857,7 @@
     Mesh *m = o ? get_mesh(c, o->mesh) : nullptr;
     Vec *d = get_vec(c, dh);
     if (!o || !m || !d || d->n != m->nv) return fail(c, PGD_ERR_INVALID, "op_diag_inv: invalid handles");
+    PGD_TRY(ensure_slots(c, m, o, OPT_READER_DIAG));
     if (o->dinv_valid && o->dinv) {
         PGD_HIP(c, hipMemcpyAsync(d->d, o->dinv, (size_t)m->nv * sizeof(double), hipMemcpyDeviceToDevice, c->stream));
         return PGD_OK;
@@ -1794,9 +1881,12 @@
     const double dbg_t0 = host_now();
     ProfIterGuard prof_iter_guard{c};
     c->prof_pend.clear();
-    PGD_TRY(csr_diag_inv(c, m, o));
-    bool sym = false;
-    PGD_TRY(ensure_sym(c, m, o, &sym));
+    if (o->derived && !(c->spmv_sym && c->pcg_scaled && n >= 2 && pcg_stencil_derivable(c, m, o))) PGD_TRY(ensure_slots(c, m, o, OPT_READER_PCG));
+    bool sym = o->derived;
+    if (!o->derived) {
+        PGD_TRY(csr_diag_inv(c, m, o));
+        PGD_TRY(ensure_sym(c, m, o, &sym));
+    }
     for (int i = 0; i < 4; ++i) PGD_TRY(ensure_work(c, i, n));
     PGD_HIP(c, hipMemsetAsync(c->flags, 0, 8 * sizeof(int), c->stream));
     PcgRun R{c, m, o, b->d, x->d, n, c->work[0], c->work[1], c->work[2], c->work[3], c->work[1]};
diff --git a/pgdrome_amd/csrc/pgd_product_plan.h b/pgdrome_amd/csrc/pgd_product_plan.h
--- a/pgdrome_amd/csrc/pgd_product_plan.h
+++ b/pgdrome_amd/csrc/pgd_product_plan.h
@@ -42,7 +42,7 @@
 
 inline ProductPlan plan_product(const Ctx *c, const Mesh *m, const Csr *a, int64_t r0, int64_t r1, bool pcg_like, int depth = 0) {
     ProductPlan P;
-    if (!(c->spmv_sym && m->sym_w && a->uvals_valid && a->uvals)) return P;
+    if (!(c->spmv_sym && m->sym_w && ((a->uvals_valid && a->uvals) || a->derived))) return P;
     if (r1 < 0) r1 = m->nv;
     if (r0 < 0 || r0 > r1 || r1 > m->nv) return P;
     P.wgs = P.nblk = (int)((r1 - r0 + 63) / 64);
diff --git a/pgdrome_amd/csrc/pgd_spmv.hip b/pgdrome_amd/csrc/pgd_spmv.hip
--- a/pgdrome_amd/csrc/pgd_spmv.hip
+++ b/pgdrome_amd/csrc/pgd_spmv.hip
@@ -1857,6 +1857,7 @@
 int ensure_sym(Ctx *c, const Mesh *m, Csr *a, bool *usable) {
     *usable = false;
     if (!c->spmv_sym || m->sym_w == 0) return PGD_OK;
+    PGD_TRY(ensure_slots(c, m, a, OPT_READER_SYM));
     if (a->uvals_valid && !a->uvals_scaled) { *usable = a->uvals != nullptr; return PGD_OK; }
     a->uvals_scaled = false;
     a->drop_classes();
@@ -2097,7 +2098,15 @@
     auto not_virtual = [&](bool ok) -> int {
         return a->st_virtual && !ok ? fail(c, PGD_ERR_INVALID, "spmv: the operator is held as a scaled stencil; this launch cannot take that form") : PGD_OK;
     };
-    if (!(c->spmv_sym && m->sym_w && a->uvals_valid && a->uvals)) {
+    if (a->derived && c->spmv_sym && m->sym_w) {
+        const int64_t q1 = r1 < 0 ? m->nv : r1;
+        if (r0 < 0 || r0 > q1 || q1 > m->nv) return fail(c, PGD_ERR_INVALID, "spmv: bad row range");
+        if (plan_product(c, m, a, r0, q1, !dot || w == x).form != KC_STENCIL_MARCH) {
+            PGD_TRY(not_virtual(false));
+            PGD_TRY(ensure_slots(c, m, const_cast<Csr *>(a), OPT_READER_PRODUCT));
+        }
+    }
+    if (!(c->spmv_sym && m->sym_w && ((a->uvals_valid && a->uvals) || a->derived))) {
         PGD_TRY(not_virtual(false));
         PGD_TRY(ensure_vals(c, m, const_cast<Csr *>(a)));
         if (c->spmv_p2_lattice && !a->immutable && r0 == 0 && (r1 < 0 || r1 == m->nv) && p2lat_degree2(c, m)) {
@@ -2363,6 +2372,40 @@
     return PGD_OK;
 }
 #endif
+
+int pgd_op_tables_counts(pgd_handle h, int64_t *derived, int64_t *at_combine, int64_t *later, int64_t *later_by_reader, int n_readers,
+                         int *last_reader) {
+    PGD_CTX(c, h);
+    if (derived) *derived = c->opt_derived;
+    if (at_combine) *at_combine = c->opt_at_combine;
+    if (later) *later = c->opt_later;
+    if (later_by_reader) for (int r = 0; r < n_readers; ++r) later_by_reader[r] = r < OPT_READERS ? c->opt_later_by[r] : 0;
+    if (last_reader) *last_reader = c->opt_last_reader;
+    return PGD_OK;
+}
+
+int pgd_op_form(pgd_handle h, pgd_handle oh, int *derived, int64_t *slot_bytes, int *classes, int *st_ok, int *st_ident, double *st_c) {
+    PGD_CTX(c, h);
+    Csr *o = get_csr(c, oh);
+    if (!o) return fail(c, PGD_ERR_INVALID, "op_form: invalid handle");
+    if (derived) *derived = o->derived ? 1 : 0;
+    if (slot_bytes) *slot_bytes = (int64_t)((o->uvals ? o->uvals_bytes : 0) + (o->dinv ? o->dinv_bytes : 0));
+    if (classes) *classes = o->cls_count;
+    if (st_ok) *st_ok = (o->cls_count > 0 && o->st_ok) ? 1 : 0;
+    if (st_ident) *st_ident = o->st_ident;
+    if (st_c) for (int s = 0; s < 8; ++s) st_c[s] = o->st_c[s];
+    return PGD_OK;
+}
+
+int pgd_op_codes(pgd_handle h, pgd_handle oh, uint8_t *codes, int64_t n) {
+    PGD_CTX(c, h);
+    Csr *o = get_csr(c, oh);
+    Mesh *m = o ? get_mesh(c, o->mesh) : nullptr;
+    if (!o || !m || !codes || n != m->nv || !(o->cls && o->cls_count > 0)) return fail(c, PGD_ERR_INVALID, "op_codes: no row classes, or a size mismatch");
+    PGD_HIP(c, hipMemcpyAsync(codes, o->cls, (size_t)n, hipMemcpyDeviceToHost, c->stream));
+    PGD_HIP(c, hipStreamSynchronize(c->stream));
+    return PGD_OK;
+}
 
 int pgd_classify_counts(pgd_handle h, int64_t *full, int64_t *cached) {
     PGD_CTX(c, h);
@@ -2428,6 +2471,7 @@
     if (knob == PGD_TUNE_BLOCK_STORAGE && value >= 0 && value <= 2) { c->block_storage = (int)value; return PGD_OK; }
     if (knob == PGD_TUNE_SPMV_BLOCK_DIA && value >= 0 && value <= 1) { c->spmv_block_dia = (int)value; return PGD_OK; }
     if (knob == PGD_TUNE_SPMV_P2_LATTICE && value >= 0 && value <= 1) { c->spmv_p2_lattice = (int)value; return PGD_OK; }
+    if (knob == PGD_TUNE_OP_TABLES && value >= 0 && value <= 1) { c->op_tables = (int)value; return PGD_OK; }
     return fail(c, PGD_ERR_INVALID, "tune: unknown knob %d or value out of range", knob);
 }
 
@@ -2439,7 +2483,7 @@
     if (!a || !m || !x || !y || x->n != m->nv || y->n != m->nv || x == y)
         return fail(c, PGD_ERR_INVALID, "spmv: invalid handles, size mismatch or x aliases y");
     if (atom_fast_form(c, m, a, r0, r1)) return launch_spmv_op(c, m, a, x->d, y->d, nullptr, r0, r1, false, true, nullptr, nullptr);
-    if (c->spmv_sym && c->atom_fast && m->sym_nx > 0 && !a->immutable && a->uvals && a->uvals_valid && !a->uvals_scaled && !a->st_virtual) {
+    if (c->spmv_sym && c->atom_fast && m->sym_nx > 0 && !a->immutable && ((a->uvals && a->uvals_valid && !a->uvals_scaled) || a->derived) && !a->st_virtual) {
         const int64_t plane = (int64_t)m->sym_nx * m->sym_ny;
         const int64_t q0 = r0 < 0 ? 0 : r0, q1 = r1 < 0 ? m->nv : r1;
         if (q0 >= 0 && q1 <= m->nv && q0 <= q1 && q0 % plane == 0 && q1 % plane == 0)
@@ -2648,14 +2692,14 @@
     c->gram_op = 0; c->gram_k = 0; c->gram_n = 0;
     if (r1 == r0) return PGD_OK;
     bool sym = false;
-    PGD_TRY(ensure_sym(c, m, a, &sym));
+    if (!a->derived) PGD_TRY(ensure_sym(c, m, a, &sym));
     PGD_TRY(ensure_work(c, 3, m->nv));
     PGD_TRY(ensure_work(c, 6, 2 * (int64_t)MAX_VEC_BLOCKS > 256 ? 2 * (int64_t)MAX_VEC_BLOCKS : 256));
     double *w = c->work[3], *res = c->work[6];
     const bool dbg_t = getenv("PGD_DEBUG_PCG") != nullptr;
     auto dbg_now = [] { return std::chrono::duration<double>(std::chrono::steady_clock::now().time_since_epoch()).count(); };
     const double dbg_t0 = dbg_now();
-    if (k >= 2) PGD_TRY(dia_classify(c, m, a));
+    if (k >= 2 && !a->derived) PGD_TRY(dia_classify(c, m, a));
     if (dbg_t) fprintf(stderr, "[start_gram] k %d classify %.2f ms (cls %d stencil %d)\n", k, 1e3 * (dbg_now() - dbg_t0), a->cls_count, (int)a->st_ok);
     if (k <= GRAM9) {
         const size_t need = (size_t)k * (size_t)m->nv * sizeof(double);
```

Result: no change. 19.53 (-0.4%).
